# exanauts/SqpSolver.jl

Hardware: AMD Instinct MI355X
Metric: QP subproblems/sec on batched ACOPF; fp64 KKT LDL^T TFLOPS vs MFMA peak (higher is better)
Workload: dtype f64

## Files before the change

include/sqphip_test_hooks.h:

```cpp
#ifndef SQPHIP_TEST_HOOKS_H
#define SQPHIP_TEST_HOOKS_H
#include "sqphip.h"
#ifdef __cplusplus
extern "C" {
#endif

int sqphip_mf_host_solve(int64_t n, int64_t m, int64_t nnzJ, const int64_t *jrow, const int64_t *jcol,
                         int64_t nnzH, const int64_t *hrow, const int64_t *hcol, const double *gL, const double *gU,
                         int32_t condense, const double *Jval, const double *Hval, const double *Dd,
                         const double *sigp, const double *hd, const int32_t *rtype, double hsc, double dw,
                         const double *rhs, double *sol, double *dinv_by_unknown, int32_t *npos);
double sqphip_mf_host_top2_err(void);
double sqphip_mf_host_spine_err(void);
int sqphip_mf_solve_test(sqphip_ctx *ctx, int32_t inst, const double *Jval, const double *Hval, const double *Dd,
                         const double *sigp, const double *hd, const int32_t *rtype, double hsc, double dw,
                         const double *rhs, double *sol_fused, double *sol_standalone, double *dinv_by_unknown);
int sqphip_mf_batch_test(sqphip_ctx *ctx, const int32_t *active, const double *Jval, const double *Hval, const double *Dd,
                         const double *sigp, const double *hd, const int32_t *rtype, const double *hsc, const double *dw,
                         const double *dw_last, const int32_t *fac_attempt, const double *rhs, double *sol_fused,
                         double *sol_standalone, double *dinv0, double *dinv1, int32_t *decision, double *dw_out);
int sqphip_mf_census(const sqphip_ctx *ctx, int64_t *counts, char *names, int32_t cap, int32_t *n_kernels);
int sqphip_trans_inline_groups(const sqphip_ctx *ctx, int64_t *count);
int sqphip_mf_plan_info(int64_t n, int64_t m, int64_t nnzJ, const int64_t *jrow, const int64_t *jcol, int64_t nnzH,
                        const int64_t *hrow, const int64_t *hcol, const double *gL, const double *gU, int32_t condense,
                        int32_t batch, int32_t *fronts, int32_t cap_fronts, int32_t *n_fronts, int32_t *launches,
                        int32_t cap_launches, int32_t *n_launches, int64_t *top2_lds_bytes, int32_t *spine_fronts);
int sqphip_ldlt_factor_host(int32_t device, int32_t batch, int64_t N, double *A, double *dinv,
                            int32_t *npos);
int sqphip_ldlt_solve_host(int32_t device, int32_t batch, int64_t N, const double *A,
                           double *rhs);
int sqphip_ldlt_bench(int32_t device, int32_t batch, int64_t N, int32_t reps,
                      double *sec_per_factor, double *sec_trailing, int64_t *trailing_launches);
int sqphip_ldlt_tile_masks(int32_t batch, int64_t N, const double *A, int32_t Ts, uint8_t *tmask, int32_t *pair_ptr,
                           int32_t *pair_k, int32_t cap_k, int32_t *n_k);
int sqphip_ldlt_case_test(int32_t device, int32_t batch, int64_t N, const double *A, int32_t nan_upper, const double *rhs,
                          const int32_t *phase, int32_t want, int32_t Ts, int32_t no_tile_mask, double sentinel,
                          double *factor, double *dinv, int32_t *npos, double *b, double *v, double *x_fused,
                          double *x_standalone, int64_t *counts, char *names, int32_t cap, int64_t *info);

int sqphip_ldlt_stress(int32_t device, int32_t batch, int64_t N, int32_t reps, int32_t *mismatches);
int sqphip_mfma_f64_peak(int32_t device, double *tflops);

int sqphip_seat_peek(sqphip_ctx *ctx, int32_t inst, double *p, double *lambda, double *mult_x_U, double *mult_x_L,
                     double *slack, int32_t *moi_status);

#ifdef __cplusplus
}
#endif
#endif
```

sqpsolver.jl_amd/__init__.py:

```python
from . import acopf_synth
from . import dense_synth
from . import qcqp
from . import nlp_terms
from . import _lib
from . import host
from .host import (Context, QpData, QpHip, default_options, SqpHipError, kkt_order,
                   kkt_symbolic, mf_host_solve, mf_host_top2_err, mf_host_spine_err, mf_plan_info)
```

sqpsolver.jl_amd/_lib.py:

```python
from __future__ import annotations

import ctypes as C
import os
import subprocess
import sys

_CSRC = os.path.join(os.path.dirname(os.path.abspath(__file__)), "csrc")
SO_PATH = os.path.join(_CSRC, "libsqphip.so")
if os.environ.get("SQPHIP_SO"):
    SO_PATH = os.path.abspath(os.environ["SQPHIP_SO"])
SOURCES = ["ldlt.hip", "kernel_api.hip", "ipm.hip", "acopf.hip", "sqp.hip", "api.hip", "order.hip", "symbolic.hip",
           "mfplan.hip", "mfront.hip", "comm.hip"]
HEADERS = ["sqphip_internal.hpp", "ctx.hpp", "sparse.hpp", "dev_util.hpp", "mf_dev.hpp", "sqp_dev.hpp", "acopf_dev.hpp", "qcqp_dev.hpp", "nlp_dev.hpp", os.path.join("..", "..", "include", "sqphip.h"),
           os.path.join("..", "..", "include", "sqphip_test_hooks.h")]

_lib = None


EXTRA_FLAGS = {"mfront.hip": ["-mllvm", "-amdgpu-mfma-vgpr-form", "-mllvm", "-pragma-unroll-threshold=131072"]}
_OBJ = os.path.join(_CSRC, "build")


def build(force: bool = False, verbose: bool = False) -> str:
    from concurrent.futures import ThreadPoolExecutor
# ... 27 lines not shown
            if rc != 0 or verbose:
                sys.stderr.write("\n".join(other) + "\n")
            if rc != 0:
                raise subprocess.CalledProcessError(rc, cmd)
    objs = [os.path.join(_OBJ, sname + ".o") for sname in srcs]
    if jobs or not os.path.exists(SO_PATH) or any(os.path.getmtime(o) > os.path.getmtime(SO_PATH) for o in objs):
        cmd = [hipcc, "--offload-arch=gfx950", "-shared", "-fPIC", "-o", SO_PATH] + objs + ["-ldl"]
        if verbose:
            print(" ".join(cmd))
        subprocess.check_call(cmd)
        remarks = ""
        for o in objs:
            if os.path.exists(o + ".remarks"):
                remarks += open(o + ".remarks").read()
        _write_kernel_resources(remarks)
    return SO_PATH


RESOURCES_PATH = os.path.join(_CSRC, "kernel_resources.json")


def _write_kernel_resources(remarks: str) -> None:
    import json
    import re
    out, cur = {}, None
    for ln in remarks.splitlines():
        m = re.search(r"Function Name: (\S+)", ln)
        if m:
            cur = out.setdefault(m.group(1), {})
            continue
        m = re.search(r"remark:\s+(VGPRs|AGPRs|ScratchSize \[bytes/lane\]|LDS Size \[bytes/block\]|Occupancy \[waves/SIMD\]): (\d+)", ln)
        if m and cur is not None:
            cur[m.group(1).split(" [")[0]] = int(m.group(2))
    with open(RESOURCES_PATH, "w") as fh:
        json.dump(out, fh, indent=0, sort_keys=True)


class Options(C.Structure):
    _fields_ = [(k, C.c_double) for k in
                ("tol_direction", "tol_residual", "tol_infeas", "init_mu", "max_mu", "tr_size",
                 "rho", "eta", "tau", "min_alpha")] + \
               [("max_iter", C.c_int32), ("use_soc", C.c_int32), ("literal_quirks", C.c_int32),
                ("ipm_tol", C.c_double), ("ipm_max_iter", C.c_int32), ("ipm_phase1", C.c_int32),
                ("device", C.c_int32), ("ipm_corrector", C.c_int32),
                ("kkt_condense", C.c_int32), ("kkt_tile_order", C.c_int32), ("kkt_mode", C.c_int32),
                ("ipm_warm_start", C.c_int32)]


class Counters(C.Structure):
    _fields_ = [("n_qp", C.c_int64), ("n_ipm_iter", C.c_int64), ("n_factor", C.c_int64),
                ("ldlt_flops", C.c_double), ("ldlt_seconds", C.c_double),
                ("trailing_seconds", C.c_double), ("solve_seconds", C.c_double),
                ("total_seconds", C.c_double), ("trailing_launches", C.c_int64), ("kkt_order", C.c_int64),
                ("lead_tiles", C.c_int64), ("trailing_flops_per_factor", C.c_double),
                ("sparse", C.c_int64), ("nnz_k", C.c_int64), ("nnz_l", C.c_int64), ("n_supernodes", C.c_int64),
                ("n_levels", C.c_int64), ("max_front", C.c_int64), ("factor_flops", C.c_double),
                ("front_doubles", C.c_int64), ("cb_doubles", C.c_int64), ("factor_launches", C.c_int64),
                ("solve_launches", C.c_int64), ("n_sweeps", C.c_int64), ("n_solve", C.c_int64), ("n_groups", C.c_int64),
                ("nnz_l_top", C.c_int64), ("nnz_k_top", C.c_int64), ("cols_top", C.c_int64)]


class SymbolicStats(C.Structure):
    _fields_ = [(k, C.c_int64) for k in ("order", "nnz_k_lower", "n_supernodes", "n_levels", "max_front", "max_cols",
                                         "nnz_l", "nnz_l_exact")] + \
               [("flops", C.c_double), ("flops_exact", C.c_double), ("front_doubles", C.c_int64)]


def lib():
    global _lib
    if _lib is None:
        if not os.path.exists(SO_PATH):
            raise RuntimeError(
                f"{SO_PATH} is missing: build it with __graft_entry__.build() "
                "(hipcc --offload-arch=gfx950); this package has no CPU fallback")
        L = C.CDLL(SO_PATH)
        dp, ip, lp = C.POINTER(C.c_double), C.POINTER(C.c_int32), C.POINTER(C.c_int64)
        vp = C.c_void_p
        if hasattr(L, "sqphip_default_options"):
            L.sqphip_default_options.argtypes = [C.POINTER(Options)]
        L.sqphip_ldlt_factor_host.argtypes = [C.c_int32, C.c_int32, C.c_int64, dp, dp, ip]
        L.sqphip_ldlt_solve_host.argtypes = [C.c_int32, C.c_int32, C.c_int64, dp, dp]
        L.sqphip_ldlt_bench.argtypes = [C.c_int32, C.c_int32, C.c_int64, C.c_int32, dp, dp, lp]
        L.sqphip_mfma_f64_peak.argtypes = [C.c_int32, dp]
        L.sqphip_ldlt_tile_masks.argtypes = [C.c_int32, C.c_int64, dp, C.c_int32, C.POINTER(C.c_uint8), ip, ip, C.c_int32, ip]
        L.sqphip_ldlt_case_test.argtypes = [C.c_int32, C.c_int32, C.c_int64, dp, C.c_int32, dp, ip, C.c_int32, C.c_int32,
                                            C.c_int32, C.c_double, dp, dp, ip, dp, dp, dp, dp, lp, C.c_char_p, C.c_int32, lp]
        if hasattr(L, "sqphip_create"):
            L.sqphip_create.argtypes = [C.POINTER(vp), C.c_int64, C.c_int64, C.c_int64,
                                        C.c_int64, lp, lp, C.c_int64, lp, lp, dp, dp, dp, dp,
                                        C.POINTER(Options), C.c_int32]
            L.sqphip_destroy.argtypes = [vp]
            L.sqphip_last_error.restype = C.c_char_p
            L.sqphip_last_error.argtypes = [vp]
            L.sqphip_set_bounds.argtypes = [vp, C.c_int32, dp, dp, dp, dp]
            L.sqphip_qp_solve.argtypes = [vp, C.c_int32, dp, C.c_double, C.c_double, dp, dp, dp, dp,
                                          dp, dp, dp, dp, dp, ip]
            L.sqphip_qp_stats.argtypes = [vp, ip, ip]
            if hasattr(L, "sqphip_qp_solve_batch"):
                L.sqphip_qp_solve_batch.argtypes = [vp, C.c_int32, ip, ip] + [dp] * 7 + [dp] * 5 + [ip]
                L.sqphip_qp_stats_batch.argtypes = [vp, C.c_int32, ip, ip, ip, ip, dp]
                L.sqphip_seat_peek.argtypes = [vp, C.c_int32, dp, dp, dp, dp, dp, ip]
                L.sqphip_norm_violations_batch.argtypes = [vp, C.c_int32, ip, dp, dp, C.c_int32, dp]
                L.sqphip_kt_residuals_batch.argtypes = [vp, C.c_int32, ip, dp, dp, dp, dp, dp, dp]
                L.sqphip_norm_complementarity_batch.argtypes = [vp, C.c_int32, ip, dp, dp, C.c_int32, dp]
                L.sqphip_compute_phi_batch.argtypes = [vp, C.c_int32, ip, dp, dp, dp, dp, C.c_int32, dp]
                L.sqphip_compute_qmodel_batch.argtypes = [vp, C.c_int32, ip, dp, dp, dp, dp, dp, dp, dp, C.c_int32, dp]
                L.sqphip_compute_derivative_full_batch.argtypes = [vp, C.c_int32, ip, dp, dp, dp, dp, dp, C.c_int32, dp, dp]
            L.sqphip_qp_termination.argtypes = [vp, ip, dp]
            L.sqphip_sqp_qp_log_term.argtypes = [vp, C.c_int32, dp, ip, C.c_int32, ip]
            L.sqphip_get_termination_counters.argtypes = [vp, C.POINTER(C.c_int64)]
            L.sqphip_norm_violations.argtypes = [vp, dp, dp, C.c_int32, dp]
            L.sqphip_kt_residuals.argtypes = [vp, dp, dp, dp, dp, dp, dp]
            L.sqphip_norm_complementarity.argtypes = [vp, dp, dp, C.c_int32, dp]
            L.sqphip_compute_phi.argtypes = [vp, C.c_double, dp, dp, C.c_double, C.c_int32, dp]
            L.sqphip_compute_qmodel.argtypes = [vp, dp, dp, dp, dp, dp, dp, C.c_double, C.c_int32, dp]
            L.sqphip_compute_derivative.argtypes = [vp, dp, dp, dp, C.c_double, dp]
            L.sqphip_compute_derivative_full.argtypes = [vp, dp, dp, dp, C.c_double, dp, C.c_int32, dp, dp]
            L.sqphip_compute_mu_rule_dev.argtypes = [vp, C.c_int32, C.c_int64, C.c_double, dp, dp, dp, dp, dp, dp, dp]
            L.sqphip_acopf_armijo.argtypes = [vp, C.c_int32, dp, dp] + [C.c_double] * 6 + [C.c_int32, dp, ip, ip]
            L.sqphip_tr_update.argtypes = [C.c_double, C.c_double, C.c_double, C.c_double,
                                           C.c_double, C.c_double, ip, dp]
            L.sqphip_acopf_attach.argtypes = [vp, C.c_int32, C.c_int32, C.c_int32, ip, ip, ip, ip, ip,
                                              ip, dp, C.c_int32]
            L.sqphip_acopf_attach_acr.argtypes = [vp, C.c_int32, C.c_int32, C.c_int32, ip, ip, ip, ip, ip,
                                              ip, dp, C.c_int32]
            L.sqphip_acopf_attach_acwr.argtypes = [vp, C.c_int32, C.c_int32, C.c_int32, ip, ip, ip, ip, ip, ip, dp, C.c_int32,
                                                   C.c_int32, ip, ip, ip, dp, dp, dp]
            L.sqphip_acopf_set_instance.argtypes = [vp, C.c_int32, dp, dp, dp, dp]
            L.sqphip_dense_attach.argtypes = [vp, dp, dp, C.c_double]
            L.sqphip_dense_set_instance.argtypes = [vp, C.c_int32, dp, dp]
            L.sqphip_qcqp_attach.argtypes = [vp, C.c_int64, lp, lp, dp, C.c_int64, lp, lp, dp, C.c_int64, lp, lp, lp, dp,
                                             dp, dp, C.c_double]
            L.sqphip_qcqp_set_instance.argtypes = [vp, C.c_int32] + [dp] * 7
            if not os.environ.get("SQPHIP_SO") or hasattr(L, "sqphip_nlp_attach"):
                L.sqphip_nlp_attach.argtypes = [vp, C.c_int64, lp, dp, lp, lp, ip, ip, dp, dp, dp, C.c_double]
                L.sqphip_nlp_set_instance.argtypes = [vp, C.c_int32, dp, dp, dp, dp]
            if not os.environ.get("SQPHIP_SO") or hasattr(L, "sqphip_nlp_attach_affine"):
                L.sqphip_nlp_attach_affine.argtypes = [vp, C.c_int64, lp, dp, lp, lp, lp, dp, ip, ip, dp, dp, C.c_double]
            L.sqphip_acopf_set_shunts.argtypes = [vp, C.c_int32, ip, dp, dp]
            L.sqphip_acopf_set_dclines.argtypes = [vp, C.c_int32, dp]
            L.sqphip_kkt_order.argtypes = [C.c_int64, C.c_int64, C.c_int64, lp, lp, C.c_int64, lp, lp, dp, dp, C.c_int32,
                                           ip, ip, ip]
            L.sqphip_kkt_symbolic.argtypes = [C.c_int64, C.c_int64, C.c_int64, lp, lp, C.c_int64, lp, lp, dp, dp, C.c_int32,
                                              C.c_int32, C.c_int32, C.c_double, ip, C.POINTER(SymbolicStats)]
            L.sqphip_mf_host_solve.argtypes = [C.c_int64, C.c_int64, C.c_int64, lp, lp, C.c_int64, lp, lp, dp, dp, C.c_int32,
                                               dp, dp, dp, dp, dp, ip, C.c_double, C.c_double, dp, dp, dp, ip]
            L.sqphip_mf_host_top2_err.argtypes = []
            L.sqphip_mf_host_top2_err.restype = C.c_double
            L.sqphip_mf_host_spine_err.argtypes = []
            L.sqphip_mf_host_spine_err.restype = C.c_double
            L.sqphip_mf_solve_test.argtypes = [vp, C.c_int32, dp, dp, dp, dp, dp, ip, C.c_double, C.c_double, dp, dp, dp, dp]
            L.sqphip_mf_batch_test.argtypes = [vp, ip, dp, dp, dp, dp, dp, ip, dp, dp, dp, ip, dp, dp, dp, dp, dp, ip, dp]
            L.sqphip_mf_census.argtypes = [vp, lp, C.c_char_p, C.c_int32, ip]
            if hasattr(L, "sqphip_trans_inline_groups"):
                L.sqphip_trans_inline_groups.argtypes = [vp, lp]
            L.sqphip_mf_plan_info.argtypes = [C.c_int64, C.c_int64, C.c_int64, lp, lp, C.c_int64, lp, lp, dp, dp, C.c_int32,
                                              C.c_int32, ip, C.c_int32, ip, ip, C.c_int32, ip, lp, ip]
            L.sqphip_acopf_eval.argtypes = [vp, C.c_int32, dp, C.c_double, dp, dp, dp, dp, dp, dp]
            L.sqphip_sqp_reset.argtypes = [vp]
            L.sqphip_sqp_run.argtypes = [vp, C.c_int32]
            L.sqphip_sqp_get.argtypes = [vp, C.c_int32, dp, dp, dp, dp, dp, dp, ip, ip]
            L.sqphip_sqp_status.argtypes = [vp, ip, ip, ip]
            L.sqphip_sqp_trace.argtypes = [vp, C.c_int32, dp, C.c_int32, ip]
            L.sqphip_comm_unique_id.argtypes = [vp]
            L.sqphip_comm_init.argtypes = [vp, vp, C.c_int32, C.c_int32]
            L.sqphip_gather_status.argtypes = [vp, C.c_int32, ip, ip, ip]
            L.sqphip_comm_destroy.argtypes = [vp]
            L.sqphip_get_counters.argtypes = [vp, C.POINTER(Counters)]
            L.sqphip_get_mode_counters.argtypes = [vp, C.POINTER(C.c_int64)]
            L.sqphip_sqp_qp_log.argtypes = [vp, C.c_int32, ip, C.c_int32, ip]
            L.sqphip_sqp_last_request.argtypes = [vp, C.c_int32, ip, dp, dp, dp, dp, dp, dp, dp]
            L.sqphip_sqp_stream_begin.argtypes = [vp, C.c_int32]
            L.sqphip_sqp_stream_set.argtypes = [vp, C.c_int32] + [dp] * 8
            L.sqphip_sqp_stream_run.argtypes = [vp]
            L.sqphip_sqp_stream_get.argtypes = [vp, C.c_int32, dp, dp, ip, ip]
            L.sqphip_qcqp_stream_begin.argtypes = [vp, C.c_int32, C.c_int32]
            L.sqphip_qcqp_stream_set.argtypes = [vp, C.c_int32] + [dp] * 11
            L.sqphip_sqp_stream_get_full.argtypes = [vp, C.c_int32, dp, dp, dp, dp, dp, dp, ip, ip]
            if not os.environ.get("SQPHIP_SO") or hasattr(L, "sqphip_nlp_stream_begin"):
                L.sqphip_nlp_stream_begin.argtypes = [vp, C.c_int32, C.c_int32]
                L.sqphip_nlp_stream_set.argtypes = [vp, C.c_int32] + [dp] * 8
            L.sqphip_sqp_work.argtypes = [vp, C.POINTER(C.c_int64), C.POINTER(C.c_int64), C.POINTER(C.c_int64)]
            L.sqphip_reset_counters.argtypes = [vp]
            L.sqphip_set_timing.argtypes = [vp, C.c_int32]
            L.sqphip_get_kernel_times.argtypes = [vp, dp, C.POINTER(C.c_int64), C.c_int32]
        _lib = L
    return _lib


EXPORTS = [
    "sqphip_default_options", "sqphip_create", "sqphip_destroy", "sqphip_last_error",
    "sqphip_set_bounds", "sqphip_qp_solve", "sqphip_qp_stats",
    "sqphip_qp_solve_batch", "sqphip_qp_stats_batch", "sqphip_seat_peek", "sqphip_norm_violations_batch", "sqphip_kt_residuals_batch",
    "sqphip_norm_complementarity_batch", "sqphip_compute_phi_batch", "sqphip_compute_qmodel_batch",
    "sqphip_compute_derivative_full_batch", "sqphip_qp_termination", "sqphip_sqp_qp_log_term", "sqphip_get_termination_counters", "sqphip_norm_violations",
    "sqphip_kt_residuals", "sqphip_norm_complementarity", "sqphip_compute_phi",
    "sqphip_compute_qmodel", "sqphip_compute_derivative", "sqphip_compute_derivative_full", "sqphip_compute_mu_rule_dev",
    "sqphip_acopf_armijo", "sqphip_tr_update",
    "sqphip_kkt_order", "sqphip_kkt_symbolic", "sqphip_mf_host_solve", "sqphip_mf_host_top2_err", "sqphip_mf_host_spine_err", "sqphip_mf_solve_test", "sqphip_mf_batch_test", "sqphip_mf_census", "sqphip_trans_inline_groups", "sqphip_mf_plan_info", "sqphip_acopf_attach", "sqphip_acopf_attach_acr", "sqphip_acopf_attach_acwr", "sqphip_acopf_set_shunts", "sqphip_acopf_set_dclines", "sqphip_acopf_set_instance", "sqphip_dense_attach", "sqphip_dense_set_instance", "sqphip_qcqp_attach", "sqphip_qcqp_set_instance", "sqphip_nlp_attach", "sqphip_nlp_attach_affine", "sqphip_nlp_set_instance", "sqphip_acopf_eval", "sqphip_sqp_reset",
    "sqphip_sqp_run", "sqphip_sqp_get", "sqphip_sqp_status", "sqphip_sqp_trace",
    "sqphip_comm_available", "sqphip_comm_unique_id", "sqphip_comm_init", "sqphip_gather_status", "sqphip_comm_destroy",
    "sqphip_get_counters", "sqphip_get_mode_counters", "sqphip_sqp_work", "sqphip_sqp_stream_begin", "sqphip_sqp_stream_set", "sqphip_sqp_stream_run", "sqphip_sqp_stream_get", "sqphip_sqp_stream_assign", "sqphip_sqp_stream_append", "sqphip_sqp_stream_release", "sqphip_sqp_stream_run_some", "sqphip_qcqp_stream_begin", "sqphip_qcqp_stream_set", "sqphip_nlp_stream_begin", "sqphip_nlp_stream_set", "sqphip_sqp_stream_get_full", "sqphip_sqp_last_request", "sqphip_sqp_qp_log", "sqphip_reset_counters", "sqphip_set_timing", "sqphip_get_kernel_times", "sqphip_ldlt_factor_host",
    "sqphip_ldlt_solve_host", "sqphip_ldlt_bench", "sqphip_ldlt_stress", "sqphip_ldlt_tile_masks", "sqphip_ldlt_case_test", "sqphip_mfma_f64_peak", "sqphip_armijo_alpha", "sqphip_compute_mu_rule",
]
```

sqpsolver.jl_amd/csrc/api.hip:

```cpp
#include "ctx.hpp"
#include "qcqp_dev.hpp"
#include "nlp_dev.hpp"
#include <algorithm>
#include <array>
#include <chrono>
#include <cmath>
#include <cstring>
#include <tuple>
#include <unordered_map>

using namespace sqphip;

Ctx::~Ctx()
{
    lanes.clear();
    tm.flush();
    comm_release(*this);
    plan.destroy_lookahead();
    for (void *p : allocs) hipFree(p);
    if (h_counters) hipHostFree(h_counters);
    if (stg_h) hipHostFree(stg_h);
    if (side) { hipStreamDestroy(side); for (auto &e : evS) if (e) hipEventDestroy(e); for (auto &e : evC) if (e) hipEventDestroy(e); }
    if (stream && owns_stream) hipStreamDestroy(stream);
}
// ... 161 lines not shown
    const IpmState *ist;
    long ist_off;
};

template <bool TO_SLOTS>
__global__ __launch_bounds__(256) void k_seat_stage(StageMap M, double *stg, const int *inst)
{
    const int k = blockIdx.y, b = inst[k];
    double *row = stg + (long)k * M.row;
#pragma unroll
    for (int f = 0; f < SQPHIP_SEAT_FIELDS; ++f) {
        if (f >= M.nf) break;
        const int len = M.len[f];
        double *slot = M.base[f] + (long)b * M.stride[f];
        const bool al = ((unsigned long)slot & 15ul) == 0;
        for (int q = blockIdx.x * 256 + threadIdx.x; 2 * q < len; q += gridDim.x * 256) {
            const bool two = 2 * q + 1 < len;
            if (TO_SLOTS) {
                const double2 v = M.off[f] < 0 ? make_double2(0.0, 0.0) : *(const double2 *)(row + M.off[f] + 2 * q);
                if (two && al) *(double2 *)(slot + 2 * q) = v;
                else { slot[2 * q] = v.x; if (two) slot[2 * q + 1] = v.y; }
            } else {
                double2 v;
                if (two && al) v = *(const double2 *)(slot + 2 * q);
                else { v.x = slot[2 * q]; v.y = two ? slot[2 * q + 1] : 0.0; }
                *(double2 *)(row + M.off[f] + 2 * q) = v;
            }
        }
    }
    if (!TO_SLOTS && M.ist && blockIdx.x == 0) {
        constexpr int W = (int)(sizeof(IpmState) / 8);
        const unsigned long long *src = (const unsigned long long *)(M.ist + b);
        unsigned long long *dst = (unsigned long long *)(stg + M.ist_off) + (long)k * W;
        for (int w = threadIdx.x; w < W; w += 256) dst[w] = src[w];
    }
}
static_assert(sizeof(IpmState) % 8 == 0, "k_seat_stage copies IpmState in 8-byte words");

__global__ void k_mf_test_setup(DV d, int inst, double hsc, double dw, int ph)
{
    for (int i = threadIdx.x; i < d.B; i += blockDim.x) { d.phase[i] = PH_IDLE; d.ist[i].start = 0; }
    __syncthreads();
    if (threadIdx.x == 0) { d.ist[inst].hsc = hsc; d.ist[inst].dw = dw; d.ist[inst].stage = 0; d.ist[inst].sel = 0; d.ist[inst].fac_attempt = 0; d.phase[inst] = ph; }
}

__global__ void k_mf_inst_set(DV d, int inst, int start, int ph, double hsc, double dw, double dw_last, int fac_attempt)
{
    if (threadIdx.x != 0) return;
    IpmState &I = d.ist[inst];
    I.start = start;
    if (start) { I.mode = 0; I.delta = 1.0; I.mu_pen = 1.0; I.rho_big = 1e4; I.ipm_iters = 0; I.n_solve = 0; I.status = 0; }
    I.stage = 0; I.hsc = hsc; I.dw = dw; I.dw_last = dw_last; I.sel = 0; I.fac_attempt = fac_attempt; I.n_factor = 0; I.rc = 0;
    d.phase[inst] = ph;
}

}

extern "C" void sqphip_default_options(sqphip_options *o)
{
    o->tol_direction = 1e-8; o->tol_residual = 1e-8; o->tol_infeas = 1e-8;
    o->init_mu = 1.0; o->max_mu = 1e10; o->tr_size = 10.0;
    o->rho = 0.8; o->eta = 0.4; o->tau = 0.9; o->min_alpha = 1e-6;
    o->max_iter = 3000; o->use_soc = 0; o->literal_quirks = 1;
    o->ipm_tol = 1e-9; o->ipm_max_iter = 200; o->ipm_phase1 = 0; o->device = 0; o->ipm_corrector = 0; o->kkt_condense = 1; o->kkt_tile_order = 1;
    o->kkt_mode = 0; o->ipm_warm_start = 0;
}

extern "C" int sqphip_create(sqphip_ctx **out, int64_t n, int64_t m, int64_t num_linear, int64_t nnzJ,
                             const int64_t *jrow, const int64_t *jcol, int64_t nnzH, const int64_t *hrow,
                             const int64_t *hcol, const double *xL, const double *xU, const double *gL,
                             const double *gU, const sqphip_options *opt, int32_t batch)
{
    if (!out || n <= 0 || m < 0 || batch <= 0 || !opt || num_linear < 0 || num_linear > m) return SQPHIP_EINVAL;
    if (nnzJ < 0 || nnzH < 0 || (nnzJ > 0 && (!jrow || !jcol)) || (nnzH > 0 && (!hrow || !hcol))) return SQPHIP_EINVAL;
    if (!xL || !xU || (m > 0 && (!gL || !gU))) return SQPHIP_EINVAL;
    for (int64_t k = 0; k < nnzJ; ++k)
        if (jrow[k] < 1 || jrow[k] > m || jcol[k] < 1 || jcol[k] > n) return SQPHIP_EINVAL;
    for (int64_t k = 0; k < nnzH; ++k)
        if (hrow[k] < 1 || hrow[k] > n || hcol[k] < 1 || hcol[k] > n) return SQPHIP_EINVAL;
    for (int64_t i = 0; i < m; ++i)
        if (gL[i] == -INFINITY && gU[i] == INFINITY) return SQPHIP_EINVAL;
    sqphip_ctx *h = new (std::nothrow) sqphip_ctx();
    if (!h) return SQPHIP_ENOMEM;
    h->c.opt = *opt;
    int rc = guarded(h, [&](Ctx &C) {
        SQPHIP_HIP_OK(hipStreamCreate(&C.stream));
        SQPHIP_HIP_OK(hipHostMalloc((void **)&C.h_counters, 8 * sizeof(int)));
        DV &d = C.d;
        std::memset(&d, 0, sizeof(d));
        C.n = n; C.m = m;
        C.h_jrow.assign(jrow, jrow + nnzJ); C.h_jcol.assign(jcol, jcol + nnzJ);
        C.h_hrow.assign(hrow, hrow + nnzH); C.h_hcol.assign(hcol, hcol + nnzH);
        C.h_xL.assign(xL, xL + n); C.h_xU.assign(xU, xU + n);
        if (m > 0) { C.h_gL.assign(gL, gL + m); C.h_gU.assign(gU, gU + m); }
        const int B = batch;
        d.n = (int)n; d.m = (int)m; d.nlin = (int)num_linear; d.N = (int)(n + m);
        d.Npad = (d.N + 63) / 64 * 64; d.B = B;
        d.nnzj_coo = (int)nnzJ; d.nnzh_coo = (int)nnzH;
        Pattern PJ = build_pattern(n, nnzJ, jrow, jcol, false);
        Pattern PH = build_pattern(n, nnzH, hrow, hcol, true);
        d.nnzjc = (int)PJ.rowval.size(); d.nnzhc = (int)PH.rowval.size();
        d.hfull = n > 1 && (long)d.nnzhc == (long)n * n;
        std::vector<int> rptr(m + 1, 0), rcol(d.nnzjc), rslot(d.nnzjc);
        for (int s = 0; s < d.nnzjc; ++s) rptr[PJ.rowval[s] + 1]++;
        for (int64_t i = 0; i < m; ++i) rptr[i + 1] += rptr[i];
        {
            std::vector<int> fill(rptr.begin(), rptr.end() - 1);
            for (int j = 0; j < (int)n; ++j)
                for (int s = PJ.colptr[j]; s < PJ.colptr[j + 1]; ++s) {
                    const int i = PJ.rowval[s];
                    rcol[fill[i]] = j; rslot[fill[i]] = s; fill[i]++;
                }
        }
        d.jcolptr = C.upload(PJ.colptr); d.jrowval = C.upload(PJ.rowval);
        d.jrowptr = C.upload(rptr); d.jrcol = C.upload(rcol); d.jrslot = C.upload(rslot);
        {
            std::vector<int> kpos(m > 0 ? m : 1, -1), krow;
            for (int64_t i = 0; i < m; ++i)
                if (kkt_row_is_kept(gL[i], gU[i], rptr[i + 1] - rptr[i])) { kpos[i] = (int)krow.size(); krow.push_back((int)i); }
            d.condense = opt->kkt_condense != 0; d.mk = (int)krow.size();
            if (krow.empty()) krow.push_back(0);
            d.kpos = C.upload(kpos); d.krow = C.upload(krow);
            C.h_kpos = kpos;
        }
        {
            const std::vector<int> &kpos = C.h_kpos;
            const int nu = d.condense ? d.n + d.mk : d.N;
            std::vector<int> upos(nu);
            d.Ts = 0; d.Nf = nu; d.sparse = 0;
            if (opt->kkt_mode != 1) {
                std::vector<int> kp(kpos);
                if (!d.condense) for (int64_t i = 0; i < m; ++i) kp[i] = (int)i;
                const SymOptions so = mf_sym_options(B);
                C.mfp_ = std::make_shared<MfPlan>(mf_build_plan(d.n, (int)m, kp, d.condense ? d.mk : (int)m, PH.colptr, PH.rowval, rptr, rcol, rslot, so));
                const SparseSym &S = C.mfp().S;
                const double dense_flops = (double)nu * nu * nu / 3.0;
                const bool fits = S.max_front <= 1024;
                if (opt->kkt_mode == 2 && !fits) throw std::string("kkt_mode = 2: a front of " + std::to_string(S.max_front) + " rows exceeds the multifrontal kernels' limit (1024)");
                d.sparse = opt->kkt_mode == 2 || (fits && S.max_front <= 512 && S.flops <= 0.25 * dense_flops);
            }
            if (d.sparse) {
                const MfPlan &P = C.mfp();
                const SparseSym &S = P.S;
                upos = S.pos;
                MfDev &M = d.mf;
                M.ns = S.ns; M.stride = P.stride;
                M.first = C.upload(S.sn_first); M.nc = C.upload(S.sn_nc); M.nr = C.upload(S.sn_nr);
                M.rowptr = C.upload(S.sn_rowptr); M.rows = C.upload(S.sn_rows.empty() ? std::vector<int>(1, 0) : S.sn_rows);
                M.rel = C.upload(S.rel.empty() ? std::vector<int>(1, 0) : S.rel);
                M.child_ptr = C.upload(S.child_ptr); M.child = C.upload(S.child.empty() ? std::vector<int>(1, 0) : S.child);
                M.off = C.upload(P.off);
                M.asm_ptr = C.upload(P.asm_ptr); M.dest_loc = C.upload(P.dest_loc); M.item_ptr = C.upload(P.item_ptr);
                M.items = C.upload(P.items); M.sched = C.upload(P.sched);
                auto nz = [](const std::vector<int> &v) { return v.empty() ? std::vector<int>(1, 0) : v; };
                M.dest_rc = C.upload(P.dest_rc);
                M.ea_ptr = C.upload(P.ea_ptr); M.ea_rc = C.upload(nz(P.ea_rc));
                M.ea_src_ptr = C.upload(P.ea_src_ptr); M.ea_src = C.upload(nz(P.ea_src));
                M.ev_ptr = C.upload(P.ev_ptr); M.ev_idx = C.upload(nz(P.ev_idx));
                M.ev_src_ptr = C.upload(P.ev_src_ptr); M.ev_src = C.upload(nz(P.ev_src));
                M.level_ptr = C.upload(S.level_ptr); M.level_sn = C.upload(S.level_sn);
                M.nlevels = S.nlevels; M.max_front = S.max_front;
                M.sol_items = C.upload(nz(P.sol_items));
                M.desc = C.upload(P.desc);
                M.ea_ent = C.upload(P.ea_ent.empty() ? std::vector<MfGather>(1) : P.ea_ent);
                M.ev_ent = C.upload(P.ev_ent.empty() ? std::vector<MfGather>(1) : P.ev_ent);
                int lds_max = 0;
                if (hipDeviceGetAttribute(&lds_max, hipDeviceAttributeMaxSharedMemoryPerBlock, C.opt.device) != hipSuccess) lds_max = 0;
                M.top_n = P.top2_lds_bytes > 0 && P.top2_lds_bytes <= lds_max ? (int)P.top_fr.size() : 0;
                if (M.top_n > 0) {
                    M.top_fr = C.upload(P.top_fr); M.top_gptr = C.upload(P.top_gptr); M.top_gsrc = C.upload(nz(P.top_gsrc));
                    M.top_rows = C.upload(nz(P.top_rows)); M.top_ext = C.upload(nz(P.top_ext));
                    M.top_next = (int)P.top_ext.size(); M.top_utotal = P.top_utotal; M.top_xtotal = P.top_xtotal;
                    M.top_buf0 = P.top_buf0; M.top_buf1 = P.top_buf1;
                }
                M.sp_n = P.spine_lds_bytes > 0 && P.spine_lds_bytes <= lds_max ? (int)P.sp_fr.size() : 0;
                if (M.sp_n > 0) {
                    M.sp_fr = C.upload(P.sp_fr); M.sp_ent = C.upload(P.sp_ent.empty() ? std::vector<MfGather>(1) : P.sp_ent);
                    M.sp_src = C.upload(nz(P.sp_src)); M.sp_rel = C.upload(nz(P.sp_rel)); M.sp_T = P.spine_T; M.sp_stage = P.spine_stage;
                }
                M.nnzK = (int)P.nnzK;
                M.vals = C.dalloc<double>((size_t)B * P.nnzK);
                M.fronts = C.dalloc<double>((size_t)B * P.stride);
                const bool small_arena = (double)B * (double)P.stride * 8.0 <= 1e9;
                d.spec_mode = getenv("SQPHIP_MF_SPEC") ? atoi(getenv("SQPHIP_MF_SPEC")) : (B <= (opt->ipm_corrector ? 256 : 192) && small_arena ? 1 : 0);
                C.spec_tail = d.spec_mode == 0 && small_arena ? (getenv("SQPHIP_MF_SPEC_TAIL") ? atoi(getenv("SQPHIP_MF_SPEC_TAIL")) : (getenv("SQPHIP_MF_SPEC") ? 0 : 32)) : 0;
                C.spec_mode0 = d.spec_mode;
            } else if (d.condense && opt->kkt_tile_order) {
                KktOrder o = kkt_order(d.n, (int)m, kpos, d.mk, PH.colptr, PH.rowval, rptr, rcol, true);
                upos = o.pos; d.Ts = o.Ts; d.Nf = o.Nf;
                if (o.Ts > 0 && o.Tr > 0 && !getenv("SQPHIP_NO_TILE_MASK")) {
                    C.plan.tmask = C.upload(o.tmask);
                    d.tmask = C.plan.tmask;
                    C.plan.pair_ptr = C.upload(o.pair_ptr);
                    C.plan.pair_k = C.upload(o.pair_k.empty() ? std::vector<int>(1, 0) : o.pair_k);
                    double fl = 0.0;
                    for (int ti = 0, pi = 0; ti < o.Tr; ++ti)
                        for (int tj = 0; tj <= ti; ++tj, ++pi)
                            fl += (ti == tj ? 64.0 * 65.0 / 2.0 : 64.0 * 64.0) * 2.0 * 64.0 * (o.pair_ptr[pi + 1] - o.pair_ptr[pi]);
                    C.plan.lead_update_flops = fl;
                }
            } else {
                for (int u = 0; u < nu; ++u) upos[u] = u;
            }
            d.Fpad = (d.Nf + 63) / 64 * 64; d.ld = d.Fpad;
            std::vector<int> uinv(d.Fpad, -1);
            for (int u = 0; u < nu; ++u) uinv[upos[u]] = u;
            d.upos = C.upload(upos); d.uinv = C.upload(uinv);
        }
        d.hcolptr = C.upload(PH.colptr); d.hrowval = C.upload(PH.rowval);
        d.jg_ptr = C.upload(PJ.g_ptr); d.jg_src = C.upload(PJ.g_src);
        d.hg_ptr = C.upload(PH.g_ptr); d.hg_src = C.upload(PH.g_src);
        const size_t Bn = (size_t)B * n, Bm = (size_t)B * m, BN = (size_t)B * d.Npad;
        d.xL = C.dalloc<double>(Bn); d.xU = C.dalloc<double>(Bn);
        d.gL = C.dalloc<double>(Bm); d.gU = C.dalloc<double>(Bm);
        for (int b = 0; b < B; ++b) {
            h2d(C, d.xL + (size_t)b * n, xL, n); h2d(C, d.xU + (size_t)b * n, xU, n);
            h2d(C, d.gL + (size_t)b * m, gL, m); h2d(C, d.gU + (size_t)b * m, gU, m);
        }
        d.xk = C.dalloc<double>(Bn); d.cin = C.dalloc<double>(Bn); d.bE = C.dalloc<double>(Bm);
        d.jcoo = C.dalloc<double>((size_t)B * nnzJ); d.hcoo = C.dalloc<double>((size_t)B * nnzH);
        d.jv = C.dalloc<double>((size_t)B * d.nnzjc); d.hv = C.dalloc<double>((size_t)B * d.nnzhc);
        double **nvec[] = { &d.c, &d.hd, &d.lb, &d.ub, &d.p, &d.zl, &d.zu, &d.dp, &d.dzl, &d.dzu, &d.rd,
                            &d.sigp, &d.wn, &d.op, &d.omxU, &d.omxL, &d.x, &d.mxL, &d.mxU, &d.df, &d.pstep,
                            &d.psoc, &d.pmxL, &d.pmxU, &d.tmpx, &d.x0, &d.socZL, &d.socZU };
        for (auto pp : nvec) *pp = C.dalloc<double>(Bn);
        double **mvec[] = { &d.lo, &d.hi, &d.wp, &d.wm, &d.s, &d.tp, &d.tm, &d.y, &d.vl, &d.vu, &d.ds,
                            &d.dtp, &d.dtm, &d.dy, &d.dvl, &d.dvu, &d.rp, &d.Dd, &d.olam, &d.lambda, &d.E,
                            &d.plam, &d.Esoc, &d.tmpE, &d.hlam, &d.zp, &d.zm, &d.rdir,
                            &d.socZP, &d.socZM, &d.socVL, &d.socVU };
        for (auto pp : mvec) *pp = C.dalloc<double>(Bm);
        d.oslack = C.dalloc<double>(2 * Bm);
        d.rtype = C.dalloc<int>(Bm); d.rbase = C.dalloc<int>(Bm); d.hard = C.dalloc<int>(Bm);
        d.rhs = C.dalloc<double>(BN); d.sol = C.dalloc<double>(BN); d.wN = C.dalloc<double>(BN);
        const size_t BF = (size_t)B * d.Fpad;
        d.xv = C.dalloc<double>(BF); d.vv = C.dalloc<double>(BF); d.dinv = C.dalloc<double>(BF);
        d.K = C.dalloc<double>(d.sparse ? 1 : (size_t)B * d.ld * d.Fpad);
        d.ist = C.dalloc<IpmState>(B); d.sst = C.dalloc<SqpState>(B);
        d.phase = C.dalloc<int>(B); d.counters = C.dalloc<int>(64);
        d.trace = C.dalloc<double>((size_t)B * SQPHIP_TRACE_CAP * SQPHIP_TRACE_COLS);
        d.ipm_tol = opt->ipm_tol; d.ipm_max_iter = opt->ipm_max_iter; d.ipm_phase1 = opt->ipm_phase1; d.ipm_corrector = opt->ipm_corrector; d.ipm_warm = opt->ipm_warm_start;
        d.refine_tol = getenv("SQPHIP_REFINE_TOL") ? atof(getenv("SQPHIP_REFINE_TOL")) : 1e-11;
        d.vstage = (d.n + d.N <= 7000 && !getenv("SQPHIP_NO_VSTAGE")) ? d.n + d.N : 0;
        d.flat = getenv("SQPHIP_VEC_FLAT") ? (atoi(getenv("SQPHIP_VEC_FLAT")) != 0) : (d.vstage == 0 && d.n + d.N > 7000);
        d.vals_inline = d.sparse && !d.flat && getenv("SQPHIP_MF_VALS_INLINE") && atoi(getenv("SQPHIP_MF_VALS_INLINE")) == 1;
        if (d.vals_inline) C.spec_tail = 0;
        if (d.sparse && (d.spec_mode != 0 || C.spec_tail > 0)) {
            d.mf.vals1 = C.dalloc<double>((size_t)B * C.mfp().nnzK);
            d.mf.fronts1 = C.dalloc<double>((size_t)B * C.mfp().stride);
            d.vv1 = C.dalloc<double>(BF); d.dinv1 = C.dalloc<double>(BF);
        }
        if (d.flat) {
            d.vstage = 0;
            d.fH = C.dalloc<double>(Bn); d.fJt = C.dalloc<double>(Bn); d.fJ = C.dalloc<double>(Bm); d.fX = C.dalloc<double>(Bm);
        }
        d.tol_direction = opt->tol_direction; d.tol_residual = opt->tol_residual;
        d.tol_infeas = opt->tol_infeas; d.init_mu = opt->init_mu; d.tr_size = opt->tr_size;
        d.max_iter = opt->max_iter; d.use_soc = opt->use_soc; d.literal_quirks = opt->literal_quirks;
        C.plan.N = d.Nf; C.plan.Npad = d.Fpad; C.plan.T = d.Fpad / 64; C.plan.ld = d.ld; C.plan.B = B;
        C.plan.Ts = d.Ts;
        C.plan.stream = C.stream;
        if (opt->kkt_tile_order && !d.condense && !d.sparse)
            C.err = "note: options.kkt_tile_order needs options.kkt_condense = 1 and was ignored";
        if (!d.sparse) {
            C.plan.Wbuf = C.dalloc<double>((size_t)std::max(2 * LdltPlan::MAX_R, d.Ts) * B * d.Fpad * 64);
            C.plan.init_lookahead();
        }
        SQPHIP_HIP_OK(hipStreamSynchronize(C.stream));
        if (const char *e = getenv("SQPHIP_TRANS_PERIOD")) C.trans_period = atoi(e);
        if (const char *e = getenv("SQPHIP_TRANS_RIDE")) C.trans_ride = atoi(e);
        C.refine_slot = getenv("SQPHIP_REFINE_SLOT") && atoi(getenv("SQPHIP_REFINE_SLOT")) == 1;
        if (const char *e = getenv("SQPHIP_REFINE_PERIOD")) C.refine_period = atoi(e);
        if (d.sparse) mf_device_setup(C);
        C.post_split = getenv("SQPHIP_POST_SPLIT") && atoi(getenv("SQPHIP_POST_SPLIT")) == 1;
        C.side_mode = getenv("SQPHIP_SIDE_TRANS") && atoi(getenv("SQPHIP_SIDE_TRANS")) == 1;
        make_lanes(C);
        return SQPHIP_OK;
    });
    if (rc != SQPHIP_OK) {
        fprintf(stderr, "sqphip_create: %s\n", h->c.err.c_str());
        delete h;
        return rc;
    }
    *out = h;
    return SQPHIP_OK;
}

extern "C" void sqphip_destroy(sqphip_ctx *h)
{
    if (!h) return;
    hipSetDevice(h->c.opt.device);
    delete h;
}

extern "C" const char *sqphip_last_error(const sqphip_ctx *h) { return h ? h->c.err.c_str() : "null context"; }

extern "C" int sqphip_set_bounds(sqphip_ctx *h, int32_t inst, const double *xL, const double *xU,
                                 const double *gL, const double *gU)
{
    if (!h || inst < 0 || inst >= h->c.d.B || !xL || !xU || (h->c.d.m > 0 && (!gL || !gU))) return SQPHIP_EINVAL;
    for (int i = 0; i < h->c.d.m; ++i)
        if (gL[i] == -INFINITY && gU[i] == INFINITY) { h->c.err = "sqphip_set_bounds: row " + std::to_string(i) + " is unbounded on both sides"; return SQPHIP_EINVAL; }
    return guarded(h, [&](Ctx &C) {
        DV &d = C.d;
        if (d.condense)
            for (int i = 0; i < d.m; ++i)
                if (gL[i] == gU[i] && C.h_kpos[i] < 0) {
// ... 5 lines not shown
        h2d(C, d.gL + (size_t)inst * d.m, gL, d.m); h2d(C, d.gU + (size_t)inst * d.m, gU, d.m);
        SQPHIP_HIP_OK(hipStreamSynchronize(C.stream));
        return SQPHIP_OK;
    });
}

extern "C" int sqphip_qp_solve(sqphip_ctx *h, int32_t mode, const double *x_k, double delta, double mu,
                               const double *df, const double *E, const double *Jval, const double *Hval,
                               double *p, double *lambda, double *mult_x_U, double *mult_x_L, double *slack,
                               int32_t *moi_status)
{
    if (!h || !x_k || !Jval || !p || !lambda || !mult_x_U || !mult_x_L || !moi_status) return SQPHIP_EINVAL;
    if (mode < 0 || mode > SQPHIP_MODE_INFEAS) return SQPHIP_EINVAL;
    if (mode != SQPHIP_MODE_LP && (!df || !E)) return SQPHIP_EINVAL;
    return guarded(h, [&](Ctx &C) {
        DV &d = C.d;
        auto t0 = std::chrono::steady_clock::now();
        h2d(C, d.xk, x_k, d.n);
        h2d(C, d.cin, df, d.n);
        h2d(C, d.bE, E, d.m);
        h2d(C, d.jcoo, Jval, d.nnzj_coo);
        if (Hval) h2d(C, d.hcoo, Hval, d.nnzh_coo);
        else SQPHIP_HIP_OK(hipMemsetAsync(d.hcoo, 0, sizeof(double) * (size_t)d.nnzh_coo, C.stream));
        hipLaunchKernelGGL(k_qp_request, dim3(1), dim3(64), 0, C.stream, d, 0, (int)mode, delta, mu);
        launch_qp_gather(C);
        ipm_run_all(C);
        IpmState st;
        SQPHIP_HIP_OK(hipMemcpyAsync(&st, d.ist, sizeof(IpmState), hipMemcpyDeviceToHost, C.stream));
        d2h(C, p, d.op, d.n); d2h(C, lambda, d.olam, d.m);
        d2h(C, mult_x_U, d.omxU, d.n); d2h(C, mult_x_L, d.omxL, d.n);
        d2h(C, slack, d.oslack, 2 * (size_t)d.m);
        SQPHIP_HIP_OK(hipStreamSynchronize(C.stream));
        *moi_status = st.status;
        C.last_ipm_iters = st.ipm_iters; C.last_n_factor = st.n_factor;
        C.last_rule = st.rc == 0 ? st.acc_rule : -1; C.last_e0 = st.e0;
        C.n_qp += 1; C.n_ipm_iter += st.ipm_iters; C.n_factor += st.n_factor; C.n_solve += st.n_solve;
        C.total_seconds += std::chrono::duration<double>(std::chrono::steady_clock::now() - t0).count();
        return SQPHIP_OK;
    });
}

extern "C" int sqphip_mf_solve_test(sqphip_ctx *h, int32_t inst, const double *Jval, const double *Hval,
                                    const double *Dd, const double *sigp, const double *hd, const int32_t *rtype,
                                    double hsc, double dw, const double *rhs, double *sol_fused,
                                    double *sol_standalone, double *dinv_by_unknown)
{
    if (!h || inst < 0 || inst >= h->c.d.B || !Jval || !Dd || !sigp || !hd || !rtype || !rhs) return SQPHIP_EINVAL;
    if (!h->c.d.sparse) { h->c.err = "sqphip_mf_solve_test: the context does not use the sparse solver"; return SQPHIP_ESTATE; }
    return guarded(h, [&](Ctx &C) {
        DV &d = C.d;
        const SparseSym &S = C.mfp().S;
        const size_t on = (size_t)inst * d.n, om = (size_t)inst * d.m;
        h2d(C, d.jcoo + (size_t)inst * d.nnzj_coo, Jval, d.nnzj_coo);
        if (Hval) h2d(C, d.hcoo + (size_t)inst * d.nnzh_coo, Hval, d.nnzh_coo);
        else SQPHIP_HIP_OK(hipMemsetAsync(d.hcoo + (size_t)inst * d.nnzh_coo, 0, sizeof(double) * (size_t)d.nnzh_coo, C.stream));
        hipLaunchKernelGGL(k_qp_request, dim3(1), dim3(64), 0, C.stream, d, (int)inst, 0, 1.0, 1.0);
        launch_qp_gather(C);
        hipLaunchKernelGGL(k_mf_test_setup, dim3(1), dim3(64), 0, C.stream, d, (int)inst, hsc, dw, (int)PH_FACTOR);
        h2d(C, d.Dd + om, Dd, d.m); h2d(C, d.sigp + on, sigp, d.n); h2d(C, d.hd + on, hd, d.n);
        SQPHIP_HIP_OK(hipMemcpyAsync(d.rtype + om, rtype, sizeof(int) * (size_t)d.m, hipMemcpyHostToDevice, C.stream));
        std::vector<double> xp(d.Fpad, 0.0), out(d.Fpad), dv(d.Fpad);
        for (int u = 0; u < S.nu; ++u) xp[S.pos[u]] = rhs[u];
        double *xv = d.xv + (size_t)inst * d.Fpad;
        h2d(C, xv, xp.data(), d.Fpad);
        mf_factor(C, PH_FACTOR, true);
        mf_solve(C, PH_FACTOR, true);
        d2h(C, out.data(), xv, d.Fpad); d2h(C, dv.data(), d.dinv + (size_t)inst * d.Fpad, d.Fpad);
        SQPHIP_HIP_OK(hipStreamSynchronize(C.stream));
        for (int u = 0; u < S.nu; ++u) {
            if (sol_fused) sol_fused[u] = out[S.pos[u]];
            if (dinv_by_unknown) dinv_by_unknown[u] = dv[S.pos[u]];
        }
        h2d(C, xv, xp.data(), d.Fpad);
        mf_solve(C, PH_FACTOR, false);
        d2h(C, out.data(), xv, d.Fpad);
        hipLaunchKernelGGL(k_mf_test_setup, dim3(1), dim3(64), 0, C.stream, d, (int)inst, 0.0, 0.0, (int)PH_IDLE);
        SQPHIP_HIP_OK(hipStreamSynchronize(C.stream));
        SQPHIP_HIP_OK(hipGetLastError());
        if (sol_standalone) for (int u = 0; u < S.nu; ++u) sol_standalone[u] = out[S.pos[u]];
        return SQPHIP_OK;
    });
}

extern "C" int sqphip_mf_batch_test(sqphip_ctx *h, const int32_t *active, const double *Jval, const double *Hval,
                                    const double *Dd, const double *sigp, const double *hd, const int32_t *rtype,
                                    const double *hsc, const double *dw, const double *dw_last, const int32_t *fac_attempt,
                                    const double *rhs, double *sol_fused, double *sol_standalone, double *dinv0,
                                    double *dinv1, int32_t *decision, double *dw_out)
{
    if (!h || !active || !Jval || !Dd || !sigp || !hd || !rtype || !hsc || !dw || !dw_last || !fac_attempt || !rhs)
        return SQPHIP_EINVAL;
    if (!h->c.d.sparse) { h->c.err = "sqphip_mf_batch_test: the context does not use the sparse solver"; return SQPHIP_ESTATE; }
    return guarded(h, [&](Ctx &C) {
        DV &d = C.d;
        const SparseSym &S = C.mfp().S;
        const int B = d.B, nu = S.nu;
        std::vector<double> xp((size_t)B * d.Fpad, 0.0), out((size_t)B * d.Fpad), dv((size_t)B * d.Fpad), dv1((size_t)B * d.Fpad, 0.0);
        for (int b = 0; b < B; ++b) {
            const size_t on = (size_t)b * d.n, om = (size_t)b * d.m;
            h2d(C, d.jcoo + (size_t)b * d.nnzj_coo, Jval + (size_t)b * d.nnzj_coo, d.nnzj_coo);
            if (Hval) h2d(C, d.hcoo + (size_t)b * d.nnzh_coo, Hval + (size_t)b * d.nnzh_coo, d.nnzh_coo);
            else SQPHIP_HIP_OK(hipMemsetAsync(d.hcoo + (size_t)b * d.nnzh_coo, 0, sizeof(double) * (size_t)d.nnzh_coo, C.stream));
            h2d(C, d.Dd + om, Dd + om, d.m); h2d(C, d.sigp + on, sigp + on, d.n); h2d(C, d.hd + on, hd + on, d.n);
            SQPHIP_HIP_OK(hipMemcpyAsync(d.rtype + om, rtype + om, sizeof(int) * (size_t)d.m, hipMemcpyHostToDevice, C.stream));
            for (int u = 0; u < nu; ++u) xp[(size_t)b * d.Fpad + S.pos[u]] = rhs[(size_t)b * nu + u];
            hipLaunchKernelGGL(k_mf_inst_set, dim3(1), dim3(64), 0, C.stream, d, b, active[b] ? 1 : 0, (int)PH_IDLE, 0.0, 0.0, 0.0, 0);
        }
        h2d(C, d.xv, xp.data(), xp.size());
        launch_qp_gather(C);
        for (int b = 0; b < B; ++b)
            hipLaunchKernelGGL(k_mf_inst_set, dim3(1), dim3(64), 0, C.stream, d, b, 0, active[b] ? (int)PH_FACTOR : (int)PH_IDLE,
                               hsc[b], dw[b], dw_last[b], (int)fac_attempt[b]);
        const bool top_inertia = mf_solve_tests_inertia(C);
        mf_factor(C, PH_FACTOR, true);
        if (!top_inertia) launch_inertia(C);
        mf_solve(C, PH_SOLVE, true, top_inertia);
        d2h(C, out.data(), d.xv, out.size()); d2h(C, dv.data(), d.dinv, dv.size());
        if (d.dinv1) d2h(C, dv1.data(), d.dinv1, dv1.size());
        std::vector<IpmState> st(B);
        std::vector<int> ph(B);
        SQPHIP_HIP_OK(hipMemcpyAsync(st.data(), d.ist, sizeof(IpmState) * (size_t)B, hipMemcpyDeviceToHost, C.stream));
        SQPHIP_HIP_OK(hipMemcpyAsync(ph.data(), d.phase, sizeof(int) * (size_t)B, hipMemcpyDeviceToHost, C.stream));
        SQPHIP_HIP_OK(hipStreamSynchronize(C.stream));
        for (int b = 0; b < B; ++b) {
            const size_t f = (size_t)b * d.Fpad, o = (size_t)b * nu;
            for (int u = 0; u < nu; ++u) {
                if (sol_fused) sol_fused[o + u] = out[f + S.pos[u]];
                if (dinv0) dinv0[o + u] = dv[f + S.pos[u]];
                if (dinv1) dinv1[o + u] = dv1[f + S.pos[u]];
            }
            const IpmState &I = st[b];
            const bool spec = d.mf.fronts1 != nullptr && d.spec_mode != 0 && (fac_attempt[b] > 0 || (d.spec_mode == 1 && dw[b] > 0.0));
            if (decision) {
                int32_t *r = decision + 5 * (size_t)b;
                r[0] = !active[b] ? 0 : ph[b] == PH_FACTOR ? 1 : ph[b] == PH_SOLVE ? 2 : 3;
                r[1] = I.sel; r[2] = I.n_factor; r[3] = I.fac_attempt; r[4] = active[b] && spec ? 1 : 0;
            }
            if (dw_out) dw_out[b] = I.dw;
        }
        h2d(C, d.xv, xp.data(), xp.size());
        mf_solve(C, PH_SOLVE, false);
        d2h(C, out.data(), d.xv, out.size());
        for (int b = 0; b < B; ++b)
            hipLaunchKernelGGL(k_mf_inst_set, dim3(1), dim3(64), 0, C.stream, d, b, 0, (int)PH_IDLE, 0.0, 0.0, 0.0, 0);
        SQPHIP_HIP_OK(hipStreamSynchronize(C.stream));
        SQPHIP_HIP_OK(hipGetLastError());
        if (sol_standalone)
            for (int b = 0; b < B; ++b)
                for (int u = 0; u < nu; ++u) sol_standalone[(size_t)b * nu + u] = out[(size_t)b * d.Fpad + S.pos[u]];
        return SQPHIP_OK;
    });
}

extern "C" int sqphip_mf_census(const sqphip_ctx *h, int64_t *counts, char *names, int32_t cap, int32_t *n_kernels)
{
    if (!h || cap < 0 || (cap > 0 && !counts)) return SQPHIP_EINVAL;
    if (n_kernels) *n_kernels = MFK_COUNT;
    for (int k = 0; k < MFK_COUNT && k < cap; ++k) {
        long c = h->c.mf_census[k];
        for (const auto &L : h->c.lanes) c += L->mf_census[k];
        counts[k] = c;
        if (names) { std::strncpy(names + 64 * (size_t)k, mf_kernel_names[k], 63); names[64 * (size_t)k + 63] = 0; }
    }
    return SQPHIP_OK;
}

extern "C" int sqphip_trans_inline_groups(const sqphip_ctx *h, int64_t *count)
{
    if (!h || !count) return SQPHIP_EINVAL;
    long c = h->c.n_trans_inline;
    for (const auto &L : h->c.lanes) c += L->n_trans_inline;
    *count = c;
    return SQPHIP_OK;
}

extern "C" int sqphip_qp_stats(const sqphip_ctx *h, int32_t *ipm_iters, int32_t *n_factor)
{
    if (!h) return SQPHIP_EINVAL;
    if (ipm_iters) *ipm_iters = h->c.last_ipm_iters;
    if (n_factor) *n_factor = h->c.last_n_factor;
    return SQPHIP_OK;
}

extern "C" int sqphip_qp_termination(const sqphip_ctx *h, int32_t *rule, double *scaled_error)
{
    if (!h) return SQPHIP_EINVAL;
    if (rule) *rule = h->c.last_rule;
    if (scaled_error) *scaled_error = h->c.last_e0;
    return SQPHIP_OK;
}

namespace {

inline long ev(long k) { return (k + 1) & ~1L; }

int seat_check(sqphip_ctx *h, const char *fn, int32_t count, const int32_t *inst)
{
    Ctx &C = h->c;
    if (count < 1 || count > C.d.B) { C.err = std::string(fn) + ": count " + std::to_string(count) + " is outside 1 .. batch = " + std::to_string(C.d.B); return SQPHIP_EINVAL; }
    if (!inst) { C.err = std::string(fn) + ": inst is NULL"; return SQPHIP_EINVAL; }
    std::vector<int> seen((size_t)C.d.B, -1);
    for (int k = 0; k < count; ++k) {
        if (inst[k] < 0 || inst[k] >= C.d.B) { C.err = std::string(fn) + ": inst[" + std::to_string(k) + "] = " + std::to_string(inst[k]) + " is outside 0 .. batch - 1 = " + std::to_string(C.d.B - 1); return SQPHIP_EINVAL; }
        if (seen[inst[k]] >= 0) { C.err = std::string(fn) + ": inst[" + std::to_string(k) + "] = " + std::to_string(inst[k]) + " repeats inst[" + std::to_string(seen[inst[k]]) + "]"; return SQPHIP_EINVAL; }
        seen[inst[k]] = k;
    }
    return SQPHIP_OK;
}

struct SeatCall {
    Ctx &C;
    int count; long cp, rows0;
    StageMap in{}, out{};
    const double *src[SQPHIP_SEAT_FIELDS] = {};
    SeatCall(Ctx &C_, int count_) : C(C_), count(count_), cp(ev(count_)), rows0(3 * ev(count_))
    {
        if (!C.stg_h) {
            const DV &d = C.d;
            const long row = 3 * ev(d.n) + 4 * ev(d.m) + ev(d.nnzj_coo) + ev(d.nnzh_coo) + (long)(sizeof(IpmState) / 8) + 2;
            C.stg_doubles = 3 * ev(d.B) + (long)d.B * row;
            SQPHIP_HIP_OK(hipHostMalloc((void **)&C.stg_h, sizeof(double) * (size_t)C.stg_doubles));
            C.stg_d = C.dalloc<double>((size_t)C.stg_doubles);
        }
    }
    double *a0() { return C.stg_h; }
    double *a1() { return C.stg_h + cp; }
    int *inst() { return (int *)(C.stg_h + 2 * cp); }
    int *mode() { return (int *)(C.stg_h + 2 * cp) + cp; }
    const double *a0_dev() const { return C.stg_d; }
    const double *a1_dev() const { return C.stg_d + cp; }
    const int *inst_dev() const { return (const int *)(C.stg_d + 2 * cp); }
    const int *mode_dev() const { return (const int *)(C.stg_d + 2 * cp) + cp; }
    void operand(const double *host, double *base, int len, bool zero = false)
    {
        if ((!host && !zero) || len == 0) return;
        const int f = in.nf++;
        in.len[f] = len; in.stride[f] = len; in.base[f] = base; src[f] = host;
        in.off[f] = host ? in.row : -1;
        if (host) in.row += (int)ev(len);
    }
    void result(double *base, int len)
    {
        if (len == 0) return;
        const int f = out.nf++;
        out.len[f] = len; out.stride[f] = len; out.base[f] = base; out.off[f] = out.row;
        out.row += (int)ev(len);
    }
    static dim3 grid(const StageMap &M, int count) { return dim3((unsigned)std::min(32L, std::max(1L, (M.row / 2 + 255L) / 256)), (unsigned)count); }
    void send(const int32_t *inst_host, const int32_t *mode_host, const double *a0_host, const double *a1_host)
    {
        for (int k = 0; k < count; ++k) {
            a0()[k] = a0_host ? a0_host[k] : 0.0; a1()[k] = a1_host ? a1_host[k] : 0.0;
            inst()[k] = inst_host[k]; mode()[k] = mode_host ? mode_host[k] : 0;
        }
        for (int k = 0; k < count; ++k)
            for (int f = 0; f < in.nf; ++f)
                if (src[f]) std::memcpy(C.stg_h + rows0 + (long)k * in.row + in.off[f], src[f] + (size_t)k * in.len[f], sizeof(double) * (size_t)in.len[f]);
        SQPHIP_HIP_OK(hipMemcpyAsync(C.stg_d, C.stg_h, sizeof(double) * (size_t)(rows0 + (long)count * in.row), hipMemcpyHostToDevice, C.stream));
        if (in.nf) hipLaunchKernelGGL(k_seat_stage<true>, grid(in, count), dim3(256), 0, C.stream, in, C.stg_d + rows0, inst_dev());
    }
    long fetch(bool with_states, long extra = 0)
    {
        const long body = (long)count * out.row;
        out.ist = with_states ? C.d.ist : nullptr; out.ist_off = body;
        if (out.nf || with_states) hipLaunchKernelGGL(k_seat_stage<false>, grid(out, count), dim3(256), 0, C.stream, out, C.stg_d + rows0, inst_dev());
        const long total = body + (with_states ? (long)count * (long)(sizeof(IpmState) / 8) : 0) + extra;
        SQPHIP_HIP_OK(hipMemcpyAsync(C.stg_h + rows0, C.stg_d + rows0, sizeof(double) * (size_t)total, hipMemcpyDeviceToHost, C.stream));
        SQPHIP_HIP_OK(hipStreamSynchronize(C.stream));
        SQPHIP_HIP_OK(hipGetLastError());
        return body;
    }
    void unpack(int f, double *host) const
    {
        if (!host) return;
        for (int k = 0; k < count; ++k)
            std::memcpy(host + (size_t)k * out.len[f], C.stg_h + rows0 + (long)k * out.row + out.off[f], sizeof(double) * (size_t)out.len[f]);
    }
    IpmState state(int k, long body) const
    {
        IpmState st;
        std::memcpy(&st, (const char *)(C.stg_h + rows0 + body) + sizeof(IpmState) * (size_t)k, sizeof(IpmState));
        return st;
    }
};

}

extern "C" int sqphip_qp_solve_batch(sqphip_ctx *h, int32_t count, const int32_t *inst, const int32_t *mode, const double *x_k,
                                     const double *delta, const double *mu, const double *df, const double *E,
                                     const double *Jval, const double *Hval, double *p, double *lambda, double *mult_x_U,
                                     double *mult_x_L, double *slack, int32_t *moi_status)
{
    if (!h || !mode || !x_k || !delta || !mu || !Jval || !p || !lambda || !mult_x_U || !mult_x_L || !moi_status) return SQPHIP_EINVAL;
    if (int rc = seat_check(h, "sqphip_qp_solve_batch", count, inst)) return rc;
    for (int k = 0; k < count; ++k) {
        if (mode[k] < 0 || mode[k] > SQPHIP_MODE_INFEAS) { h->c.err = "sqphip_qp_solve_batch: mode[" + std::to_string(k) + "] = " + std::to_string(mode[k]) + " is no sub-problem mode"; return SQPHIP_EINVAL; }
        if (mode[k] != SQPHIP_MODE_LP && (!df || !E)) { h->c.err = "sqphip_qp_solve_batch: mode[" + std::to_string(k) + "] needs df and E"; return SQPHIP_EINVAL; }
    }
    return guarded(h, [&](Ctx &C) {
        DV &d = C.d;
        auto t0 = std::chrono::steady_clock::now();
        SeatCall S(C, count);
        S.operand(x_k, d.xk, d.n); S.operand(df, d.cin, d.n); S.operand(E, d.bE, d.m);
        S.operand(Jval, d.jcoo, d.nnzj_coo); S.operand(Hval, d.hcoo, d.nnzh_coo, true);
        S.send(inst, mode, delta, mu);
        hipLaunchKernelGGL(k_qp_request_batch, dim3(1), dim3(256), 0, C.stream, d, (int)count, S.inst_dev(), S.mode_dev(), S.a0_dev(), S.a1_dev());
// ... 1546 lines not shown
```

sqpsolver.jl_amd/csrc/ctx.hpp:

```cpp
#pragma once
#include <memory>
#include <vector>
#include "../../include/sqphip.h"
#include "../../include/sqphip_test_hooks.h"
#include "sqphip_internal.hpp"
#include "sparse.hpp"

namespace sqphip {

enum { PH_IDLE = 0, PH_PREP = 1, PH_FACTOR = 2, PH_SOLVE = 3, PH_STEP = 4, PH_MPC = 5, PH_RESOLVE = 6, PH_DONE = 9,
       PH_PEND = 10, PH_DONE2 = 11, PH_PREP_S = 12 };
enum { ROW_FREE = 0, ROW_EQ = 1, ROW_INEQ = 2 };

enum MfKernel { MFK_VALUES, MFK_FACTOR_R1, MFK_F2_1_3, MFK_F2_2_5, MFK_F2_4_4, MFK_F2_4_9, MFK_F2_8_12,
                MFK_FRONT_1, MFK_FRONT_2, MFK_FRONT_3, MFK_FRONT_4_2, MFK_FRONT_4_4, MFK_FRONT_5_2, MFK_FRONT_5_4,
                MFK_FRONT_6_4, MFK_FRONT_6_4_IMG, MFK_FRONT_6_8_IMG, MFK_FRONT_7_4, MFK_FRONT_7_4_IMG, MFK_FRONT_7_8_IMG,
                MFK_FRONT_8_4, MFK_FRONT_8_4_IMG, MFK_FRONT_8_8_IMG, MFK_FRONT_9, MFK_FRONT_10, MFK_FRONT_11, MFK_FRONT_12,
                MFK_SPINE, MFK_SOLVE_INST, MFK_FWD, MFK_FWD2, MFK_FWD2_BIG, MFK_SOLVE_TOP, MFK_SOLVE_TOP2, MFK_BWD, MFK_BWD2,
                MFK_BWD2_BIG, MFK_INERTIA, MFK_COUNT };
extern const char *const mf_kernel_names[];

struct IpmState {
    int mode, start, stage;
    double delta, mu_pen;
    double sf, rho_big, soft_w, hsc;
    double mu, tau, dw, dw_last, dw_floor, cn, relres, rn, e0;
    int iter, rc, fac_attempt, dir_attempt, refine_it, n_acc, n_acc2, n_acc3;
    int mpc, use_soc;
    double cavg;
    double e_best;
    int n_stall;
    int prev_mode;
    int status, ipm_iters, n_factor, n_solve;
    int reload;
    int sel;
    int acc_rule;
    double elastic;
};

#define SQPHIP_QLOG_CAP 64
struct SqpState {
    double f, phi, mu, Delta, prim_infeas, dual_infeas, pnorm, obj_val;
    double f_trial, phi_k, q0, ared, pred;
    int iter, ret, step_acceptance, fr, sub_status, done, stage, need_qp, qp_mode, want_eval;
    int n_qp, trace_len, it_ipm, soc_pending, lp_pending, started;
    long tot_ipm, tot_fac, tot_sol;
    long md_qp[4], md_ipm[4], md_fac[4];
    int qlog_n, qlog[4 * SQPHIP_QLOG_CAP];
    float qerr[SQPHIP_QLOG_CAP];
    signed char qrule[SQPHIP_QLOG_CAP];
    long term_rule[4];
    int budget;
};

enum { ST_TOP = 0, ST_QP = 1, ST_SOC = 2, ST_LP = 3, ST_DONE = 4 };

#define SQPHIP_TRACE_COLS 12
#define SQPHIP_TRACE_CAP 4096

struct MfDev {
    int ns;
    const int *first, *nc, *nr, *rowptr, *rows, *rel, *child_ptr, *child;
    const long *off;
    long stride;
    double *fronts;
    double *fronts1, *vals1;
    const int *asm_ptr, *dest_loc, *dest_rc, *item_ptr;
    const MfItem *items;
    const int *ea_ptr, *ea_rc, *ea_src_ptr, *ea_src;
    const int *ev_ptr, *ev_idx, *ev_src_ptr, *ev_src;
    const MfFrontDesc *desc;
    const MfGather *ea_ent, *ev_ent;
    const int *level_ptr, *level_sn;
    int nlevels, max_front;
    const int *sched, *sol_items;
    const MfTopFront *top_fr;
    const int *top_gptr, *top_gsrc, *top_rows, *top_ext;
    int top_n, top_next, top_utotal, top_xtotal, top_buf0, top_buf1;
    const MfSpineFront *sp_fr;
    const MfGather *sp_ent;
    const int *sp_src, *sp_rel;
    int sp_n, sp_T, sp_stage;
    int nnzK;
    double *vals;
};

struct StreamDev {
    int M;
    int *next;
    int *qend;
    int *qids;
    int *slot_scen;
    const double *xL, *xU, *gL, *gU, *ohm, *c2, *c1, *x0;
    double *rx, *robj;
    int *rstat, *riter;
    const double *val;
    double *rE, *rlam, *rmxL, *rmxU;
};

struct QcqpDev;
struct NlpDev;

struct DV {
    int n, m, nlin, N, Npad, ld, B;
    int Nf, Fpad;
    int condense, mk;
    const int *kpos, *krow;
    const int *upos, *uinv;
    int Ts;
    const unsigned char *tmask;
    int sparse;
    MfDev mf;
    int nnzj_coo, nnzh_coo, nnzjc, nnzhc;
    const int *jcolptr, *jrowval, *jrowptr, *jrcol, *jrslot;
    const int *hcolptr, *hrowval;
    const int *jg_ptr, *jg_src, *hg_ptr, *hg_src;
    double *xL, *xU, *gL, *gU;
    double *xk, *cin, *bE, *jcoo, *hcoo, *jv, *hv;
    double *c, *hd, *lb, *ub, *lo, *hi, *wp, *wm;
    int *rtype, *rbase, *hard;
    double *p, *zl, *zu, *s, *tp, *tm, *y, *vl, *vu, *zp, *zm, *rdir;
    double *dp, *dzl, *dzu, *ds, *dtp, *dtm, *dy, *dvl, *dvu;
    double *rd, *rp, *sigp, *Dd, *rhs, *sol, *wn, *wN;
    double *socZL, *socZU, *socZP, *socZM, *socVL, *socVU;
    double *K, *dinv, *xv, *vv;
    double *dinv1, *vv1;
    int spec_mode;
    double *op, *olam, *omxU, *omxL, *oslack;
    IpmState *ist;
    int *phase;
    int *counters;
    double ipm_tol;
    int ipm_max_iter, ipm_phase1, ipm_corrector, ipm_warm;
    int side;
    double refine_tol;
    int vstage;
    int hfull;
    int vals_inline;
    int flat;
    double *fH, *fJt, *fJ, *fX;
    double *x, *lambda, *mxL, *mxU, *df, *E, *pstep, *psoc, *plam, *pmxL, *pmxU, *Esoc, *tmpx, *tmpE,
        *hlam;
    SqpState *sst;
    double *trace;
    int nb, ng, nl, ref_bus;
    StreamDev stream;
    int dense_nlp;
    const double *dnQ, *dnA;
    double *dnc; double dn_kappa;
    int acr;
    int acwr, nbp;
    const int *bp_i, *bp_j, *br_bp;
    const double *br_sig, *bp_tmin, *bp_tmax;
    int ndc; const double *dc_loss1;
    int nsh; const int *sh_bus, *sh_of_bus; const double *sh_gs, *sh_bs;
    const int *f_bus, *t_bus, *gen_bus, *bal_ptr, *bal_colP, *bal_colQ;
    const double *bal_coef;
    double *br_ohm, *c2, *c1, *x0;
    double tol_direction, tol_residual, tol_infeas, init_mu, tr_size;
    int max_iter, use_soc, literal_quirks;
    const QcqpDev *qc;
    double *qcv;
    const NlpDev *nlp;
    double *nlv, *nlw;
};

static __device__ __forceinline__ int ph_done(const DV &d) { return d.side == 2 ? PH_DONE2 : PH_DONE; }
static __device__ __forceinline__ int ph_prep(const DV &d) { return d.side == 1 ? PH_PREP_S : PH_PREP; }
static __device__ __forceinline__ int ph_fact(const DV &d) { return d.side == 1 ? PH_PEND : PH_FACTOR; }

struct Ctx {
    sqphip_options opt;
    DV d;
    LdltPlan plan;
    std::shared_ptr<MfPlan> mfp_;
    const MfPlan &mfp() const { return *mfp_; }
    std::vector<std::unique_ptr<Ctx>> lanes;
    bool is_lane = false, owns_stream = true;
    long mf_factor_launches = 0, n_sweeps = 0;
    long mf_census[MFK_COUNT] = {};
    long run_sweep = 0;
    bool post_split = false;
    bool want_resolve = true;
    bool side_mode = false, side_on = false;
    hipStream_t side = nullptr;
    hipEvent_t evS[4] = {}, evC[4] = {};
    int spec_tail = 0, spec_mode0 = 0;
    bool refine_slot = false;
    int refine_period = 0;
    long resolve_served = -1;
    int trans_period = 0;
    int trans_ride = -1;
    long n_trans_inline = 0;
    Timers tm;
    std::vector<void *> allocs;
    std::string err;
    hipStream_t stream = nullptr;
    int *h_counters = nullptr;
    double *stg_h = nullptr, *stg_d = nullptr;
    long stg_doubles = 0;
    std::vector<int> h_kpos;
    std::vector<int64_t> h_jrow, h_jcol, h_hrow, h_hcol;
    long qc_nv = 0;
    long qc_off[7] = {};
    std::vector<double> h_qc_base;
    long nl_nv = 0, nl_nfac = 0, nl_nterms = 0;
    std::vector<double> h_nl_base;
    std::vector<double> h_xL, h_xU, h_gL, h_gU;
    bool acopf_attached = false;
    bool mf_big_lds = false;
    bool stream_started = false;
    void *comm = nullptr, *comm_buf = nullptr;
    int comm_world = 1, comm_rank = 0, comm_cap = 0;
    int64_t n = 0, m = 0;
    int64_t n_qp = 0, n_ipm_iter = 0, n_factor = 0, n_solve = 0;
    double total_seconds = 0;
    int last_ipm_iters = 0, last_n_factor = 0, last_rule = -1;
    double last_e0 = 0.0;

    template <class T> T *dalloc(size_t count)
    {
        void *p = nullptr;
        SQPHIP_HIP_OK(hipMalloc(&p, sizeof(T) * (count ? count : 1)));
        SQPHIP_HIP_OK(hipMemsetAsync(p, 0, sizeof(T) * (count ? count : 1), stream));
        allocs.push_back(p);
        return (T *)p;
    }
    template <class T> T *upload(const std::vector<T> &v)
    {
        T *p = dalloc<T>(v.size());
        if (!v.empty())
            SQPHIP_HIP_OK(hipMemcpyAsync(p, v.data(), sizeof(T) * v.size(), hipMemcpyHostToDevice, stream));
        return p;
    }
    ~Ctx();
};

void ipm_run_all(Ctx &C);
bool ipm_sweep(Ctx &C, bool sqp_level, int *host_slot = nullptr);
void sqp_stage_kernels(Ctx &C, hipStream_t s, const DV &d);
void sqp_stream_arm(Ctx &C);
void sqp_stream_rearm(Ctx &C);
void launch_qp_gather(Ctx &C);
void comm_release(Ctx &C);
void mf_device_setup(Ctx &C);
void mf_factor(Ctx &C, int want, bool with_rhs, bool values_done = false);
void mf_solve(Ctx &C, int want, bool skip_fwd, bool inertia = false, int also = -1);
bool mf_solve_tests_inertia(const Ctx &C);
void launch_inertia(Ctx &C);
void launch_acopf_eval_point(Ctx &C, int inst, const double *x_dev, double sigma, const double *lam_dev,
                             double *f_dev, double *grad_dev, double *g_dev, double *jcoo_dev,
                             double *hcoo_dev);
void sqp_reset(Ctx &C);
void sqp_run(Ctx &C, int max_outer);
void merit_eval(Ctx &C, int op, double a0, double a1, int flag, double *out_host);
void merit_eval_batch(Ctx &C, int count, const int *inst_dev, int op, const double *a0_dev, const double *a1_dev, int flag,
                      double *out_dev);
void armijo_eval(Ctx &C, int inst, double mu, double phi0, double D, double eta, double tau, double min_alpha, int fr,
                 double *out3_host);

}

struct sqphip_ctx { sqphip::Ctx c; };
```

sqpsolver.jl_amd/csrc/mfplan.hip:

```cpp
#include "sparse.hpp"
#include "../../include/sqphip.h"
#include "../../include/sqphip_test_hooks.h"
#include <algorithm>
#include <cmath>
#include <cstdio>
#include <cstdlib>
#include <tuple>

namespace sqphip {

MfPlan mf_build_plan(int n, int m, const std::vector<int> &kpos, int mk, const std::vector<int> &hcolptr,
                     const std::vector<int> &hrowval, const std::vector<int> &jrowptr, const std::vector<int> &jrcol,
                     const std::vector<int> &jrslot, const SymOptions &opt)
{
    MfPlan P;
    std::vector<std::vector<int>> adj, before;
    kkt_graph(n, m, kpos, mk, hcolptr, hrowval, jrowptr, jrcol, adj, before);
    P.S = sparse_symbolic(n + mk, adj, before, opt);
    const SparseSym &S = P.S;
    P.off.resize(S.ns);
    for (int s = 0; s < S.ns; ++s) {
        const long fs = S.sn_nc[s] + S.sn_nr[s];
        P.off[s] = P.stride;
        P.stride += ((fs + 1) * fs + 1) / 2 * 2;
    }
    struct Rec { int sn, loc, seq; MfItem it; };
    std::vector<Rec> recs;
    auto add = [&](int ua, int ub, MfItem it) {
        int pa = S.pos[ua], pb = S.pos[ub];
        if (pa < pb) std::swap(pa, pb);
        const int s = S.col2sn[pb], f = S.sn_first[s], nc = S.sn_nc[s], fs = nc + S.sn_nr[s];
        int li;
        if (pa < f + nc) li = pa - f;
        else {
            const int *R = S.sn_rows.data() + S.sn_rowptr[s];
            const int *q = std::lower_bound(R, R + S.sn_nr[s], pa);
            if (q == R + S.sn_nr[s] || *q != pa) { fprintf(stderr, "sqphip: mf_build_plan: entry outside its front\n"); abort(); }
            li = nc + (int)(q - R);
        }
        recs.push_back({s, (pb - f) * (fs + 1) + li, (int)recs.size(), it});
    };
    for (int j = 0; j < n; ++j) {
        add(j, j, {MF_ITEM_VDIAG, -1, j, 0});
        for (int k = hcolptr[j]; k < hcolptr[j + 1]; ++k) {
            const int i = hrowval[k];
            if (i >= j) add(i, j, {MF_ITEM_H, -1, k, 0});
        }
    }
    for (int i = 0; i < m; ++i) {
        const int s = jrowptr[i], e = jrowptr[i + 1];
        if (kpos[i] >= 0) {
            add(n + kpos[i], n + kpos[i], {MF_ITEM_RDIAG, i, 0, 0});
            for (int t = s; t < e; ++t) add(n + kpos[i], jrcol[t], {MF_ITEM_JKEPT, i, jrslot[t], 0});
        } else {
            for (int a = s; a < e; ++a)
                for (int b = s; b <= a; ++b) add(jrcol[a], jrcol[b], {MF_ITEM_PAIR, i, jrslot[a], jrslot[b]});
        }
    }
    std::sort(recs.begin(), recs.end(), [](const Rec &x, const Rec &y) {
        return std::tie(x.sn, x.loc, x.seq) < std::tie(y.sn, y.loc, y.seq); });
    P.asm_ptr.assign(S.ns + 1, 0);
    for (size_t r = 0; r < recs.size(); ++r) {
        const bool fresh = r == 0 || recs[r].sn != recs[r - 1].sn || recs[r].loc != recs[r - 1].loc;
        if (fresh) {
            P.dest_loc.push_back(recs[r].loc);
            P.item_ptr.push_back((int)P.items.size());
            P.asm_ptr[recs[r].sn + 1]++;
        }
        P.items.push_back(recs[r].it);
    }
    P.item_ptr.push_back((int)P.items.size());
    for (int s = 0; s < S.ns; ++s) P.asm_ptr[s + 1] += P.asm_ptr[s];
    P.nnzK = (long)P.dest_loc.size();
    P.dest_rc.resize(P.dest_loc.size());
    for (int s = 0; s < S.ns; ++s) {
        const int ld = S.sn_nc[s] + S.sn_nr[s] + 1;
        for (int e = P.asm_ptr[s]; e < P.asm_ptr[s + 1]; ++e) P.dest_rc[e] = (P.dest_loc[e] % ld) | ((P.dest_loc[e] / ld) << 16);
    }
    if (P.stride >= (1L << 31)) { fprintf(stderr, "sqphip: mf_build_plan: front arena too large for 32-bit offsets\n"); abort(); }
    const bool big_solve = !(getenv("SQPHIP_MF_BIG_SOLVE") && atoi(getenv("SQPHIP_MF_BIG_SOLVE")) == 0);
    P.top_level = S.nlevels;
    if (big_solve && !(getenv("SQPHIP_MF_TOP") && atoi(getenv("SQPHIP_MF_TOP")) == 0)) {
        auto joins = [&](int lev) {
            const int cnt = S.level_ptr[lev + 1] - S.level_ptr[lev];
            if (cnt <= 2) return true;
            if (cnt > 4 || getenv("SQPHIP_MF_TOP_NARROW")) return false;
            for (int q = S.level_ptr[lev]; q < S.level_ptr[lev + 1]; ++q)
                if (S.sn_nc[S.level_sn[q]] + S.sn_nr[S.level_sn[q]] > 64) return false;
            return true;
        };
        int l = S.nlevels;
        while (l > 0 && joins(l - 1)) --l;
        if (S.nlevels - l >= 2) P.top_level = l;
    }
    P.spine_level = P.top_level; P.narrow_level = P.top_level;
    auto children_of = [&](int s) {
        std::vector<int> ch(S.child.begin() + S.child_ptr[s], S.child.begin() + S.child_ptr[s + 1]);
        std::stable_sort(ch.begin(), ch.end(), [&](int a, int b) { return (S.sn_level[a] >= P.spine_level) < (S.sn_level[b] >= P.spine_level); });
        return ch;
    };
    P.ea_ptr.assign(S.ns + 1, 0);
    P.ea_src_ptr.push_back(0);
    {
        std::vector<std::tuple<int, int, int>> con;
        for (int s = 0; s < S.ns; ++s) {
            const int fs = S.sn_nc[s] + S.sn_nr[s];
            con.clear();
            for (int c : children_of(s)) {
                const int cnc = S.sn_nc[c], cnr = S.sn_nr[c], cld = cnc + cnr + 1;
                const int *rel = S.rel.data() + S.sn_rowptr[c];
                for (int jj = 0; jj < cnr; ++jj)
                    for (int ii = jj; ii <= cnr; ++ii)
                        con.emplace_back(rel[jj], ii < cnr ? rel[ii] : fs, (int)(P.off[c] + (long)(cnc + jj) * cld + cnc + ii));
            }
            std::stable_sort(con.begin(), con.end(), [](const std::tuple<int, int, int> &a, const std::tuple<int, int, int> &b) {
                return std::tie(std::get<0>(a), std::get<1>(a)) < std::tie(std::get<0>(b), std::get<1>(b)); });
            for (size_t r = 0; r < con.size(); ++r) {
                const bool fresh = r == 0 || std::get<0>(con[r]) != std::get<0>(con[r - 1]) || std::get<1>(con[r]) != std::get<1>(con[r - 1]);
                if (fresh) {
                    if (r) P.ea_src_ptr.push_back((int)P.ea_src.size());
                    P.ea_rc.push_back(std::get<1>(con[r]) | (std::get<0>(con[r]) << 16));
                    P.ea_ptr[s + 1]++;
                }
                P.ea_src.push_back(std::get<2>(con[r]));
            }
            if (!con.empty()) P.ea_src_ptr.push_back((int)P.ea_src.size());
        }
        for (int s = 0; s < S.ns; ++s) P.ea_ptr[s + 1] += P.ea_ptr[s];
    }
    P.ev_ptr.assign(S.ns + 1, 0);
    P.ev_src_ptr.push_back(0);
    {
        std::vector<std::pair<int, int>> con;
        for (int s = 0; s < S.ns; ++s) {
            con.clear();
            for (int q = S.child_ptr[s]; q < S.child_ptr[s + 1]; ++q) {
                const int c = S.child[q], cnc = S.sn_nc[c], cnr = S.sn_nr[c], cfs = cnc + cnr, cld = cfs + 1;
                const int *rel = S.rel.data() + S.sn_rowptr[c];
                for (int jj = 0; jj < cnr; ++jj) con.emplace_back(rel[jj], (int)(P.off[c] + (long)(cnc + jj) * cld + cfs));
            }
            std::stable_sort(con.begin(), con.end(), [](const std::pair<int, int> &a, const std::pair<int, int> &b) { return a.first < b.first; });
            for (size_t r = 0; r < con.size(); ++r) {
                if (r == 0 || con[r].first != con[r - 1].first) {
                    if (r) P.ev_src_ptr.push_back((int)P.ev_src.size());
                    P.ev_idx.push_back(con[r].first);
                    P.ev_ptr[s + 1]++;
                }
                P.ev_src.push_back(con[r].second);
            }
            if (!con.empty()) P.ev_src_ptr.push_back((int)P.ev_src.size());
        }
        for (int s = 0; s < S.ns; ++s) P.ev_ptr[s + 1] += P.ev_ptr[s];
    }
    auto tiles = [&](int s) { return (S.sn_nc[s] + S.sn_nr[s] + 1 + 15) / 16; };
    auto cls = [&](int s) { const int T = tiles(s); return T <= 2 ? 1 : (T <= 6 ? T - 1 : (T <= 8 ? 7 : (T <= 13 ? 8 : 9))); };
    for (int l = 0; l < S.nlevels; ++l) {
        int cnt = 0, tmax = 0;
        for (int q = S.level_ptr[l]; q < S.level_ptr[l + 1]; ++q) { ++cnt; tmax = std::max(tmax, tiles(S.level_sn[q])); }
        const int merge_t = getenv("SQPHIP_MF_MERGE_T") ? atoi(getenv("SQPHIP_MF_MERGE_T")) : opt.merge_tiles;
        const bool merge = ((cnt <= 8 && tmax <= 8) || tmax <= merge_t) && !getenv("SQPHIP_MF_NO_LEVEL_MERGE");
        for (int c = 0; c < 10; ++c) {
            MfLaunch L{(int)P.sched.size(), 0, 0, 0, c, 0};
            L.level = l;
            for (int q = S.level_ptr[l]; q < S.level_ptr[l + 1]; ++q) {
                const int s = S.level_sn[q];
                if (merge ? c != tmax - 1 : cls(s) != c) continue;
                P.sched.push_back(s);
                L.count++;
                L.tiles = std::max(L.tiles, tiles(s));
            }
            if (!L.count) continue;
            if (!merge && c == 1) L.tiles = 2;
            if (!merge && c == 7) L.tiles = 8;
            P.fac.push_back(L);
        }
    }
    auto build_solve_launches = [&]() {
    P.sol_items.clear(); P.fwd.clear(); P.bwd.clear(); P.top = MfLaunch{0, 0, 256, 0, 0, 0};
    int top_maxfs = 64, top_lcap = 0;
    for (int l = 0; l < S.nlevels; ++l) {
        const bool top = l >= P.top_level;
        MfLaunch L{(int)P.sol_items.size() / 4, 0, 256, 0, 0, 0};
        int maxfs = 64, lcap = 0;
        std::vector<int> small;
        for (int q = S.level_ptr[l]; q < S.level_ptr[l + 1]; ++q) {
            const int s = S.level_sn[q], fs = S.sn_nc[s] + S.sn_nr[s];
            if (!big_solve) maxfs = std::max(maxfs, fs);
            if (fs > 64 && big_solve) {
                for (int t : {s, -2, -2, -2}) P.sol_items.push_back(t);
                maxfs = std::max(maxfs, fs);
                const int nc = S.sn_nc[s];
                if (nc <= 80) lcap = std::max(lcap, nc * nc);
            } else small.push_back(s);
        }
        for (size_t q = 0; q < small.size(); q += 4)
            for (size_t t = q; t < q + 4; ++t) P.sol_items.push_back(t < small.size() ? small[t] : -1);
        L.count = (int)P.sol_items.size() / 4 - L.begin;
        L.tiles = big_solve ? 64 : maxfs;
        L.cls = std::max(4 * L.tiles, maxfs + 16);
        L.lds_bytes = 8 * (L.cls + lcap);
        {
            int wimg = 0; long bigimg = 0; bool ok2 = big_solve;
            for (int q = S.level_ptr[l]; q < S.level_ptr[l + 1]; ++q) {
                const int s = S.level_sn[q], nc = S.sn_nc[s], fs = nc + S.sn_nr[s];
                if (fs > 128 || nc > 112) { ok2 = false; break; }
                if (fs > 64) bigimg = std::max(bigimg, (long)nc * (fs | 1)); else wimg = std::max(wimg, nc * (fs | 1));
            }
            const long lds2 = 8 * std::max(4L * (64 + wimg), 128 + bigimg);
            if (ok2 && lds2 <= 150 * 1024) { L.wimg = wimg; L.lds2 = (int)lds2; L.hasbig = bigimg > 0 ? 1 : 0; }
        }
        if (!top) { P.fwd.push_back(L); continue; }
        if (l == P.top_level) P.top.begin = L.begin;
        P.top.count += L.count;
        top_maxfs = std::max(top_maxfs, maxfs); top_lcap = std::max(top_lcap, lcap);
    }
    if (P.top.count) {
        P.top.tiles = 64;
        P.top.cls = std::max(4 * 64, top_maxfs + 16);
        P.top.lds_bytes = 8 * (P.top.cls + top_lcap);
    }
    P.bwd.assign(P.fwd.rbegin(), P.fwd.rend());
    };
    build_solve_launches();
    if (P.top.count > 0 && !(getenv("SQPHIP_MF_TOP2") && atoi(getenv("SQPHIP_MF_TOP2")) == 0)) {
        std::vector<int> kof(S.ns, -1);
        bool ok = true;
// ... 200 lines not shown
                        err = std::max(err, std::fabs(img[c * Rn + r] - A[c * ld + r]));
                        scale = std::max(scale, std::fabs(A[c * ld + r]));
                    }
                g_spine_err = std::max(g_spine_err, err / std::max(scale, 1e-300));
            }
        }
        for (int k = 0; k < nc; ++k) {
            const double d = A[k * ld + k], di = 1.0 / d;
            dinv[f0 + k] = di;
            for (int j = k + 1; j < fs; ++j) {
                const double lj = A[k * ld + j] * di;
                for (int i = j; i <= fs; ++i) A[j * ld + i] -= A[k * ld + i] * lj;
            }
            for (int i = k + 1; i <= fs; ++i) A[k * ld + i] *= di;
            v[f0 + k] = A[k * ld + fs];
        }
    }
    g_top2_err = -1.0;
    std::vector<double> xtop, ytop;
    if (P.top2_lds_bytes > 0) {
        const int n_ext = (int)P.top_ext.size();
        std::vector<double> uvec(n_ext + P.top_utotal, 0.0), y;
        xtop.assign(P.top_xtotal, 0.0); ytop.assign(P.top_xtotal, 0.0);
        for (int t = 0; t < n_ext; ++t) uvec[t] = F[P.top_ext[t]];
        double err = 0.0, scale = 0.0;
        for (const MfTopFront &T : P.top_fr) {
            const int nc = T.nc, fs = T.nc + T.nr, ld = fs + 1;
            const double *A = F.data() + T.off;
            y.assign(fs, 0.0);
            for (int i = 0; i < fs; ++i) {
                if (i < nc) y[i] = x[T.first + i];
                for (int q = P.top_gptr[T.gptr + i]; q < P.top_gptr[T.gptr + i + 1]; ++q) y[i] += uvec[P.top_gsrc[T.gsrc0 + q]];
            }
            for (int k = 0; k < nc; ++k)
                for (int i = k + 1; i < fs; ++i) y[i] -= A[k * ld + i] * y[k];
            for (int i = 0; i < nc; ++i) {
                ytop[T.xloc + i] = y[i] * dinv[T.first + i];
                err = std::max(err, std::fabs(ytop[T.xloc + i] - v[T.first + i])); scale = std::max(scale, std::fabs(v[T.first + i]));
            }
            for (int i = nc; i < fs; ++i) uvec[n_ext + T.uoff + i - nc] = y[i];
        }
        g_top2_err = err / std::max(scale, 1e-300);
    }
    for (int s = S.ns - 1; s >= 0; --s) {
        const int nc = S.sn_nc[s], nr = S.sn_nr[s], fs = nc + nr, ld = fs + 1, f0 = S.sn_first[s];
        const double *A = F.data() + P.off[s];
        const int *R = S.sn_rows.data() + S.sn_rowptr[s];
        for (int k = nc - 1; k >= 0; --k) {
            double a = v[f0 + k];
            for (int i = k + 1; i < nc; ++i) a -= A[k * ld + i] * x[f0 + i];
            for (int r = 0; r < nr; ++r) a -= A[k * ld + nc + r] * x[R[r]];
            x[f0 + k] = a;
        }
    }
    if (P.top2_lds_bytes > 0) {
        double err = 0.0, scale = 0.0;
        std::vector<double> t;
        for (int k = (int)P.top_fr.size() - 1; k >= 0; --k) {
            const MfTopFront &T = P.top_fr[k];
            const int nc = T.nc, nr = T.nr, fs = nc + nr, ld = fs + 1;
            const double *A = F.data() + T.off;
            t.assign(nc, 0.0);
            for (int c = 0; c < nc; ++c) {
                t[c] = ytop[T.xloc + c];
                for (int r = 0; r < nr; ++r) t[c] -= A[c * ld + nc + r] * xtop[P.top_rows[T.rloc + r]];
            }
            for (int i = nc - 1; i >= 1; --i)
                for (int c = 0; c < i; ++c) t[c] -= A[c * ld + i] * t[i];
            for (int c = 0; c < nc; ++c) {
                xtop[T.xloc + c] = t[c];
                err = std::max(err, std::fabs(t[c] - x[T.first + c])); scale = std::max(scale, std::fabs(x[T.first + c]));
            }
        }
        g_top2_err = std::max(g_top2_err, err / std::max(scale, 1e-300));
    }
    for (int u = 0; u < S.nu; ++u) sol[u] = x[S.pos[u]];
}

}

extern "C" double sqphip_mf_host_top2_err(void) { return sqphip::g_top2_err; }
extern "C" double sqphip_mf_host_spine_err(void) { return sqphip::g_spine_err; }

namespace {

sqphip::MfPlan host_plan(int64_t n, int64_t m, int64_t nnzJ, const int64_t *jrow, const int64_t *jcol, int64_t nnzH,
                         const int64_t *hrow, const int64_t *hcol, const double *gL, const double *gU, int32_t condense,
                         const sqphip::SymOptions &so, const double *Jval, const double *Hval, std::vector<double> &jv,
                         std::vector<double> &hv)
{
    using namespace sqphip;
    struct Ent { int c, r; double v; };
    auto build = [](int64_t ncols, int64_t nnz, const int64_t *row, const int64_t *col, const double *val, bool sym,
                    std::vector<int> &colptr, std::vector<int> &rowval, std::vector<double> &vals) {
        std::vector<Ent> e;
        for (int64_t k = 0; k < nnz; ++k) {
            e.push_back({(int)col[k] - 1, (int)row[k] - 1, val ? val[k] : 0.0});
            if (sym && row[k] != col[k]) e.push_back({(int)row[k] - 1, (int)col[k] - 1, val ? val[k] : 0.0});
        }
        std::stable_sort(e.begin(), e.end(), [](const Ent &a, const Ent &b) { return std::tie(a.c, a.r) < std::tie(b.c, b.r); });
        colptr.assign(ncols + 1, 0);
        for (size_t i = 0; i < e.size(); ++i) {
            if (i && e[i].c == e[i - 1].c && e[i].r == e[i - 1].r) { vals.back() += e[i].v; continue; }
            rowval.push_back(e[i].r); vals.push_back(e[i].v); colptr[e[i].c + 1]++;
        }
        for (int64_t j = 0; j < ncols; ++j) colptr[j + 1] += colptr[j];
    };
    std::vector<int> jcp, jrv, hcp, hrv;
    build(n, nnzJ, jrow, jcol, Jval, false, jcp, jrv, jv);
    build(n, nnzH, hrow, hcol, Hval, true, hcp, hrv, hv);
    std::vector<int> rptr(m + 1, 0), rcol(jrv.size()), rslot(jrv.size());
    for (int r : jrv) rptr[r + 1]++;
    for (int64_t i = 0; i < m; ++i) rptr[i + 1] += rptr[i];
    {
        std::vector<int> fill(rptr.begin(), rptr.end() - 1);
        for (int j = 0; j < (int)n; ++j)
            for (int s = jcp[j]; s < jcp[j + 1]; ++s) { const int i = jrv[s]; rcol[fill[i]] = j; rslot[fill[i]] = s; fill[i]++; }
    }
    std::vector<int> kpos(m > 0 ? m : 1, -1);
    int mk = 0;
    for (int64_t i = 0; i < m; ++i)
        if (!condense || kkt_row_is_kept(gL[i], gU[i], rptr[i + 1] - rptr[i])) kpos[i] = mk++;
    return mf_build_plan((int)n, (int)m, kpos, mk, hcp, hrv, rptr, rcol, rslot, so);
}

}

extern "C" int sqphip_mf_host_solve(int64_t n, int64_t m, int64_t nnzJ, const int64_t *jrow, const int64_t *jcol,
                                    int64_t nnzH, const int64_t *hrow, const int64_t *hcol, const double *gL,
                                    const double *gU, int32_t condense, const double *Jval, const double *Hval,
                                    const double *Dd, const double *sigp, const double *hd, const int32_t *rtype,
                                    double hsc, double dw, const double *rhs, double *sol, double *dinv_by_unknown,
                                    int32_t *npos)
{
    if (n <= 0 || m < 0 || !rhs || !sol) return SQPHIP_EINVAL;
    using namespace sqphip;
    std::vector<double> jv, hv;
    MfPlan P = host_plan(n, m, nnzJ, jrow, jcol, nnzH, hrow, hcol, gL, gU, condense, SymOptions(), Jval, Hval, jv, hv);
    std::vector<int> rt(m > 0 ? m : 1, 1);
    for (int64_t i = 0; i < m; ++i) rt[i] = rtype ? rtype[i] : 1;
    MfValues V{hv.data(), jv.data(), Dd, sigp, hd, rt.data(), hsc, dw};
    std::vector<double> dinv(P.S.nu);
    mf_host_factor_solve(P, V, rhs, sol, dinv.data());
    int np = 0;
    for (int u = 0; u < P.S.nu; ++u) {
        const double d = dinv[P.S.pos[u]];
        if (dinv_by_unknown) dinv_by_unknown[u] = d;
        if (d > 0.0 && std::isfinite(d)) ++np;
    }
    if (npos) *npos = np;
    return SQPHIP_OK;
}

extern "C" int sqphip_mf_plan_info(int64_t n, int64_t m, int64_t nnzJ, const int64_t *jrow, const int64_t *jcol, int64_t nnzH,
                                   const int64_t *hrow, const int64_t *hcol, const double *gL, const double *gU,
                                   int32_t condense, int32_t batch, int32_t *fronts, int32_t cap_fronts, int32_t *n_fronts,
                                   int32_t *launches, int32_t cap_launches, int32_t *n_launches, int64_t *top2_lds_bytes,
                                   int32_t *spine_fronts)
{
    if (n <= 0 || m < 0 || batch <= 0 || cap_fronts < 0 || cap_launches < 0 || (cap_fronts > 0 && !fronts) ||
        (cap_launches > 0 && !launches))
        return SQPHIP_EINVAL;
    using namespace sqphip;
    const SymOptions so = mf_sym_options(batch);
    std::vector<double> jv, hv;
    const MfPlan P = host_plan(n, m, nnzJ, jrow, jcol, nnzH, hrow, hcol, gL, gU, condense, so, nullptr, nullptr, jv, hv);
    const SparseSym &S = P.S;
    std::vector<int> level(S.ns, 0);
    for (int l = 0; l < S.nlevels; ++l)
        for (int q = S.level_ptr[l]; q < S.level_ptr[l + 1]; ++q) level[S.level_sn[q]] = l;
    for (int f = 0; f < S.ns && f < cap_fronts; ++f) { fronts[3 * f] = S.sn_nc[f]; fronts[3 * f + 1] = S.sn_nr[f]; fronts[3 * f + 2] = level[f]; }
    for (int k = 0; k < (int)P.fac.size() && k < cap_launches; ++k) {
        const MfLaunch &L = P.fac[k];
        int tmin = 1 << 30;
        for (int q = L.begin; q < L.begin + L.count; ++q) tmin = std::min(tmin, (S.sn_nc[P.sched[q]] + S.sn_nr[P.sched[q]] + 1 + 15) / 16);
        launches[4 * k] = L.level; launches[4 * k + 1] = L.tiles; launches[4 * k + 2] = L.count; launches[4 * k + 3] = tmin;
    }
    if (n_fronts) *n_fronts = S.ns;
    if (n_launches) *n_launches = (int32_t)P.fac.size();
    if (top2_lds_bytes) *top2_lds_bytes = P.top2_lds_bytes;
    if (spine_fronts) *spine_fronts = (int32_t)P.sp_fr.size();
    return SQPHIP_OK;
}
```

sqpsolver.jl_amd/csrc/mfront.hip:

```cpp
#include "ctx.hpp"
#include "dev_util.hpp"
#include "mf_dev.hpp"
#include <cstdlib>
#include <mutex>

namespace sqphip {

#ifdef SQPHIP_MF_TRACE
__device__ long long g_mf_trace[1 << 16][8];
#define MF_TR(i) if (inst == 0 && threadIdx.x == 0 && s < (1 << 16)) g_mf_trace[s][i] = (long long)wall_clock64();
__device__ long long g_mf_trace2[1 << 12][16];
#define MF_TRW(i) if (W == 0 && trs >= 0 && trs < (1 << 12) && lane == 0) g_mf_trace2[trs][i] = (long long)clock64();
__device__ long long g_mf_trace3[1 << 12][16];
#define MF_TRS(i) if (inst == 0 && tid == 0 && s < (1 << 12)) g_mf_trace3[s][i] = (long long)clock64();
#define MF_TR2S(a, b) if (inst == 0 && lane == 0 && j < 64 && wave < 2) g_mf_trace3[(do_fwd ? 64 : 0) + j][wave == 0 ? (a) : (b)] = (long long)clock64();
#define MF_TR2W(c) if (trj >= 0 && lane == 0) g_mf_trace3[trj][c] = (long long)clock64();
#define MF_TRSP(c) if (inst == 0 && cand == 0 && tid == 0 && k < 64) g_mf_trace3[128 + k][c] = (long long)wall_clock64();
#else
#define MF_TR(i)
#define MF_TRW(i)
#define MF_TRS(i)
#define MF_TR2S(a, b)
#define MF_TR2W(c)
#define MF_TRSP(c)
#endif

template <int NT, bool INPLACE>
__global__ __launch_bounds__(NT) void k_mf_factor(DV d, int sbegin, int want, int with_rhs)
{
    int inst, cand;
    if (!mf_candidate(d, want, inst, cand)) return;
    const MfDev &M = d.mf;
    const int s = M.sched[sbegin + blockIdx.x];
    const MfFrontDesc Fd = M.desc[s];
    const int nc = Fd.nc, nr = Fd.nr, fs = nc + nr, ld = fs + 1, f0 = Fd.first;
    double *G = mf_arena(d, inst, cand) + Fd.off;
    extern __shared__ double mf_lds[];
    double *F = INPLACE ? G : mf_lds;
    const int tid = threadIdx.x;
    const int rl_log = ld <= 16 ? 4 : (ld <= 32 ? 5 : 6);
    const int RL = 1 << rl_log, rlane = tid & (RL - 1), cg = tid >> rl_log, ncg = NT >> rl_log;
    MF_TR(0)
    for (int e = tid; e < ld * fs; e += NT) F[e] = 0.0;
    __syncthreads();
    MF_TR(1)
    {
        const IpmState &st = d.ist[inst];
        const double hsc = st.hsc, dw = cand ? next_shift(st.dw, st.dw_last) : st.dw;
        const double *hv = d.hv + (long)inst * d.nnzhc, *jv = d.jv + (long)inst * d.nnzjc;
        const double *Dd = d.Dd + (long)inst * d.m, *sigp = d.sigp + (long)inst * d.n, *hd = d.hd + (long)inst * d.n;
        const int *rt = d.rtype + (long)inst * d.m;
        for (int e = Fd.asm_begin + tid; e < Fd.asm_end; e += NT) {
            double a = 0.0;
            for (int k = M.item_ptr[e]; k < M.item_ptr[e + 1]; ++k) a += mf_item_value(M.items[k], hv, jv, Dd, sigp, hd, rt, hsc, dw);
            F[M.dest_loc[e]] = a;
        }
        if (with_rhs) {
            const double *b = d.xv + (long)inst * d.Fpad + f0;
            for (int j = tid; j < nc; j += NT) F[j * ld + fs] = b[j];
        }
    }
    __syncthreads();
    MF_TR(2)
    for (int q = M.child_ptr[s]; q < M.child_ptr[s + 1]; ++q) {
        const int c = M.child[q];
        const int cnc = M.nc[c], cnr = M.nr[c], cld = cnc + cnr + 1;
        const double *Cg = mf_arena(d, inst, cand) + M.off[c] + (long)cnc * cld + cnc;
        const int *rel = M.rel + M.rowptr[c];
        for (int jj = cg; jj < cnr; jj += ncg) {
            const int gj = rel[jj] * ld;
            const double *Cc = Cg + (long)jj * cld;
            for (int ii = jj + rlane; ii <= cnr; ii += RL) F[gj + (ii < cnr ? rel[ii] : fs)] += Cc[ii];
        }
        __syncthreads();
    }
    MF_TR(3)
    for (int k = 0; k < nc; ++k) {
        const double *Fk = F + k * ld;
        const double di = 1.0 / Fk[k];
        for (int j = k + 1 + cg; j < fs; j += ncg) {
            const double lj = Fk[j] * di;
            double *Fj = F + j * ld;
            for (int i = j + rlane; i <= fs; i += RL) Fj[i] -= Fk[i] * lj;
        }
        __syncthreads();
    }
    MF_TR(4)
    double *dinv = mf_dinv(d, inst, cand) + f0, *vv = mf_vv(d, inst, cand) + f0;
    for (int j = cg; j < fs; j += ncg) {
        const double *Fj = F + j * ld;
        double *Gj = G + (long)j * ld;
        if (j < nc) {
            const double di = 1.0 / Fj[j];
            for (int i = j + 1 + rlane; i < fs; i += RL) Gj[i] = Fj[i] * di;
            if (rlane == 0) { dinv[j] = di; if (with_rhs) vv[j] = Fj[fs] * di; }
        } else if (!INPLACE) {
            for (int i = j + rlane; i <= fs; i += RL) Gj[i] = Fj[i];
        }
    }
    MF_TR(5)
}

#ifdef SQPHIP_MF_TRACE
extern "C" int sqphip_mf_trace_read(long long *out, int nfronts)
{
    return (int)hipMemcpyFromSymbol(out, HIP_SYMBOL(g_mf_trace), sizeof(long long) * 8 * (size_t)nfronts);
}
extern "C" int sqphip_mf_trace3_read(long long *out, int nfronts)
{
    return (int)hipMemcpyFromSymbol(out, HIP_SYMBOL(g_mf_trace3), sizeof(long long) * 16 * (size_t)nfronts);
}
extern "C" int sqphip_mf_trace2_read(long long *out, int nfronts)
{
    return (int)hipMemcpyFromSymbol(out, HIP_SYMBOL(g_mf_trace2), sizeof(long long) * 16 * (size_t)nfronts);
}
#endif

__global__ __launch_bounds__(256) void k_mf_values(DV d, int want)
{
    int inst, cand;
    if (!mf_candidate(d, want, inst, cand)) return;
    const MfDev &M = d.mf;
    const int e = blockIdx.x * 256 + threadIdx.x;
    if (e >= M.nnzK) return;
    const IpmState &st = d.ist[inst];
    const double dw = cand ? next_shift(st.dw, st.dw_last) : st.dw;
    const double *hv = d.hv + (long)inst * d.nnzhc, *jv = d.jv + (long)inst * d.nnzjc;
    const double *Dd = d.Dd + (long)inst * d.m, *sigp = d.sigp + (long)inst * d.n, *hd = d.hd + (long)inst * d.n;
    const int *rt = d.rtype + (long)inst * d.m;
    double a = 0.0;
    for (int k = M.item_ptr[e]; k < M.item_ptr[e + 1]; ++k) a += mf_item_value(M.items[k], hv, jv, Dd, sigp, hd, rt, st.hsc, dw);
    mf_vals(d, inst, cand)[e] = a;
}

typedef double d4 __attribute__((ext_vector_type(4)));

#ifndef SQPHIP_MF_RCP_NR
#define SQPHIP_MF_RCP_NR 2
#endif
#ifndef SQPHIP_MF_LDL4_FAST
#define SQPHIP_MF_LDL4_FAST 0
#endif
__device__ __forceinline__ double mf_rcp(double x)
{
    double r = __builtin_amdgcn_rcp(x);
    r = fma(fma(-x, r, 1.0), r, r);
#if SQPHIP_MF_RCP_NR >= 2
    r = fma(fma(-x, r, 1.0), r, r);
#endif
    return r;
}

__device__ __forceinline__ double mf_readlane(double x, int lane)
{
    const int lo = __builtin_amdgcn_readlane(__double2loint(x), lane), hi = __builtin_amdgcn_readlane(__double2hiint(x), lane);
    return __hiloint2double(hi, lo);
}

#ifndef SQPHIP_MF_SHFL
#define SQPHIP_MF_SHFL 0
#endif
#ifndef SQPHIP_MF_EARLY_STORE
#define SQPHIP_MF_EARLY_STORE 1
#endif
struct MfRows { double r0, r1, r2; };
__device__ __forceinline__ double mf_hilo(unsigned hi, unsigned lo) { return __hiloint2double((int)hi, (int)lo); }
__device__ __forceinline__ MfRows mf_rows3(double x, int l15)
{
#if SQPHIP_MF_SHFL
    return {__shfl(x, l15), __shfl(x, l15 + 16), __shfl(x, l15 + 32)};
#else
    (void)l15;
    const unsigned lo = (unsigned)__double2loint(x), hi = (unsigned)__double2hiint(x);
    const auto pl = __builtin_amdgcn_permlane16_swap(lo, lo, false, false), ph = __builtin_amdgcn_permlane16_swap(hi, hi, false, false);
    const auto al = __builtin_amdgcn_permlane32_swap(pl[0], pl[0], false, false), ah = __builtin_amdgcn_permlane32_swap(ph[0], ph[0], false, false);
    const auto bl = __builtin_amdgcn_permlane32_swap(pl[1], pl[1], false, false), bh = __builtin_amdgcn_permlane32_swap(ph[1], ph[1], false, false);
    return {mf_hilo(ah[0], al[0]), mf_hilo(bh[0], bl[0]), mf_hilo(ah[1], al[1])};
#endif
}

template <int NW, int MAXT, bool LDSIMG>
__global__ __launch_bounds__(64 * NW) void k_mf_factor2(DV d, int sbegin, int want, int with_rhs, int Tl)
{
    constexpr int NT = 64 * NW;
    int inst, cand;
    if (!mf_candidate(d, want, inst, cand)) return;
    const MfDev &M = d.mf;
    const int s = M.sched[sbegin + blockIdx.x];
    const MfFrontDesc Fd = M.desc[s];
    const int nc = Fd.nc, nr = Fd.nr, fs = nc + nr, ld = fs + 1, f0 = Fd.first;
    const double *arena = mf_arena(d, inst, cand);
    double *G = mf_arena(d, inst, cand) + Fd.off;
    extern __shared__ double mf_lds[];
    const int R = 16 * Tl;
    double *Xp = mf_lds + (LDSIMG ? R * R : 0), *Lp = Xp + 4 * R, *blk = Lp + 4 * R, *dl = blk + 16;
    double *F = LDSIMG ? mf_lds : G;
    const int LD = LDSIMG ? R : ld;
    const int tid = threadIdx.x, lane = tid & 63, l15 = lane & 15, l4 = lane >> 4;
    const int wave = __builtin_amdgcn_readfirstlane(tid >> 6);
    const int T = (ld + 15) >> 4;
    MF_TR(0)
    if (LDSIMG) {
        if (T == Tl) for (int e = tid; e < R * R; e += NT) F[e] = 0.0;
        else for (int e = tid; e < 256 * T * T; e += NT) F[(e / (16 * T)) * LD + e % (16 * T)] = 0.0;
    } else for (int e = tid; e < ld * fs; e += NT) F[e] = 0.0;
    __syncthreads();
    MF_TR(1)
    {
        const double *vals = mf_vals(d, inst, cand);
        for (int e = Fd.asm_begin + tid; e < Fd.asm_end; e += NT) {
            const int rc = M.dest_rc[e];
            F[(rc >> 16) * LD + (rc & 0xffff)] = vals[e];
        }
        if (with_rhs) {
            const double *b = d.xv + (long)inst * d.Fpad + f0;
            for (int j = tid; j < nc; j += NT) F[j * LD + fs] = b[j];
        }
    }
    __syncthreads();
    MF_TR(2)
    for (int t = Fd.ea_begin + tid; t < Fd.ea_end; t += NT) {
        const MfGather g = M.ea_ent[t];
        double a = arena[g.src0];
        for (int q = g.src_begin + 1; q < g.src_end; ++q) a += arena[M.ea_src[q]];
        const int rc = g.where;
        F[(rc >> 16) * LD + (rc & 0xffff)] += a;
    }
    __syncthreads();
    MF_TR(3)
    int ti_[MAXT], tj_[MAXT];
    d4 acc[MAXT];
#pragma unroll
    for (int q = 0; q < MAXT; ++q) {
        int rem = q * NW + wave, tj = 0;
        while (tj < T && rem >= T - tj) { rem -= T - tj; ++tj; }
        const bool valid = tj < T;
        const int ti = tj + rem;
        ti_[q] = valid ? ti : -1; tj_[q] = tj;
#pragma unroll
        for (int rr = 0; rr < 4; ++rr) {
            const int col = 16 * tj + l4 + 4 * rr, row = 16 * ti + l15;
            const bool in = valid && (LDSIMG || (row <= fs && col < fs));
            acc[q][rr] = in ? F[col * LD + row] : 0.0;
        }
    }
    __syncthreads();
    for (int tk = 0; 16 * tk < nc; ++tk) {
#pragma unroll
        for (int rr0 = 0; rr0 < 4; ++rr0) {
            const int k0 = 16 * tk + 4 * rr0;
            if (k0 >= nc) break;
            const int bw = nc - k0 < 4 ? nc - k0 : 4;
            double a00, a10, a11, a20, a21, a22, a30, a31, a32, a33;
            if (NW == 1) {
                double dv = 0.0;
#pragma unroll
                for (int q = 0; q < MAXT; ++q) if (ti_[q] == tk && tj_[q] == tk) dv = acc[q][rr0];
                const int b0 = 4 * rr0;
                a00 = mf_readlane(dv, b0);
                a10 = mf_readlane(dv, b0 + 1); a11 = mf_readlane(dv, b0 + 1 + 16);
                a20 = mf_readlane(dv, b0 + 2); a21 = mf_readlane(dv, b0 + 2 + 16); a22 = mf_readlane(dv, b0 + 2 + 32);
                a30 = mf_readlane(dv, b0 + 3); a31 = mf_readlane(dv, b0 + 3 + 16); a32 = mf_readlane(dv, b0 + 3 + 32);
                a33 = mf_readlane(dv, b0 + 3 + 48);
            } else {
#pragma unroll
                for (int q = 0; q < MAXT; ++q)
                    if (ti_[q] == tk && tj_[q] == tk) {
                        const int a = l15 - 4 * rr0;
                        if (a >= 0 && a < 4) blk[a * 4 + l4] = acc[q][rr0];
                    }
                __syncthreads();
                a00 = blk[0]; a10 = blk[4]; a11 = blk[5]; a20 = blk[8]; a21 = blk[9]; a22 = blk[10]; a30 = blk[12]; a31 = blk[13];
                a32 = blk[14]; a33 = blk[15];
            }
            double i1 = 0.0, i2 = 0.0, i3 = 0.0, l21 = 0.0, l31 = 0.0, l32 = 0.0;
            const double i0 = mf_rcp(a00);
            const double l10 = a10 * i0, l20 = a20 * i0, l30 = a30 * i0;
            a11 -= l10 * a10; a21 -= l10 * a20; a22 -= l20 * a20; a31 -= l10 * a30; a32 -= l20 * a30; a33 -= l30 * a30;
            if (bw > 1) { i1 = mf_rcp(a11); l21 = a21 * i1; l31 = a31 * i1; a22 -= l21 * a21; a32 -= l21 * a31; a33 -= l31 * a31; }
            if (bw > 2) { i2 = mf_rcp(a22); l32 = a32 * i2; a33 -= l32 * a32; }
            if (bw > 3) i3 = mf_rcp(a33);
            const double lc0 = l4 == 1 ? l10 : (l4 == 2 ? l20 : (l4 == 3 ? l30 : 0.0));
            const double lc1 = l4 == 2 ? l21 : (l4 == 3 ? l31 : 0.0);
            const double lc2 = l4 == 3 ? l32 : 0.0;
            const double ic = l4 == 0 ? i0 : (l4 == 1 ? i1 : (l4 == 2 ? i2 : i3));
#pragma unroll
            for (int q = 0; q < MAXT; ++q)
                if (tj_[q] == tk && ti_[q] >= 0) {
                    double x = acc[q][rr0];
                    x -= __shfl(x, l15) * lc0;
                    x -= __shfl(x, l15 + 16) * lc1;
                    x -= __shfl(x, l15 + 32) * lc2;
                    acc[q][rr0] = x;
                    const int row = 16 * ti_[q] + l15;
                    Xp[l4 * R + row] = x;
                    Lp[l4 * R + row] = row >= k0 + 4 ? x * ic : 0.0;
                }
            if (tid < bw) dl[k0 + tid] = tid == 0 ? i0 : (tid == 1 ? i1 : (tid == 2 ? i2 : i3));
            __syncthreads();
#pragma unroll
            for (int q = 0; q < MAXT; ++q)
                if (ti_[q] >= 0 && tj_[q] >= tk) {
                    const double b = Xp[l4 * R + 16 * ti_[q] + l15];
                    const double a = -Lp[l4 * R + 16 * tj_[q] + l15];
                    acc[q] = __builtin_amdgcn_mfma_f64_16x16x4f64(a, b, acc[q], 0, 0, 0);
                }
        }
    }
    __syncthreads();
    MF_TR(4)
    double *dinv = mf_dinv(d, inst, cand) + f0, *vv = mf_vv(d, inst, cand) + f0;
#pragma unroll
    for (int q = 0; q < MAXT; ++q) {
        if (ti_[q] < 0) continue;
#pragma unroll
        for (int rr = 0; rr < 4; ++rr) {
            const int col = 16 * tj_[q] + l4 + 4 * rr, row = 16 * ti_[q] + l15;
            const double v = acc[q][rr];
            if (col < nc) {
                if (row > col && row < fs) G[(long)col * ld + row] = v * dl[col];
                else if (row == fs && with_rhs) vv[col] = v * dl[col];
            } else if (col < fs && row >= col && row <= fs) G[(long)col * ld + row] = v;
        }
    }
    for (int k = tid; k < nc; k += NT) dinv[k] = dl[k];
    MF_TR(5)
}

struct MfBlk4 { double i0, i1, i2, i3, m10, m20, m21, m30, m31, m32; };

__device__ __forceinline__ MfBlk4 mf_ldl4(double a00, double a10, double a11, double a20, double a21, double a22, double a30,
                                           double a31, double a32, double a33, int bw)
{
    double i1 = 0.0, i2 = 0.0, i3 = 0.0, l21 = 0.0, l31 = 0.0, l32 = 0.0;
    const double i0 = mf_rcp(a00);
    const double l10 = a10 * i0, l20 = a20 * i0, l30 = a30 * i0;
#if SQPHIP_MF_LDL4_FAST
    {
        const double p11 = a10 * a10, p21 = a10 * a20, p22 = a20 * a20, p31 = a10 * a30, p32 = a20 * a30, p33 = a30 * a30;
        a11 = fma(-p11, i0, a11); a21 = fma(-p21, i0, a21); a22 = fma(-p22, i0, a22); a31 = fma(-p31, i0, a31); a32 = fma(-p32, i0, a32); a33 = fma(-p33, i0, a33);
    }
    if (bw > 1) {
        i1 = mf_rcp(a11); l21 = a21 * i1; l31 = a31 * i1;
        const double q22 = a21 * a21, q32 = a21 * a31, q33 = a31 * a31;
        a22 = fma(-q22, i1, a22); a32 = fma(-q32, i1, a32); a33 = fma(-q33, i1, a33);
    }
    if (bw > 2) { i2 = mf_rcp(a22); l32 = a32 * i2; a33 = fma(-(a32 * a32), i2, a33); }
#else
    a11 -= l10 * a10; a21 -= l10 * a20; a22 -= l20 * a20; a31 -= l10 * a30; a32 -= l20 * a30; a33 -= l30 * a30;
    if (bw > 1) { i1 = mf_rcp(a11); l21 = a21 * i1; l31 = a31 * i1; a22 -= l21 * a21; a32 -= l21 * a31; a33 -= l31 * a31; }
    if (bw > 2) { i2 = mf_rcp(a22); l32 = a32 * i2; a33 -= l32 * a32; }
#endif
    if (bw > 3) i3 = mf_rcp(a33);
    MfBlk4 B;
    B.i0 = i0; B.i1 = i1; B.i2 = i2; B.i3 = i3;
    B.m10 = -l10; B.m21 = -l21; B.m32 = -l32;
    B.m20 = -(l20 + l21 * B.m10);
    B.m31 = -(l31 + l32 * B.m21);
    B.m30 = -(l30 + l31 * B.m10 + l32 * B.m20);
    return B;
}

struct MfLaneSel { double s0, s1, s2, s3; };
__device__ __forceinline__ MfLaneSel mf_lane_sel(int l4)
{
    return {l4 == 0 ? 1.0 : 0.0, l4 == 1 ? 1.0 : 0.0, l4 == 2 ? 1.0 : 0.0, l4 == 3 ? 1.0 : 0.0};
}
__device__ __forceinline__ double mf_sel_ic(const MfLaneSel &S, const MfBlk4 &B)
{
    return fma(S.s3, B.i3, fma(S.s2, B.i2, fma(S.s1, B.i1, S.s0 * B.i0)));
}
__device__ __forceinline__ double mf_apply4(double x, int l15, const MfLaneSel &S, const MfBlk4 &B)
{
    const MfRows V = mf_rows3(x, l15);
    const double v0 = V.r0, v1 = V.r1, v2 = V.r2;
    const double c0 = fma(S.s3, B.m30, fma(S.s2, B.m20, S.s1 * B.m10));
    const double c1 = fma(S.s3, B.m31, S.s2 * B.m21);
    const double c2 = S.s3 * B.m32;
    return fma(c2, v2, fma(c1, v1, fma(c0, v0, x)));
}

__device__ __forceinline__ void wave_sync_lds()
{
    __builtin_amdgcn_fence(__ATOMIC_ACQ_REL, "wavefront");
    __builtin_amdgcn_wave_barrier();
}

__host__ __device__ constexpr int mf_front_lds_doubles(int T, int NW, bool ldsimg)
{
    const int R = 16 * T, u = (ldsimg ? R * R : 0) > 16 * R ? R * R : 16 * R;
    return u + 256 + 40 + R + 64 * NW;
}

template <int T, int NW, int W> struct MfTileSet {
    static constexpr int NROWS = W < T ? (T - W + NW - 1) / NW : 0;
    static constexpr int NTILES = NROWS > 0 ? NROWS * (2 * W + (NROWS - 1) * NW + 2) / 2 : 1;
// ... 1186 lines not shown
    for (int cb = lw; cb < nc; cb += CH * NLW) {
        double v0[CH], v1[CH];
#pragma unroll
        for (int q = 0; q < CH; ++q) {
            const int c = cb + q * NLW;
            v0[q] = 0.0; v1[q] = 0.0;
            if (c < nc) { v0[q] = G[(unsigned)(c * ld) + (unsigned)r0]; if constexpr (TWO) v1[q] = G[(unsigned)(c * ld) + (unsigned)r1]; }
        }
#pragma unroll
        for (int q = 0; q < CH; ++q) {
            const int c = cb + q * NLW;
            if (c < nc) { Bf[c * ll + r0] = r0 > c ? v0[q] : 0.0; if constexpr (TWO) Bf[c * ll + r1] = r1 > c ? v1[q] : 0.0; }
        }
    }
}

template <bool HASBIG>
__global__ __launch_bounds__(256, HASBIG ? 4 : 6) void k_mf_fwd2(DV d, int ibegin, int want, int wimg)
{
    const int inst = blockIdx.y;
    if (d.phase[inst] != want) return;
    extern __shared__ double mf_lds[];
    const MfDev &M = d.mf;
    const int4 it = reinterpret_cast<const int4 *>(M.sol_items)[ibegin + blockIdx.x];
    const int tid = threadIdx.x, lane = tid & 63, wave = __builtin_amdgcn_readfirstlane(tid >> 6);
    const bool big = HASBIG && it.y == -2;
    const int s = big ? it.x : (wave == 0 ? it.x : (wave == 1 ? it.y : (wave == 2 ? it.z : it.w)));
    if (s < 0) return;
    const MfFrontDesc Fd = M.desc[s];
    const int nc = Fd.nc, nr = Fd.nr, fs = nc + nr, ld = fs + 1, f0 = Fd.first, ll = fs | 1;
    const int cand = d.ist[inst].sel;
    const double *arena = mf_arena(d, inst, cand);
    double *G = mf_arena(d, inst, cand) + Fd.off;
    const double *b = d.xv + (long)inst * d.Fpad + f0, *dinv = mf_dinv(d, inst, cand) + f0;
    double *vv = mf_vv(d, inst, cand) + f0;
    double *y = big ? mf_lds : mf_lds + wave * (64 + wimg), *Bf = y + (big ? 128 : 64);
    const int i0 = lane, i1 = lane + 64;
    if (!big || wave == 0) {
        const int t0 = Fd.ev_begin + i0, t1 = Fd.ev_begin + i1;
        MfGather g0{0, 0, 0, 0}, g1{0, 0, 0, 0};
        const bool h0 = t0 < Fd.ev_end, h1 = big && t1 < Fd.ev_end;
        if (h0) g0 = M.ev_ent[t0];
        if (h1) g1 = M.ev_ent[t1];
        const double b0 = i0 < nc ? b[i0] : 0.0, b1 = (big && i1 < nc) ? b[i1] : 0.0;
        const double d0 = i0 < nc ? dinv[i0] : 0.0, d1 = (big && i1 < nc) ? dinv[i1] : 0.0;
        if (!big) mf_img_load<1, 24, false>(G, ld, nc, fs, Bf, ll, 0, lane);
        else mf_img_load<4, 14, true>(G, ld, nc, fs, Bf, ll, 0, lane);
        if (i0 < fs) y[i0] = b0;
        if (big && i1 < fs) y[i1] = b1;
        wave_sync();
        if (h0) { double a = arena[g0.src0]; for (int q = g0.src_begin + 1; q < g0.src_end; ++q) a += arena[M.ev_src[q]]; y[g0.where] += a; }
        wave_sync();
        if (h1) { double a = arena[g1.src0]; for (int q = g1.src_begin + 1; q < g1.src_end; ++q) a += arena[M.ev_src[q]]; y[g1.where] += a; }
        wave_sync();
        double y0 = i0 < fs ? y[i0] : 0.0, y1 = (big && i1 < fs) ? y[i1] : 0.0;
        if (big) __syncthreads();
        if (!big) { wave_sync(); mf_chain_fwd<false>(Bf, ll, nc, fs, lane, y0, y1); }
        else mf_chain_fwd<true>(Bf, ll, nc, fs, lane, y0, y1);
        if (i0 < nc) vv[i0] = y0 * d0; else if (i0 < fs) G[(long)i0 * ld + fs] = y0;
        if (big) { if (i1 < nc) vv[i1] = y1 * d1; else if (i1 < fs) G[(long)i1 * ld + fs] = y1; }
    } else {
        mf_img_load<4, 14, true>(G, ld, nc, fs, Bf, ll, wave, lane);
        __syncthreads();
    }
}

template <bool HASBIG>
__global__ __launch_bounds__(256, HASBIG ? 4 : 5) void k_mf_bwd2(DV d, int ibegin, int want, int wimg, int also)
{
    const int inst = blockIdx.y;
    const int ph = d.phase[inst];
    if (ph != want && ph != also) return;
    extern __shared__ double mf_lds[];
    const MfDev &M = d.mf;
    const int4 it = reinterpret_cast<const int4 *>(M.sol_items)[ibegin + blockIdx.x];
    const int tid = threadIdx.x, lane = tid & 63, wave = __builtin_amdgcn_readfirstlane(tid >> 6);
    const bool big = HASBIG && it.y == -2;
    const int s = big ? it.x : (wave == 0 ? it.x : (wave == 1 ? it.y : (wave == 2 ? it.z : it.w)));
    if (s < 0) return;
    const MfFrontDesc Fd = M.desc[s];
    const int nc = Fd.nc, nr = Fd.nr, fs = nc + nr, ld = fs + 1, f0 = Fd.first, ll = fs | 1;
    const int cand = d.ist[inst].sel;
    const double *G = mf_arena(d, inst, cand) + Fd.off;
    double *xg = d.xv + (long)inst * d.Fpad;
    const double *vv = mf_vv(d, inst, cand) + f0;
    const int *rows = M.rows + Fd.rowptr;
    double *Bf = (big ? mf_lds : mf_lds + wave * (64 + wimg)) + (big ? 128 : 64);
    const int i0 = lane, i1 = lane + 64;
    if (!big || wave == 0) {
        const int q0 = i0 < nr ? rows[i0] : -1, q1 = (big && i1 < nr) ? rows[i1] : -1;
        double t0 = i0 < nc ? vv[i0] : 0.0, t1 = (big && i1 < nc) ? vv[i1] : 0.0;
        if (!big) mf_img_load<1, 24, false>(G, ld, nc, fs, Bf, ll, 0, lane);
        else mf_img_load<4, 14, true>(G, ld, nc, fs, Bf, ll, 0, lane);
        const double xr0 = q0 >= 0 ? xg[q0] : 0.0, xr1 = q1 >= 0 ? xg[q1] : 0.0;
        if (big) __syncthreads(); else wave_sync();
        if (nc <= 64) mf_chain_bwd<false>(Bf, ll, nc, nr, lane, xr0, xr1, t0, t1);
        else mf_chain_bwd<true>(Bf, ll, nc, nr, lane, xr0, xr1, t0, t1);
        if (i0 < nc) xg[f0 + i0] = t0;
        if (big && i1 < nc) xg[f0 + i1] = t1;
    } else {
        mf_img_load<4, 14, true>(G, ld, nc, fs, Bf, ll, wave, lane);
        __syncthreads();
    }
}

const char *const mf_kernel_names[] = {
    "k_mf_values", "k_mf_factor<256, true>", "k_mf_factor2<1, 3, true>", "k_mf_factor2<2, 5, true>", "k_mf_factor2<4, 4, true>",
    "k_mf_factor2<4, 9, false>", "k_mf_factor2<8, 12, false>",
    "k_mf_front<1, 1, true>", "k_mf_front<2, 1, true>", "k_mf_front<3, 1, true>", "k_mf_front<4, 2, true>", "k_mf_front<4, 4, true>",
    "k_mf_front<5, 2, true>", "k_mf_front<5, 4, true>",
    "k_mf_front<6, 4, false>", "k_mf_front<6, 4, true>", "k_mf_front<6, 8, true>",
    "k_mf_front<7, 4, false>", "k_mf_front<7, 4, true>", "k_mf_front<7, 8, true>",
    "k_mf_front<8, 4, false>", "k_mf_front<8, 4, true>", "k_mf_front<8, 8, true>",
    "k_mf_front<9, 8, false>", "k_mf_front<10, 8, false>", "k_mf_front<11, 8, false>", "k_mf_front<12, 8, false>",
    "k_mf_spine", "k_mf_solve_inst<16>", "k_mf_fwd", "k_mf_fwd2<false>", "k_mf_fwd2<true>", "k_mf_solve_top", "k_mf_solve_top2",
    "k_mf_bwd", "k_mf_bwd2<false>", "k_mf_bwd2<true>", "k_inertia" };
static_assert(sizeof(mf_kernel_names) / sizeof(mf_kernel_names[0]) == MFK_COUNT, "a name per MfKernel entry");
static constexpr int mf_front_kid(int T, int NW, bool IMG)
{
    return T >= 1 && T <= 3 ? (NW == 1 && IMG ? MFK_FRONT_1 + T - 1 : -1)
         : T <= 5 ? ((NW == 2 || NW == 4) && IMG ? MFK_FRONT_4_2 + 2 * (T - 4) + (NW == 4) : -1)
         : T <= 8 ? (NW == 4 ? MFK_FRONT_6_4 + 3 * (T - 6) + (IMG ? 1 : 0) : NW == 8 && IMG ? MFK_FRONT_6_4 + 3 * (T - 6) + 2 : -1)
         : T <= 12 ? (NW == 8 && !IMG ? MFK_FRONT_9 + T - 9 : -1) : -1;
}
static constexpr int mf_factor2_kid(int NW, int MAXT, bool IMG)
{
    return NW == 1 && MAXT == 3 && IMG ? MFK_F2_1_3 : NW == 2 && MAXT == 5 && IMG ? MFK_F2_2_5 : NW == 4 && MAXT == 4 && IMG ? MFK_F2_4_4
         : NW == 4 && MAXT == 9 && !IMG ? MFK_F2_4_9 : NW == 8 && MAXT == 12 && !IMG ? MFK_F2_8_12 : -1;
}

static int mf_generic_solves()
{
    static const int g = getenv("SQPHIP_MF_GENERIC") ? atoi(getenv("SQPHIP_MF_GENERIC")) : 0;
    return g;
}

void mf_device_setup(Ctx &C)
{
    static std::mutex mu;
    std::lock_guard<std::mutex> lk(mu);
    bool ok = true;
    auto big = [&](const void *f) { ok &= hipFuncSetAttribute(f, hipFuncAttributeMaxDynamicSharedMemorySize, 160 * 1024) == hipSuccess; };
    big(reinterpret_cast<const void *>(k_mf_front<6, 4, true>)); big(reinterpret_cast<const void *>(k_mf_front<7, 4, true>));
    big(reinterpret_cast<const void *>(k_mf_front<8, 4, true>)); big(reinterpret_cast<const void *>(k_mf_front<6, 8, true>));
    big(reinterpret_cast<const void *>(k_mf_front<7, 8, true>)); big(reinterpret_cast<const void *>(k_mf_front<8, 8, true>));
    big(reinterpret_cast<const void *>(k_mf_fwd2<true>)); big(reinterpret_cast<const void *>(k_mf_bwd2<true>));
    big(reinterpret_cast<const void *>(k_mf_fwd2<false>)); big(reinterpret_cast<const void *>(k_mf_bwd2<false>));
    big(reinterpret_cast<const void *>(k_mf_solve_top2));
    big(reinterpret_cast<const void *>(k_mf_spine));
    (void)hipGetLastError();
    C.mf_big_lds = ok;
}

void mf_factor(Ctx &C, int want, bool with_rhs, bool values_done)
{
    const DV &d = C.d;
    hipStream_t s = C.stream;
    static const bool v1 = getenv("SQPHIP_MF_V1") != nullptr;
    const int wr = (int)with_rhs;
    const int nb = d.mf.fronts1 && d.spec_mode != 0 ? 2 * d.B : d.B;
    if (!v1 && !values_done) { C.tm.open(s); C.mf_census[MFK_VALUES]++; hipLaunchKernelGGL(k_mf_values, dim3((d.mf.nnzK + 255) / 256, nb), dim3(256), 0, s, d, want); C.tm.close(KC_VALUES, s); }
    const bool stat = !(getenv("SQPHIP_MF_STATIC") && atoi(getenv("SQPHIP_MF_STATIC")) == 0);
    const bool spine = !v1 && d.mf.sp_n > 0 && C.mf_big_lds;
    int li = 0, cls_open = -1;
    for (const MfLaunch &L : C.mfp().fac) {
        if (spine && li++ >= C.mfp().fac_below) break;
        const int cls = L.level >= C.mfp().narrow_level ? KC_FRONTS_TOP : KC_FRONTS_LOW;
        if (cls != cls_open) { if (cls_open >= 0) C.tm.close(cls_open, s); C.tm.open(s); cls_open = cls; }
        const dim3 grid(L.count, nb);
        const int T = L.tiles, R = 16 * T;
        if (v1 || T > 13) { C.mf_census[MFK_FACTOR_R1]++; hipLaunchKernelGGL((k_mf_factor<256, true>), grid, dim3(256), 0, s, d, L.begin, want, wr); continue; }
#define MF_GENERIC(NW, MAXT, IMG) do { constexpr int kid_ = mf_factor2_kid(NW, MAXT, IMG); static_assert(kid_ >= 0, "census: no counter"); C.mf_census[kid_]++; hipLaunchKernelGGL((k_mf_factor2<NW, MAXT, IMG>), grid, dim3(64 * NW), 8 * (size_t)((IMG ? R * R : 0) + 9 * R + 16), s, d, L.begin, want, wr, T); } while (0)
#define MF_STATIC(TT, NW, IMG) do { constexpr int kid_ = mf_front_kid(TT, NW, IMG); static_assert(kid_ >= 0, "census: no counter"); C.mf_census[kid_]++; hipLaunchKernelGGL((k_mf_front<TT, NW, IMG>), grid, dim3(64 * NW), 8 * (size_t)mf_front_lds_doubles(TT, NW, IMG), s, d, L.begin, want, wr); } while (0)
        const int stat_min = getenv("SQPHIP_MF_STATIC_MIN") ? atoi(getenv("SQPHIP_MF_STATIC_MIN")) : (L.count <= 8 && L.level >= C.mfp().narrow_level ? 1 : 4);
        const bool nw8 = !(getenv("SQPHIP_MF_NW8") && atoi(getenv("SQPHIP_MF_NW8")) == 0);
        const int nw4 = L.count <= 8 ? (getenv("SQPHIP_MF_NW4") ? atoi(getenv("SQPHIP_MF_NW4")) : 3) : 0;
        const bool big_img = C.mf_big_lds && !(getenv("SQPHIP_MF_BIG_LDSIMG") && atoi(getenv("SQPHIP_MF_BIG_LDSIMG")) == 0);
        static const int stat_max = getenv("SQPHIP_MF_STATIC_MAX") ? atoi(getenv("SQPHIP_MF_STATIC_MAX")) : 12;
        if (!stat || T > stat_max || T > 12 || T < stat_min) {
            if (T <= 2) MF_GENERIC(1, 3, true);
            else if (T <= 4) MF_GENERIC(2, 5, true);
            else if (T <= 5) MF_GENERIC(4, 4, true);
            else if (T <= 8) MF_GENERIC(4, 9, false);
            else MF_GENERIC(8, 12, false);
            continue;
        }
        switch (T) {
        case 1: MF_STATIC(1, 1, true); break;
        case 2: MF_STATIC(2, 1, true); break;
        case 3: MF_STATIC(3, 1, true); break;
        case 4: if (nw4 & 1) MF_STATIC(4, 4, true); else MF_STATIC(4, 2, true); break;
        case 5: if (nw4 & 2) MF_STATIC(5, 4, true); else MF_STATIC(5, 2, true); break;
        case 6: if (big_img && L.count <= 8) { if (nw8) MF_STATIC(6, 8, true); else MF_STATIC(6, 4, true); } else MF_STATIC(6, 4, false); break;
        case 7: if (big_img && L.count <= 8) { if (nw8) MF_STATIC(7, 8, true); else MF_STATIC(7, 4, true); } else MF_STATIC(7, 4, false); break;
        case 8: if (big_img && L.count <= 8) { if (nw8) MF_STATIC(8, 8, true); else MF_STATIC(8, 4, true); } else MF_STATIC(8, 4, false); break;
        case 9: MF_STATIC(9, 8, false); break;
        case 10: MF_STATIC(10, 8, false); break;
        case 11: MF_STATIC(11, 8, false); break;
        default: MF_STATIC(12, 8, false); break;
        }
#undef MF_GENERIC
#undef MF_STATIC
    }
    if (cls_open >= 0) C.tm.close(cls_open, s);
    if (spine) { C.tm.open(s); C.mf_census[MFK_SPINE]++; hipLaunchKernelGGL(k_mf_spine, dim3(1, nb), dim3(MF_SP_NT), (size_t)C.mfp().spine_lds_bytes, s, d, want, wr); C.tm.close(KC_FRONTS_TOP, s); }
    C.mf_factor_launches += spine ? (long)C.mfp().fac_below + 1 : (long)C.mfp().fac.size();
}

bool mf_solve_tests_inertia(const Ctx &C)
{
    static const bool off = getenv("SQPHIP_MF_INERTIA_KERNEL") != nullptr;
    return !off && C.d.sparse && C.d.mf.top_n > 0 && !mf_generic_solves() && !(C.d.B >= (getenv("SQPHIP_MF_INST_SOLVE_MIN") ? atoi(getenv("SQPHIP_MF_INST_SOLVE_MIN")) : (1 << 30)));
}

void mf_solve(Ctx &C, int want, bool skip_fwd, bool inertia, int also)
{
    const DV &d = C.d;
    hipStream_t s = C.stream;
    const int generic = mf_generic_solves();
    static const int inst_min = getenv("SQPHIP_MF_INST_SOLVE_MIN") ? atoi(getenv("SQPHIP_MF_INST_SOLVE_MIN")) : (1 << 30);
    if (d.B >= inst_min && d.mf.max_front * 8 * 16 <= 64 * 1024) {
        C.mf_census[MFK_SOLVE_INST]++;
        hipLaunchKernelGGL(k_mf_solve_inst<16>, dim3(d.B), dim3(1024), (size_t)d.mf.max_front * 8 * 16, s, d, want, skip_fwd ? 0 : 1, generic);
        return;
    }
    const bool lvl2 = !(getenv("SQPHIP_MF_LEVEL2") && atoi(getenv("SQPHIP_MF_LEVEL2")) == 0);
    if (!C.mf_big_lds) throw std::string("sqphip: the solve kernels could not be granted 160 KB of dynamic LDS on this device (mf_device_setup)");
    if (also >= 0 && !(skip_fwd && d.mf.top_n > 0 && !generic && d.B < inst_min)) throw std::string("sqphip: mf_solve: a second phase needs the streamed top behind a fused forward pass");
    const int fwant = also >= 0 ? also : want;
    const bool run_fwd = !skip_fwd || also >= 0;
    if (run_fwd && !C.mfp().fwd.empty()) C.tm.open(s);
    if (run_fwd)
        for (const MfLaunch &L : C.mfp().fwd) {
            C.mf_census[lvl2 && !generic && L.wimg >= 0 ? (L.hasbig ? MFK_FWD2_BIG : MFK_FWD2) : MFK_FWD]++;
            if (lvl2 && !generic && L.wimg >= 0) {
                if (L.hasbig) hipLaunchKernelGGL(k_mf_fwd2<true>, dim3(L.count, d.B), dim3(256), L.lds2, s, d, L.begin, fwant, L.wimg);
                else hipLaunchKernelGGL(k_mf_fwd2<false>, dim3(L.count, d.B), dim3(256), L.lds2, s, d, L.begin, fwant, L.wimg);
            }
            else hipLaunchKernelGGL(k_mf_fwd, dim3(L.count, d.B), dim3(256), L.lds_bytes, s, d, L.begin, fwant, generic, L.tiles, L.cls, L.lds_bytes / 8 - L.cls);
        }
    if (run_fwd && !C.mfp().fwd.empty()) C.tm.close(KC_SOLVE_LEVELS, s);
    const bool has_top = (d.mf.top_n > 0 && !generic) || C.mfp().top.count > 0;
    if (has_top) C.tm.open(s);
    if (d.mf.top_n > 0 && !generic) {
        const size_t lds = (size_t)C.mfp().top2_lds_bytes;
        C.mf_census[MFK_SOLVE_TOP2]++;
        hipLaunchKernelGGL(k_mf_solve_top2, dim3(d.B), dim3(256), lds, s, d, want, skip_fwd ? 0 : 1, inertia ? 1 : 0, also);
    } else if (const MfLaunch &T = C.mfp().top; T.count > 0) {
        C.mf_census[MFK_SOLVE_TOP]++;
        hipLaunchKernelGGL(k_mf_solve_top, dim3(d.B), dim3(256), T.lds_bytes, s, d, T.begin, T.count, want, skip_fwd ? 0 : 1, generic,
                           T.tiles, T.cls, T.lds_bytes / 8 - T.cls);
    }
    if (has_top) C.tm.close(KC_SOLVE_TOP, s);
    if (!C.mfp().bwd.empty()) C.tm.open(s);
    for (const MfLaunch &L : C.mfp().bwd) {
        C.mf_census[lvl2 && !generic && L.wimg >= 0 ? (L.hasbig ? MFK_BWD2_BIG : MFK_BWD2) : MFK_BWD]++;
        if (lvl2 && !generic && L.wimg >= 0) {
            if (L.hasbig) hipLaunchKernelGGL(k_mf_bwd2<true>, dim3(L.count, d.B), dim3(256), L.lds2, s, d, L.begin, want, L.wimg, also);
            else hipLaunchKernelGGL(k_mf_bwd2<false>, dim3(L.count, d.B), dim3(256), L.lds2, s, d, L.begin, want, L.wimg, also);
        }
        else hipLaunchKernelGGL(k_mf_bwd, dim3(L.count, d.B), dim3(256), L.lds_bytes, s, d, L.begin, want, generic, L.tiles, L.cls, L.lds_bytes / 8 - L.cls, also);
    }
    if (!C.mfp().bwd.empty()) C.tm.close(KC_SOLVE_LEVELS, s);
}

}
```

sqpsolver.jl_amd/csrc/sparse.hpp:

```cpp
#pragma once
#include <cstdint>
#include <cstdlib>
#include <vector>

namespace sqphip {

struct SparseSym {
    int nu = 0;
    std::vector<int> pos, inv;
    int ns = 0;
    std::vector<int> sn_first, sn_nc, sn_nr, sn_rowptr, sn_rows, sn_parent, sn_level;
    std::vector<int> col2sn;
    std::vector<int> rel;
    std::vector<int> child_ptr, child;
    std::vector<long> front_off;
    long front_total = 0;
    int nlevels = 0;
    std::vector<int> level_ptr, level_sn;
    long nnzL = 0;
    long nnzL_exact = 0;
    double flops = 0;
    double flops_exact = 0;
    int max_front = 0, max_nc = 0;
};

constexpr int KKT_LONG_ROW = 32;
inline bool kkt_row_is_kept(double gl, double gu, int row_nnz) { return gl == gu || row_nnz > KKT_LONG_ROW; }

struct SymOptions {
    int rows_after_vars = 1;
    int small_front = 32;
    double zero_frac = 0.25;
    int order_method = 0;
    int merge_tiles = 0;
    int chain_front = 0;
};
inline SymOptions mf_sym_options(int B)
{
    SymOptions so;
    if (const char *e = getenv("SQPHIP_MF_SMALL_FRONT")) so.small_front = atoi(e);
    if (const char *e = getenv("SQPHIP_MF_ZERO_FRAC")) so.zero_frac = atof(e);
    if (const char *e = getenv("SQPHIP_MF_ROWS_AFTER")) so.rows_after_vars = atoi(e);
    so.merge_tiles = B <= 64 ? 4 : 0;
    return so;
}

SparseSym sparse_symbolic(int nu, const std::vector<std::vector<int>> &adj, const std::vector<std::vector<int>> &before,
                          const SymOptions &opt);

void kkt_graph(int n, int m, const std::vector<int> &kpos, int mk, const std::vector<int> &hcolptr,
               const std::vector<int> &hrowval, const std::vector<int> &jrowptr, const std::vector<int> &jrcol,
               std::vector<std::vector<int>> &adj, std::vector<std::vector<int>> &before);

enum { MF_ITEM_H = 0,
       MF_ITEM_JKEPT = 1,
       MF_ITEM_PAIR = 2,
       MF_ITEM_VDIAG = 3,
       MF_ITEM_RDIAG = 4 };
struct MfItem { int type, row, a, b; };

struct MfFrontDesc { int nc, nr, first, rowptr, off, asm_begin, asm_end, ea_begin, ea_end, ev_begin, ev_end, pad; };
struct MfGather { int where, src_begin, src_end, src0; };

struct MfLaunch { int begin, count, threads, lds_bytes, cls, tiles; int wimg = -1, lds2 = 0, hasbig = 1; int level = 0; };

struct MfTopFront { int s, nc, nr, first, off, ll, xloc, uoff, gptr, gsrc0, nsrc, rloc, lbuf, pad0, pad1, pad2; };

struct MfSpineFront { int s, nc, nr, first, off, T, asm_begin, asm_end, ea_begin, ea_end, handoff, rel, pad0, pad1, pad2, pad3; };

struct MfPlan {
    SparseSym S;
    std::vector<long> off;
    long stride = 0;
    std::vector<int> asm_ptr, dest_loc, item_ptr;
    std::vector<MfItem> items;
    std::vector<int> dest_rc;
    std::vector<int> ea_ptr, ea_rc, ea_src_ptr, ea_src;
    std::vector<int> ev_ptr, ev_idx, ev_src_ptr, ev_src;
    std::vector<int> sol_items;
    std::vector<MfFrontDesc> desc;
    std::vector<MfGather> ea_ent, ev_ent;
    std::vector<int> sched;
    std::vector<MfLaunch> fac, fwd, bwd;
    MfLaunch top{0, 0, 256, 0, 0, 0};
    int top_level = 0;
    std::vector<MfTopFront> top_fr;
    std::vector<int> top_gptr, top_gsrc, top_rows, top_ext;
    int top_xtotal = 0, top_utotal = 0, top_buf0 = 0, top_buf1 = 0;
    long top2_lds_bytes = 0;
    long nnzK = 0;
    int spine_level = 0, spine_T = 0;
    int narrow_level = 0;
    std::vector<MfSpineFront> sp_fr;
    std::vector<MfGather> sp_ent;
    std::vector<int> sp_src, sp_rel;
    long spine_lds_bytes = 0;
    int spine_stage = 0;
    int fac_below = 0;
};

MfPlan mf_build_plan(int n, int m, const std::vector<int> &kpos, int mk, const std::vector<int> &hcolptr,
                     const std::vector<int> &hrowval, const std::vector<int> &jrowptr, const std::vector<int> &jrcol,
                     const std::vector<int> &jrslot, const SymOptions &opt);

struct MfValues { const double *hv, *jv, *Dd, *sigp, *hd; const int *rtype; double hsc, dw; };
void mf_host_factor_solve(const MfPlan &P, const MfValues &V, const double *rhs, double *sol, double *dinv);

}
```

sqpsolver.jl_amd/host.py:

```python
from __future__ import annotations

import ctypes as C
import dataclasses
import math
import numpy as np

from . import _lib

MODE_QP, MODE_FR, MODE_SOC, MODE_LP, MODE_L1QP, MODE_INFEAS = range(6)
LOCALLY_SOLVED, LOCALLY_INFEASIBLE, ITERATION_LIMIT, NUMERICAL_ERROR = 4, 5, 11, 20
_OK = (1, 7, 10, 4)
_INFEAS = (2, 5)

_dp = C.POINTER(C.c_double)


def _d(a):
    return None if a is None else a.ctypes.data_as(_dp)


def _f(a):
    return None if a is None else np.ascontiguousarray(a, dtype=np.float64)


def _l(a):
    return a.ctypes.data_as(C.POINTER(C.c_int64))


def _i(a):
    return a.ctypes.data_as(C.POINTER(C.c_int32))


class SqpHipError(RuntimeError):
    pass


def default_options(**kw) -> _lib.Options:
    o = _lib.Options()
    _lib.lib().sqphip_default_options(C.byref(o))
    for k, v in kw.items():
        if not hasattr(o, k):
            raise KeyError(k)
        setattr(o, k, v)
    return o


def kkt_order(n, m, jrow, jcol, hrow, hcol, gL, gU, rows_last=True):
    L = _lib.lib()
    jr, jc, hr, hc = (np.ascontiguousarray(a, dtype=np.int64) for a in (jrow, jcol, hrow, hcol))
    mk = int(np.sum((np.asarray(gL) == np.asarray(gU)) | (np.bincount(jr - 1, minlength=m) > 32)))
    pos = np.zeros(n + mk, dtype=np.int32); ts = C.c_int32(); nf = C.c_int32()
    rc = L.sqphip_kkt_order(n, m, len(jr), jr.ctypes.data_as(C.POINTER(C.c_int64)), jc.ctypes.data_as(C.POINTER(C.c_int64)),
                            len(hr), hr.ctypes.data_as(C.POINTER(C.c_int64)), hc.ctypes.data_as(C.POINTER(C.c_int64)),
                            _d(_f(gL)), _d(_f(gU)), int(rows_last), pos.ctypes.data_as(C.POINTER(C.c_int32)), C.byref(ts), C.byref(nf))
    if rc != 0:
        raise SqpHipError(f"sqphip_kkt_order failed ({rc})")
    return pos, ts.value, nf.value


def kkt_symbolic(n, m, jrow, jcol, hrow, hcol, gL, gU, condense=True, rows_after_vars=True, small_front=0,
                 zero_frac=-1.0):
    L = _lib.lib()
    jr, jc, hr, hc = (np.ascontiguousarray(a, dtype=np.int64) for a in (jrow, jcol, hrow, hcol))
    pos = np.zeros(n + m, dtype=np.int32); st = _lib.SymbolicStats()
    rc = L.sqphip_kkt_symbolic(n, m, len(jr), _l(jr), _l(jc), len(hr), _l(hr), _l(hc), _d(_f(gL)), _d(_f(gU)),
                               int(condense), int(rows_after_vars), int(small_front), float(zero_frac), _i(pos), C.byref(st))
    if rc != 0:
        raise SqpHipError(f"sqphip_kkt_symbolic failed ({rc})")
    out = {k: getattr(st, k) for k, _ in _lib.SymbolicStats._fields_}
    return pos[:out["order"]], out


def mf_host_solve(n, m, jrow, jcol, hrow, hcol, gL, gU, condense, jval, hval, Dd, sigp, hd, rtype, hsc, dw, rhs):
    L = _lib.lib()
    jr, jc, hr, hc = (np.ascontiguousarray(a, dtype=np.int64) for a in (jrow, jcol, hrow, hcol))
    rhs = _f(rhs); sol = np.zeros_like(rhs); dinv = np.zeros_like(rhs); npos = C.c_int32()
    rt = np.ascontiguousarray(rtype, dtype=np.int32)
    rc = L.sqphip_mf_host_solve(n, m, len(jr), _l(jr), _l(jc), len(hr), _l(hr), _l(hc), _d(_f(gL)), _d(_f(gU)),
                                int(condense), _d(_f(jval)), _d(_f(hval)), _d(_f(Dd)), _d(_f(sigp)), _d(_f(hd)), _i(rt),
                                float(hsc), float(dw), _d(rhs), _d(sol), _d(dinv), C.byref(npos))
    if rc != 0:
        raise SqpHipError(f"sqphip_mf_host_solve failed ({rc})")
    return sol, dinv, npos.value


def mf_host_top2_err() -> float:
    return float(_lib.lib().sqphip_mf_host_top2_err())


def mf_host_spine_err() -> float:
    return float(_lib.lib().sqphip_mf_host_spine_err())


def mf_plan_info(n, m, jrow, jcol, hrow, hcol, gL, gU, condense=1, batch=1):
    L = _lib.lib()
    jr, jc, hr, hc = (np.ascontiguousarray(a, dtype=np.int64) for a in (jrow, jcol, hrow, hcol))
    nf, nl, top, sp = C.c_int32(), C.c_int32(), C.c_int64(), C.c_int32()
    args = (n, m, len(jr), _l(jr), _l(jc), len(hr), _l(hr), _l(hc), _d(_f(gL)), _d(_f(gU)), int(condense), int(batch))
    if L.sqphip_mf_plan_info(*args, None, 0, C.byref(nf), None, 0, C.byref(nl), C.byref(top), C.byref(sp)) != 0:
        raise SqpHipError("sqphip_mf_plan_info failed")
    fr = np.zeros((nf.value, 3), dtype=np.int32); la = np.zeros((nl.value, 4), dtype=np.int32)
    if L.sqphip_mf_plan_info(*args, _i(fr), nf.value, C.byref(nf), _i(la), nl.value, C.byref(nl), C.byref(top), C.byref(sp)) != 0:
        raise SqpHipError("sqphip_mf_plan_info failed")
    return fr, la, top.value, sp.value


class Context:

    def __init__(self, n, m, num_linear, jrow, jcol, hrow, hcol, xL, xU, gL, gU,
                 options: _lib.Options | None = None, batch: int = 1):
        self.L = _lib.lib()
        self.n, self.m, self.batch = int(n), int(m), int(batch)
        self.nnzj, self.nnzh = len(jrow), len(hrow)
        self.opts = options or default_options()
        jr, jc, hr, hc = (np.ascontiguousarray(a, dtype=np.int64) for a in (jrow, jcol, hrow, hcol))
        h = C.c_void_p()
        rc = self.L.sqphip_create(C.byref(h), n, m, num_linear, len(jr), _l(jr), _l(jc), len(hr), _l(hr),
                                  _l(hc), _d(_f(xL)), _d(_f(xU)), _d(_f(gL)), _d(_f(gU)),
                                  C.byref(self.opts), batch)
        if rc != 0:
            raise SqpHipError(f"sqphip_create failed with code {rc}")
        self.h = h

    def close(self):
        if getattr(self, "h", None):
            self.L.sqphip_destroy(self.h)
            self.h = None

    def __del__(self):
        try:
            self.close()
        except Exception:
            pass

    def _ck(self, rc):
        if rc != 0:
            msg = self.L.sqphip_last_error(self.h)
            raise SqpHipError(f"libsqphip error {rc}: {msg.decode() if msg else ''}")

    def qp_solve(self, mode, x_k, delta, mu, df, E, jval, hval):
        p = np.zeros(self.n); lam = np.zeros(self.m)
        mu_u = np.zeros(self.n); mu_l = np.zeros(self.n); slack = np.zeros(2 * self.m)
        st = C.c_int32()
        self._ck(self.L.sqphip_qp_solve(self.h, mode, _d(_f(x_k)), float(delta), float(mu), _d(_f(df)),
                                        _d(_f(E)), _d(_f(jval)),
                                        _d(_f(hval)) if hval is not None and len(hval) else None,
                                        _d(p), _d(lam), _d(mu_u), _d(mu_l), _d(slack), C.byref(st)))
        it, nf = C.c_int32(), C.c_int32()
        self.L.sqphip_qp_stats(self.h, C.byref(it), C.byref(nf))
        rule, err = C.c_int32(), C.c_double()
        self.L.sqphip_qp_termination(self.h, C.byref(rule), C.byref(err))
        return dict(p=p, lam=lam, mult_x_U=mu_u, mult_x_L=mu_l, slack=slack, status=st.value,
                    ipm_iters=it.value, n_factor=nf.value, term_rule=rule.value, scaled_error=err.value)

    def _insts(self, inst):
        a = np.ascontiguousarray(inst, dtype=np.int32)
        if a.ndim != 1 or len(a) == 0:
            raise ValueError("inst must be a non-empty list of instance numbers")
        return a

    @staticmethod
    def _rows(name, rows, count, width):
        if rows is None:
            return None
        rows = list(rows) if not isinstance(rows, np.ndarray) else rows
        if len(rows) != count:
            raise ValueError(f"{name}: {len(rows)} rows for {count} requests")
        for k, r in enumerate(rows):
            if r is None or np.ndim(r) != 1 or len(r) != width:
                raise ValueError(f"{name}[{k}]: expected a vector of length {width}")
        return np.ascontiguousarray(np.asarray(rows, dtype=np.float64).reshape(count, width))

    @staticmethod
    def _scalars(name, v, count):
        a = np.ascontiguousarray(np.broadcast_to(np.asarray(v, dtype=np.float64), (count,)) if np.ndim(v) == 0 else v,
                                 dtype=np.float64)
        if a.shape != (count,):
            raise ValueError(f"{name}: expected {count} values")
        return a

    def qp_solve_batch(self, inst, mode, x_k, delta, mu, df, E, jval, hval):
        ins = self._insts(inst); cnt = len(ins)
        md = np.ascontiguousarray(mode, dtype=np.int32)
        if md.shape != (cnt,):
            raise ValueError(f"mode: expected {cnt} values")
        dl, pen = self._scalars("delta", delta, cnt), self._scalars("mu", mu, cnt)
        xk = self._rows("x_k", x_k, cnt, self.n); c = self._rows("df", df, cnt, self.n); b = self._rows("E", E, cnt, self.m)
        jv = self._rows("jval", jval, cnt, self.nnzj)
        hv = self._rows("hval", hval, cnt, self.nnzh) if hval is not None and self.nnzh and all(h is not None for h in hval) else None
        if hval is not None and self.nnzh and hv is None and any(h is not None for h in hval):
            raise ValueError("hval: given for some requests only")
        p = np.zeros((cnt, self.n)); lam = np.zeros((cnt, self.m)); mu_u = np.zeros((cnt, self.n)); mu_l = np.zeros((cnt, self.n))
        slack = np.zeros((cnt, 2 * self.m)); st = np.zeros(cnt, dtype=np.int32)
        self._ck(self.L.sqphip_qp_solve_batch(self.h, cnt, _i(ins), _i(md), _d(xk), _d(dl), _d(pen), _d(c), _d(b), _d(jv), _d(hv),
                                              _d(p), _d(lam), _d(mu_u), _d(mu_l), _d(slack), _i(st)))
        stats = self.qp_stats_batch(ins)
        return [dict(p=p[k].copy(), lam=lam[k].copy(), mult_x_U=mu_u[k].copy(), mult_x_L=mu_l[k].copy(), slack=slack[k].copy(),
                     status=int(st[k]), **stats[k]) for k in range(cnt)]

    def qp_stats_batch(self, inst):
        ins = self._insts(inst); cnt = len(ins)
        it = np.zeros(cnt, dtype=np.int32); nf = np.zeros(cnt, dtype=np.int32); rule = np.zeros(cnt, dtype=np.int32); err = np.zeros(cnt)
        self._ck(self.L.sqphip_qp_stats_batch(self.h, cnt, _i(ins), _i(it), _i(nf), _i(rule), _d(err)))
        return [dict(ipm_iters=int(it[k]), n_factor=int(nf[k]), term_rule=int(rule[k]), scaled_error=float(err[k])) for k in range(cnt)]

    def seat_peek(self, inst):
        p = np.zeros(self.n); lam = np.zeros(self.m); mu_u = np.zeros(self.n); mu_l = np.zeros(self.n); slack = np.zeros(2 * self.m)
        st = C.c_int32()
        self._ck(self.L.sqphip_seat_peek(self.h, int(inst), _d(p), _d(lam), _d(mu_u), _d(mu_l), _d(slack), C.byref(st)))
        return dict(p=p, lam=lam, mult_x_U=mu_u, mult_x_L=mu_l, slack=slack, status=st.value)

    _PN = {1: 1, 2: 2, math.inf: 0, "inf": 0}

    def norm_violations_batch(self, inst, E, x, p=1):
        ins = self._insts(inst); cnt = len(ins); out = np.zeros(cnt)
        self._ck(self.L.sqphip_norm_violations_batch(self.h, cnt, _i(ins), _d(self._rows("E", E, cnt, self.m)),
                                                     _d(self._rows("x", x, cnt, self.n)), self._PN[p], _d(out)))
        return out

    def kt_residuals_batch(self, inst, df, lam, mult_x_U, mult_x_L, jval):
        ins = self._insts(inst); cnt = len(ins); out = np.zeros(cnt)
        self._ck(self.L.sqphip_kt_residuals_batch(self.h, cnt, _i(ins), _d(self._rows("df", df, cnt, self.n)),
                                                  _d(self._rows("lam", lam, cnt, self.m)),
                                                  _d(self._rows("mult_x_U", mult_x_U, cnt, self.n)),
                                                  _d(self._rows("mult_x_L", mult_x_L, cnt, self.n)),
                                                  _d(self._rows("jval", jval, cnt, self.nnzj)), _d(out)))
        return out

    def norm_complementarity_batch(self, inst, E, lam, p=math.inf):
        ins = self._insts(inst); cnt = len(ins); out = np.zeros(cnt)
        self._ck(self.L.sqphip_norm_complementarity_batch(self.h, cnt, _i(ins), _d(self._rows("E", E, cnt, self.m)),
                                                          _d(self._rows("lam", lam, cnt, self.m)), self._PN[p], _d(out)))
        return out

    def compute_phi_batch(self, inst, f_trial, E_trial, x_trial, mu, fr):
        ins = self._insts(inst); cnt = len(ins); out = np.zeros(cnt)
        self._ck(self.L.sqphip_compute_phi_batch(self.h, cnt, _i(ins), _d(self._scalars("f_trial", f_trial, cnt)),
                                                 _d(self._rows("E_trial", E_trial, cnt, self.m)),
                                                 _d(self._rows("x_trial", x_trial, cnt, self.n)),
                                                 _d(self._scalars("mu", mu, cnt)), int(fr), _d(out)))
        return out

    def compute_qmodel_batch(self, inst, x, p, df, E, jval, hval, mu, with_step):
        ins = self._insts(inst); cnt = len(ins); out = np.zeros(cnt)
        hv = self._rows("hval", hval, cnt, self.nnzh) if hval is not None and self.nnzh and all(h is not None for h in hval) else None
        self._ck(self.L.sqphip_compute_qmodel_batch(self.h, cnt, _i(ins), _d(self._rows("x", x, cnt, self.n)),
                                                    _d(self._rows("p", p, cnt, self.n)), _d(self._rows("df", df, cnt, self.n)),
                                                    _d(self._rows("E", E, cnt, self.m)), _d(self._rows("jval", jval, cnt, self.nnzj)),
                                                    _d(hv), _d(self._scalars("mu", mu, cnt)), int(with_step), _d(out)))
        return out

    def compute_derivative_full_batch(self, inst, df, p, E, mu, mu_vec=None, feasibility_restoration=False, slack=None):
        ins = self._insts(inst); cnt = len(ins); out = np.zeros(cnt)
        self._ck(self.L.sqphip_compute_derivative_full_batch(
            self.h, cnt, _i(ins), _d(self._rows("df", df, cnt, self.n)), _d(self._rows("p", p, cnt, self.n)),
            _d(self._rows("E", E, cnt, self.m)), _d(self._scalars("mu", mu, cnt)), _d(self._rows("mu_vec", mu_vec, cnt, self.m)),
            int(feasibility_restoration), _d(self._rows("slack", slack, cnt, 2 * self.m)), _d(out)))
        return out

    def compute_derivative_full(self, df, p, E, mu, mu_vec=None, feasibility_restoration=False, slack=None):
        out = C.c_double()
        self._ck(self.L.sqphip_compute_derivative_full(self.h, _d(_f(df)), _d(_f(p)), _d(_f(E)), float(mu), _d(_f(mu_vec)),
                                                       int(feasibility_restoration), _d(_f(slack)), C.byref(out)))
        return out.value

    def compute_mu_rule(self, rule, it, rho, x, E, df, p, hval, lam, mu):
        mu = _f(mu).copy()
        self._ck(self.L.sqphip_compute_mu_rule_dev(self.h, int(rule), int(it), float(rho), _d(_f(x)), _d(_f(E)), _d(_f(df)),
                                                   _d(_f(p)), _d(_f(hval)) if hval is not None and len(hval) else None,
                                                   _d(_f(lam)), _d(mu)))
        return mu

    def acopf_armijo(self, inst, x, p, mu, phi0, D, eta=0.4, tau=0.9, min_alpha=1e-6, feasibility_restoration=False):
        al = C.c_double(); ok = C.c_int32(); ne = C.c_int32()
        self._ck(self.L.sqphip_acopf_armijo(self.h, inst, _d(_f(x)), _d(_f(p)), float(mu), float(phi0), float(D), float(eta),
                                            float(tau), float(min_alpha), int(feasibility_restoration), C.byref(al),
                                            C.byref(ok), C.byref(ne)))
        return al.value, bool(ok.value), ne.value

    def mf_solve_test(self, inst, jval, hval, Dd, sigp, hd, rtype, hsc, dw, rhs):
        rhs = _f(rhs); a = np.zeros_like(rhs); b = np.zeros_like(rhs); dv = np.zeros_like(rhs)
        rt = np.ascontiguousarray(rtype, dtype=np.int32)
        self._ck(self.L.sqphip_mf_solve_test(self.h, inst, _d(_f(jval)), _d(_f(hval)), _d(_f(Dd)), _d(_f(sigp)),
                                             _d(_f(hd)), _i(rt), float(hsc), float(dw), _d(rhs), _d(a), _d(b), _d(dv)))
        return a, b, dv

    def mf_batch_test(self, active, jval, hval, Dd, sigp, hd, rtype, hsc, dw, dw_last, fac_attempt, rhs):
        rhs = _f(rhs); B = rhs.shape[0]
        out = {k: np.zeros_like(rhs) for k in ("fused", "standalone", "dinv0", "dinv1")}
        dec = np.zeros((B, 5), dtype=np.int32); dwo = np.zeros(B)
        i32 = lambda a: np.ascontiguousarray(a, dtype=np.int32)
        act, rt, fa = i32(active), i32(rtype), i32(fac_attempt)
        self._ck(self.L.sqphip_mf_batch_test(self.h, _i(act), _d(_f(jval)), _d(_f(hval)), _d(_f(Dd)), _d(_f(sigp)), _d(_f(hd)),
                                             _i(rt), _d(_f(hsc)), _d(_f(dw)), _d(_f(dw_last)), _i(fa), _d(rhs),
                                             _d(out["fused"]), _d(out["standalone"]), _d(out["dinv0"]), _d(out["dinv1"]),
                                             _i(dec), _d(dwo)))
        out["decision"] = dec; out["dw"] = dwo
        return out

    def mf_census(self):
        nk = C.c_int32()
        self._ck(self.L.sqphip_mf_census(self.h, None, None, 0, C.byref(nk)))
        cnt = np.zeros(nk.value, dtype=np.int64); names = C.create_string_buffer(64 * nk.value)
        self._ck(self.L.sqphip_mf_census(self.h, _l(cnt), names, nk.value, C.byref(nk)))
        return {names.raw[64 * k:64 * (k + 1)].split(b"\0")[0].decode(): int(cnt[k]) for k in range(nk.value)}

    def trans_inline_groups(self):
        out = C.c_int64()
        self._ck(self.L.sqphip_trans_inline_groups(self.h, C.byref(out)))
        return int(out.value)

    def norm_violations(self, E, x, p=1):
        out = C.c_double()
        pn = {1: 1, 2: 2, math.inf: 0, "inf": 0}[p]
        self._ck(self.L.sqphip_norm_violations(self.h, _d(_f(E)), _d(_f(x)), pn, C.byref(out)))
        return out.value

    def kt_residuals(self, df, lam, mult_x_U, mult_x_L, jval):
        out = C.c_double()
        self._ck(self.L.sqphip_kt_residuals(self.h, _d(_f(df)), _d(_f(lam)), _d(_f(mult_x_U)),
                                            _d(_f(mult_x_L)), _d(_f(jval)), C.byref(out)))
        return out.value

    def norm_complementarity(self, E, lam, p=math.inf):
        out = C.c_double()
        pn = {1: 1, 2: 2, math.inf: 0, "inf": 0}[p]
        self._ck(self.L.sqphip_norm_complementarity(self.h, _d(_f(E)), _d(_f(lam)), pn, C.byref(out)))
        return out.value

    def compute_phi(self, f_trial, E_trial, x_trial, mu, fr):
        out = C.c_double()
        self._ck(self.L.sqphip_compute_phi(self.h, float(f_trial), _d(_f(E_trial)), _d(_f(x_trial)),
                                           float(mu), int(fr), C.byref(out)))
        return out.value

    def compute_qmodel(self, x, p, df, E, jval, hval, mu, with_step):
        out = C.c_double()
        self._ck(self.L.sqphip_compute_qmodel(self.h, _d(_f(x)), _d(_f(p)), _d(_f(df)), _d(_f(E)),
                                              _d(_f(jval)),
                                              _d(_f(hval)) if hval is not None and len(hval) else None,
                                              float(mu), int(with_step), C.byref(out)))
        return out.value

    def compute_derivative(self, df, p, E, mu):
        out = C.c_double()
        self._ck(self.L.sqphip_compute_derivative(self.h, _d(_f(df)), _d(_f(p)), _d(_f(E)), float(mu),
                                                  C.byref(out)))
        return out.value

    def tr_update(self, ared, pred, delta, pnorm, delta_max=1e8):
        acc = C.c_int32(); dn = C.c_double()
        self._ck(self.L.sqphip_tr_update(float(ared), float(pred), float(delta), float(pnorm),
                                         float(delta_max), float(self.opts.tol_direction),
                                         C.byref(acc), C.byref(dn)))
        return bool(acc.value), dn.value

    def acopf_attach(self, net, lay):
        keep = [np.ascontiguousarray(a, dtype=np.int32) for a in
                (net.f_bus, net.t_bus, net.gen_bus, lay.bal_ptr, lay.bal_colP, lay.bal_colQ)]
        coef = _f(lay.bal_coef)
        form = getattr(lay, "form", "polar")
        if form == "acwr":
            bp = [np.ascontiguousarray(a, dtype=np.int32) for a in (lay.bp_i, lay.bp_j, lay.br_bp)]
            self._ck(self.L.sqphip_acopf_attach_acwr(self.h, net.nb, net.ng, net.nl, *[_i(a) for a in keep], _d(coef),
                                                     int(net.ref_bus), len(bp[0]), *[_i(a) for a in bp], _d(_f(lay.br_sig)),
                                                     _d(_f(lay.bp_tmin)), _d(_f(lay.bp_tmax))))
        else:
            attach = self.L.sqphip_acopf_attach_acr if form == "acr" else self.L.sqphip_acopf_attach
            self._ck(attach(self.h, net.nb, net.ng, net.nl, *[_i(a) for a in keep], _d(coef), int(net.ref_bus)))
        if len(lay.dc_loss1):
            self._ck(self.L.sqphip_acopf_set_dclines(self.h, len(lay.dc_loss1), _d(_f(lay.dc_loss1))))
        if len(lay.sh_bus):
            sb = np.ascontiguousarray(lay.sh_bus, dtype=np.int32)
            self._ck(self.L.sqphip_acopf_set_shunts(self.h, len(sb), _i(sb), _d(_f(lay.sh_gs)), _d(_f(lay.sh_bs))))

    def set_bounds(self, inst, lay):
        self._ck(self.L.sqphip_set_bounds(self.h, inst, _d(_f(lay.xL)), _d(_f(lay.xU)), _d(_f(lay.gL)),
                                          _d(_f(lay.gU))))

    def acopf_set_instance(self, inst, net, lay, x0=None):
        ohm = _f(net.branch_coeffs().ravel())
        self._ck(self.L.sqphip_set_bounds(self.h, inst, _d(_f(lay.xL)), _d(_f(lay.xU)), _d(_f(lay.gL)),
                                          _d(_f(lay.gU))))
        self._ck(self.L.sqphip_acopf_set_instance(self.h, inst, _d(ohm), _d(_f(net.c2)),
                                                  _d(_f(net.c1)), _d(_f(lay.x0 if x0 is None else x0))))

    def dense_attach(self, nlp):
        self._ck(self.L.sqphip_dense_attach(self.h, _d(_f(nlp.Q.ravel())), _d(_f(nlp.A.ravel())), float(nlp.kappa)))

    def dense_set_instance(self, inst, nlp, lay, x0=None):
        self._ck(self.L.sqphip_set_bounds(self.h, inst, _d(_f(lay.xL)), _d(_f(lay.xU)), _d(_f(lay.gL)), _d(_f(lay.gU))))
        self._ck(self.L.sqphip_dense_set_instance(self.h, inst, _d(_f(nlp.c)), _d(_f(lay.x0 if x0 is None else x0))))

    def qcqp_attach(self, q):
        t = [np.ascontiguousarray(a, dtype=np.int64) for a in (q.q0r, q.q0c, q.ar, q.ac, q.qi, q.qr, q.qc)]
        v = [_f(a) for a in (q.q0v, q.av, q.qv, q.c, q.g0)]
        self._ck(self.L.sqphip_qcqp_attach(self.h, len(v[0]), _l(t[0]), _l(t[1]), _d(v[0]), len(v[1]), _l(t[2]), _l(t[3]),
                                           _d(v[1]), len(v[2]), _l(t[4]), _l(t[5]), _l(t[6]), _d(v[2]), _d(v[3]), _d(v[4]),
                                           float(q.f0)))

    def qcqp_set_instance(self, inst, q=None, x0=None, **values):
        if q is not None:
            self.set_bounds(inst, q)
            values = {**{k: getattr(q, k) for k in ("f0", "c", "q0v", "g0", "av", "qv")}, **values}
            x0 = q.x0 if x0 is None else x0
        bad = set(values) - {"f0", "c", "q0v", "g0", "av", "qv"}
        if bad:
            raise TypeError(f"qcqp_set_instance: unknown values {sorted(bad)}")
        arr = [None if values.get(k) is None else _f(np.atleast_1d(values[k])) for k in ("f0", "c", "q0v", "g0", "av", "qv")]
        self._ck(self.L.sqphip_qcqp_set_instance(self.h, inst, *[_d(a) for a in arr], _d(_f(x0))))

    def nlp_attach(self, p):
        if getattr(p, "aptr", None) is not None:
            t = [np.ascontiguousarray(a, dtype=np.int64) for a in (p.trow, p.tptr, p.aptr, p.avar)]
            k = [np.ascontiguousarray(a, dtype=np.int32) for a in (p.fkind, p.fexp)]
            v = [_f(a) for a in (p.tcoef, p.acoef, p.fshift, p.g0)]
            self._ck(self.L.sqphip_nlp_attach_affine(self.h, len(t[0]), _l(t[0]), _d(v[0]), _l(t[1]), _l(t[2]), _l(t[3]), _d(v[1]),
                                                     _i(k[0]), _i(k[1]), _d(v[2]), _d(v[3]), float(p.f0)))
            return
        t = [np.ascontiguousarray(a, dtype=np.int64) for a in (p.trow, p.tptr, p.fvar)]
        k = [np.ascontiguousarray(a, dtype=np.int32) for a in (p.fkind, p.fexp)]
        v = [_f(a) for a in (p.tcoef, p.fscale, p.fshift, p.g0)]
        self._ck(self.L.sqphip_nlp_attach(self.h, len(t[0]), _l(t[0]), _d(v[0]), _l(t[1]), _l(t[2]), _i(k[0]), _i(k[1]),
                                          _d(v[1]), _d(v[2]), _d(v[3]), float(p.f0)))

    def nlp_set_instance(self, inst, p=None, x0=None, **values):
        if p is not None:
            self.set_bounds(inst, p)
            values = {**{k: getattr(p, k) for k in ("f0", "g0", "tcoef")}, **values}
            x0 = p.x0 if x0 is None else x0
        bad = set(values) - {"f0", "g0", "tcoef"}
        if bad:
            raise TypeError(f"nlp_set_instance: unknown values {sorted(bad)}")
        arr = [None if values.get(k) is None else _f(np.atleast_1d(values[k])) for k in ("f0", "g0", "tcoef")]
        self._ck(self.L.sqphip_nlp_set_instance(self.h, inst, *[_d(a) for a in arr], _d(_f(x0))))

    def acopf_eval(self, inst, x, sigma=1.0, lam=None):
        f = C.c_double(); grad = np.zeros(self.n); g = np.zeros(self.m)
        jv = np.zeros(self.nnzj); hv = np.zeros(self.nnzh) if lam is not None else None
        self._ck(self.L.sqphip_acopf_eval(self.h, inst, _d(_f(x)), float(sigma), _d(_f(lam)), C.byref(f),
                                          _d(grad), _d(g), _d(jv), _d(hv)))
        return dict(f=f.value, grad=grad, g=g, jval=jv, hval=hv)

    def sqp_reset(self):
        self._ck(self.L.sqphip_sqp_reset(self.h))

    def sqp_run(self, max_outer=0):
        self._ck(self.L.sqphip_sqp_run(self.h, int(max_outer)))

    def sqp_get(self, inst):
        x = np.zeros(self.n); g = np.zeros(self.m); mg = np.zeros(self.m)
        ml = np.zeros(self.n); mu = np.zeros(self.n)
# ... 232 lines not shown
```

Before: 9407.

## Stage KKT value items in LDS per block and pack factor2 front images

Replaces the one-thread-per-destination KKT value assembly kernel with a blocked kernel. Each 256-thread block loads up to 256 items cooperatively into shared memory, then sums them per destination, using a host-built block partition. It also adds a packed triangular-tile LDS layout for the image variant of the factor2 front kernel, enabled by default, to shrink LDS use and improve access patterns. The serial path and the unpacked layout stay available through environment variables, and test hooks compare the two value paths.

```diff
diff --git a/include/sqphip_test_hooks.h b/include/sqphip_test_hooks.h
--- a/include/sqphip_test_hooks.h
+++ b/include/sqphip_test_hooks.h
@@ -19,6 +19,16 @@
                          const double *sigp, const double *hd, const int32_t *rtype, const double *hsc, const double *dw,
                          const double *dw_last, const int32_t *fac_attempt, const double *rhs, double *sol_fused,
                          double *sol_standalone, double *dinv0, double *dinv1, int32_t *decision, double *dw_out);
+int sqphip_mf_values_test(sqphip_ctx *ctx, const int32_t *active, const double *Jval, const double *Hval, const double *Dd,
+                          const double *sigp, const double *hd, const int32_t *rtype, const double *hsc, const double *dw,
+                          const double *dw_last, const int32_t *fac_attempt, double sentinel, double *vals0, double *vals1,
+                          int64_t *nnzK);
+int sqphip_mf_values_blocks(int64_t n, int64_t m, int64_t nnzJ, const int64_t *jrow, const int64_t *jcol, int64_t nnzH,
+                            const int64_t *hrow, const int64_t *hcol, const double *gL, const double *gU, int32_t condense,
+                            const double *Jval, const double *Hval, const double *Dd, const double *sigp, const double *hd,
+                            const int32_t *rtype, double hsc, double dw, int32_t *blocks, int32_t cap_blocks,
+                            int32_t *n_blocks, int32_t *item_ptr, int64_t cap_dest, int64_t *n_dest, int64_t *n_items,
+                            double *vals_list, double *vals_block);
 int sqphip_mf_census(const sqphip_ctx *ctx, int64_t *counts, char *names, int32_t cap, int32_t *n_kernels);
 int sqphip_trans_inline_groups(const sqphip_ctx *ctx, int64_t *count);
 int sqphip_mf_plan_info(int64_t n, int64_t m, int64_t nnzJ, const int64_t *jrow, const int64_t *jcol, int64_t nnzH,
diff --git a/sqpsolver.jl_amd/__init__.py b/sqpsolver.jl_amd/__init__.py
--- a/sqpsolver.jl_amd/__init__.py
+++ b/sqpsolver.jl_amd/__init__.py
@@ -5,4 +5,4 @@
 from . import _lib
 from . import host
 from .host import (Context, QpData, QpHip, default_options, SqpHipError, kkt_order,
-                   kkt_symbolic, mf_host_solve, mf_host_top2_err, mf_host_spine_err, mf_plan_info)
+                   kkt_symbolic, mf_host_solve, mf_host_top2_err, mf_host_spine_err, mf_plan_info, mf_values_blocks)
diff --git a/sqpsolver.jl_amd/_lib.py b/sqpsolver.jl_amd/_lib.py
--- a/sqpsolver.jl_amd/_lib.py
+++ b/sqpsolver.jl_amd/_lib.py
@@ -203,6 +203,11 @@
             L.sqphip_mf_solve_test.argtypes = [vp, C.c_int32, dp, dp, dp, dp, dp, ip, C.c_double, C.c_double, dp, dp, dp, dp]
             L.sqphip_mf_batch_test.argtypes = [vp, ip, dp, dp, dp, dp, dp, ip, dp, dp, dp, ip, dp, dp, dp, dp, dp, ip, dp]
             L.sqphip_mf_census.argtypes = [vp, lp, C.c_char_p, C.c_int32, ip]
+            if not os.environ.get("SQPHIP_SO") or hasattr(L, "sqphip_mf_values_test"):
+                L.sqphip_mf_values_test.argtypes = [vp, ip, dp, dp, dp, dp, dp, ip, dp, dp, dp, ip, C.c_double, dp, dp, lp]
+                L.sqphip_mf_values_blocks.argtypes = [C.c_int64, C.c_int64, C.c_int64, lp, lp, C.c_int64, lp, lp, dp, dp, C.c_int32,
+                                                      dp, dp, dp, dp, dp, ip, C.c_double, C.c_double, ip, C.c_int32, ip, ip,
+                                                      C.c_int64, lp, lp, dp, dp]
             if hasattr(L, "sqphip_trans_inline_groups"):
                 L.sqphip_trans_inline_groups.argtypes = [vp, lp]
             L.sqphip_mf_plan_info.argtypes = [C.c_int64, C.c_int64, C.c_int64, lp, lp, C.c_int64, lp, lp, dp, dp, C.c_int32,
@@ -248,7 +253,7 @@
     "sqphip_kt_residuals", "sqphip_norm_complementarity", "sqphip_compute_phi",
     "sqphip_compute_qmodel", "sqphip_compute_derivative", "sqphip_compute_derivative_full", "sqphip_compute_mu_rule_dev",
     "sqphip_acopf_armijo", "sqphip_tr_update",
-    "sqphip_kkt_order", "sqphip_kkt_symbolic", "sqphip_mf_host_solve", "sqphip_mf_host_top2_err", "sqphip_mf_host_spine_err", "sqphip_mf_solve_test", "sqphip_mf_batch_test", "sqphip_mf_census", "sqphip_trans_inline_groups", "sqphip_mf_plan_info", "sqphip_acopf_attach", "sqphip_acopf_attach_acr", "sqphip_acopf_attach_acwr", "sqphip_acopf_set_shunts", "sqphip_acopf_set_dclines", "sqphip_acopf_set_instance", "sqphip_dense_attach", "sqphip_dense_set_instance", "sqphip_qcqp_attach", "sqphip_qcqp_set_instance", "sqphip_nlp_attach", "sqphip_nlp_attach_affine", "sqphip_nlp_set_instance", "sqphip_acopf_eval", "sqphip_sqp_reset",
+    "sqphip_kkt_order", "sqphip_kkt_symbolic", "sqphip_mf_host_solve", "sqphip_mf_host_top2_err", "sqphip_mf_host_spine_err", "sqphip_mf_solve_test", "sqphip_mf_batch_test", "sqphip_mf_values_test", "sqphip_mf_values_blocks", "sqphip_mf_census", "sqphip_trans_inline_groups", "sqphip_mf_plan_info", "sqphip_acopf_attach", "sqphip_acopf_attach_acr", "sqphip_acopf_attach_acwr", "sqphip_acopf_set_shunts", "sqphip_acopf_set_dclines", "sqphip_acopf_set_instance", "sqphip_dense_attach", "sqphip_dense_set_instance", "sqphip_qcqp_attach", "sqphip_qcqp_set_instance", "sqphip_nlp_attach", "sqphip_nlp_attach_affine", "sqphip_nlp_set_instance", "sqphip_acopf_eval", "sqphip_sqp_reset",
     "sqphip_sqp_run", "sqphip_sqp_get", "sqphip_sqp_status", "sqphip_sqp_trace",
     "sqphip_comm_available", "sqphip_comm_unique_id", "sqphip_comm_init", "sqphip_gather_status", "sqphip_comm_destroy",
     "sqphip_get_counters", "sqphip_get_mode_counters", "sqphip_sqp_work", "sqphip_sqp_stream_begin", "sqphip_sqp_stream_set", "sqphip_sqp_stream_run", "sqphip_sqp_stream_get", "sqphip_sqp_stream_assign", "sqphip_sqp_stream_append", "sqphip_sqp_stream_release", "sqphip_sqp_stream_run_some", "sqphip_qcqp_stream_begin", "sqphip_qcqp_stream_set", "sqphip_nlp_stream_begin", "sqphip_nlp_stream_set", "sqphip_sqp_stream_get_full", "sqphip_sqp_last_request", "sqphip_sqp_qp_log", "sqphip_reset_counters", "sqphip_set_timing", "sqphip_get_kernel_times", "sqphip_ldlt_factor_host",
diff --git a/sqpsolver.jl_amd/csrc/api.hip b/sqpsolver.jl_amd/csrc/api.hip
--- a/sqpsolver.jl_amd/csrc/api.hip
+++ b/sqpsolver.jl_amd/csrc/api.hip
@@ -337,6 +337,8 @@
                 M.off = C.upload(P.off);
                 M.asm_ptr = C.upload(P.asm_ptr); M.dest_loc = C.upload(P.dest_loc); M.item_ptr = C.upload(P.item_ptr);
                 M.items = C.upload(P.items); M.sched = C.upload(P.sched);
+                M.nvblk = (int)P.vblk.size();
+                if (M.nvblk > 0) { M.vitems = C.upload(P.vitems); M.vblk = C.upload(P.vblk); }
                 auto nz = [](const std::vector<int> &v) { return v.empty() ? std::vector<int>(1, 0) : v; };
                 M.dest_rc = C.upload(P.dest_rc);
                 M.ea_ptr = C.upload(P.ea_ptr); M.ea_rc = C.upload(nz(P.ea_rc));
@@ -648,6 +650,48 @@
     });
 }
 
+extern "C" int sqphip_mf_values_test(sqphip_ctx *h, const int32_t *active, const double *Jval, const double *Hval,
+                                     const double *Dd, const double *sigp, const double *hd, const int32_t *rtype,
+                                     const double *hsc, const double *dw, const double *dw_last, const int32_t *fac_attempt,
+                                     double sentinel, double *vals0, double *vals1, int64_t *nnzK)
+{
+    if (!h) return SQPHIP_EINVAL;
+    if (!h->c.d.sparse) { h->c.err = "sqphip_mf_values_test: the context does not use the sparse solver"; return SQPHIP_ESTATE; }
+    if (nnzK) *nnzK = h->c.d.mf.nnzK;
+    if (!vals0 && !vals1) return SQPHIP_OK;
+    if (!active || !Jval || !Dd || !sigp || !hd || !rtype || !hsc || !dw || !dw_last || !fac_attempt) return SQPHIP_EINVAL;
+    return guarded(h, [&](Ctx &C) {
+        DV &d = C.d;
+        const int B = d.B;
+        const size_t nv = (size_t)B * d.mf.nnzK;
+        for (int b = 0; b < B; ++b) {
+            const size_t on = (size_t)b * d.n, om = (size_t)b * d.m;
+            h2d(C, d.jcoo + (size_t)b * d.nnzj_coo, Jval + (size_t)b * d.nnzj_coo, d.nnzj_coo);
+            if (Hval) h2d(C, d.hcoo + (size_t)b * d.nnzh_coo, Hval + (size_t)b * d.nnzh_coo, d.nnzh_coo);
+            else SQPHIP_HIP_OK(hipMemsetAsync(d.hcoo + (size_t)b * d.nnzh_coo, 0, sizeof(double) * (size_t)d.nnzh_coo, C.stream));
+            h2d(C, d.Dd + om, Dd + om, d.m); h2d(C, d.sigp + on, sigp + on, d.n); h2d(C, d.hd + on, hd + on, d.n);
+            SQPHIP_HIP_OK(hipMemcpyAsync(d.rtype + om, rtype + om, sizeof(int) * (size_t)d.m, hipMemcpyHostToDevice, C.stream));
+            hipLaunchKernelGGL(k_mf_inst_set, dim3(1), dim3(64), 0, C.stream, d, b, active[b] ? 1 : 0, (int)PH_IDLE, 0.0, 0.0, 0.0, 0);
+        }
+        launch_qp_gather(C);
+        for (int b = 0; b < B; ++b)
+            hipLaunchKernelGGL(k_mf_inst_set, dim3(1), dim3(64), 0, C.stream, d, b, 0, active[b] ? (int)PH_FACTOR : (int)PH_IDLE,
+                               hsc[b], dw[b], dw_last[b], (int)fac_attempt[b]);
+        std::vector<double> fill(nv, sentinel), out1(nv, sentinel);
+        h2d(C, d.mf.vals, fill.data(), nv);
+        if (d.mf.vals1) h2d(C, d.mf.vals1, fill.data(), nv);
+        mf_values(C, PH_FACTOR);
+        if (vals0) d2h(C, vals0, d.mf.vals, nv);
+        if (d.mf.vals1) d2h(C, out1.data(), d.mf.vals1, nv);
+        for (int b = 0; b < B; ++b)
+            hipLaunchKernelGGL(k_mf_inst_set, dim3(1), dim3(64), 0, C.stream, d, b, 0, (int)PH_IDLE, 0.0, 0.0, 0.0, 0);
+        SQPHIP_HIP_OK(hipStreamSynchronize(C.stream));
+        SQPHIP_HIP_OK(hipGetLastError());
+        if (vals1) std::copy(out1.begin(), out1.end(), vals1);
+        return SQPHIP_OK;
+    });
+}
+
 extern "C" int sqphip_mf_census(const sqphip_ctx *h, int64_t *counts, char *names, int32_t cap, int32_t *n_kernels)
 {
     if (!h || cap < 0 || (cap > 0 && !counts)) return SQPHIP_EINVAL;
diff --git a/sqpsolver.jl_amd/csrc/ctx.hpp b/sqpsolver.jl_amd/csrc/ctx.hpp
--- a/sqpsolver.jl_amd/csrc/ctx.hpp
+++ b/sqpsolver.jl_amd/csrc/ctx.hpp
@@ -67,6 +67,9 @@
     double *fronts1, *vals1;
     const int *asm_ptr, *dest_loc, *dest_rc, *item_ptr;
     const MfItem *items;
+    const MfItem *vitems;
+    const MfValBlock *vblk;
+    int nvblk;
     const int *ea_ptr, *ea_rc, *ea_src_ptr, *ea_src;
     const int *ev_ptr, *ev_idx, *ev_src_ptr, *ev_src;
     const MfFrontDesc *desc;
@@ -244,6 +247,7 @@
 void launch_qp_gather(Ctx &C);
 void comm_release(Ctx &C);
 void mf_device_setup(Ctx &C);
+void mf_values(Ctx &C, int want);
 void mf_factor(Ctx &C, int want, bool with_rhs, bool values_done = false);
 void mf_solve(Ctx &C, int want, bool skip_fwd, bool inertia = false, int also = -1);
 bool mf_solve_tests_inertia(const Ctx &C);
diff --git a/sqpsolver.jl_amd/csrc/mfplan.hip b/sqpsolver.jl_amd/csrc/mfplan.hip
--- a/sqpsolver.jl_amd/csrc/mfplan.hip
+++ b/sqpsolver.jl_amd/csrc/mfplan.hip
@@ -72,6 +72,21 @@
     P.item_ptr.push_back((int)P.items.size());
     for (int s = 0; s < S.ns; ++s) P.asm_ptr[s + 1] += P.asm_ptr[s];
     P.nnzK = (long)P.dest_loc.size();
+    {
+        int longest = 0;
+        for (long e = 0; e < P.nnzK; ++e) longest = std::max(longest, P.item_ptr[e + 1] - P.item_ptr[e]);
+        if (longest <= MF_VBLK_ITEMS && m > 0 && !jrslot.empty()) {
+            P.vitems = P.items;
+            for (MfItem &it : P.vitems) { if (it.row < 0) it.row = 0; if (it.a < 0) it.a = 0; if (it.b < 0) it.b = 0; }
+            MfValBlock blk{0, 0, 0, 0};
+            for (int e = 0; e < (int)P.nnzK; ++e) {
+                const int cnt = P.item_ptr[e + 1] - P.item_ptr[e];
+                if (blk.nitems + cnt > MF_VBLK_ITEMS) { P.vblk.push_back(blk); blk = MfValBlock{e, P.item_ptr[e], 0, 0}; }
+                blk.ndest++; blk.nitems += cnt;
+            }
+            if (blk.ndest > 0) P.vblk.push_back(blk);
+        }
+    }
     P.dest_rc.resize(P.dest_loc.size());
     for (int s = 0; s < S.ns; ++s) {
         const int ld = S.sn_nc[s] + S.sn_nr[s] + 1;
@@ -578,6 +593,59 @@
     return SQPHIP_OK;
 }
 
+extern "C" int sqphip_mf_values_blocks(int64_t n, int64_t m, int64_t nnzJ, const int64_t *jrow, const int64_t *jcol, int64_t nnzH,
+                                       const int64_t *hrow, const int64_t *hcol, const double *gL, const double *gU,
+                                       int32_t condense, const double *Jval, const double *Hval, const double *Dd,
+                                       const double *sigp, const double *hd, const int32_t *rtype, double hsc, double dw,
+                                       int32_t *blocks, int32_t cap_blocks, int32_t *n_blocks, int32_t *item_ptr,
+                                       int64_t cap_dest, int64_t *n_dest, int64_t *n_items, double *vals_list, double *vals_block)
+{
+    if (n <= 0 || m < 0 || cap_blocks < 0 || cap_dest < 0 || (cap_blocks > 0 && !blocks)) return SQPHIP_EINVAL;
+    using namespace sqphip;
+    std::vector<double> jv, hv;
+    const MfPlan P = host_plan(n, m, nnzJ, jrow, jcol, nnzH, hrow, hcol, gL, gU, condense, SymOptions(), Jval, Hval, jv, hv);
+    if (n_blocks) *n_blocks = (int32_t)P.vblk.size();
+    if (n_dest) *n_dest = P.nnzK;
+    if (n_items) *n_items = (int64_t)P.items.size();
+    for (int k = 0; k < (int)P.vblk.size() && k < cap_blocks; ++k) {
+        const MfValBlock &b = P.vblk[k];
+        blocks[4 * k] = b.dest0; blocks[4 * k + 1] = b.item0; blocks[4 * k + 2] = b.ndest; blocks[4 * k + 3] = b.nitems;
+    }
+    if (cap_dest < P.nnzK) return SQPHIP_OK;
+    if (item_ptr) std::copy(P.item_ptr.begin(), P.item_ptr.end(), item_ptr);
+    if (!vals_list && !vals_block) return SQPHIP_OK;
+    if (!Jval || !Dd || !sigp || !hd) return SQPHIP_EINVAL;
+    std::vector<int> rt(m > 0 ? m : 1, 1);
+    for (int64_t i = 0; i < m; ++i) rt[i] = rtype ? rtype[i] : 1;
+    const MfValues V{hv.data(), jv.data(), Dd, sigp, hd, rt.data(), hsc, dw};
+    if (vals_list)
+        for (long e = 0; e < P.nnzK; ++e) {
+            double a = 0.0;
+            for (int k = P.item_ptr[e]; k < P.item_ptr[e + 1]; ++k) a += item_value(P.items[k], V);
+            vals_list[e] = a;
+        }
+    if (vals_block)
+        for (const MfValBlock &b : P.vblk) {
+            double stage[MF_VBLK_ITEMS];
+            for (int t = 0; t < b.nitems; ++t) {
+                const MfItem it = P.vitems[b.item0 + t];
+                const double *p1 = it.type == MF_ITEM_H ? V.hv : (it.type == MF_ITEM_VDIAG ? V.hd : V.jv);
+                const double *p3 = it.type == MF_ITEM_VDIAG ? V.sigp + it.a : V.Dd + it.row;
+                const bool live = V.rtype[it.row] != 0;
+                const double x = p1[it.a], y = V.jv[it.b], z = *p3;
+                stage[t] = it.type == MF_ITEM_H ? hsc * x : it.type == MF_ITEM_JKEPT ? (live ? x : 0.0)
+                         : it.type == MF_ITEM_PAIR ? (live ? x * y / (z + 1e-8) : 0.0)
+                         : it.type == MF_ITEM_VDIAG ? x + z + dw + 1e-8 : (live ? -(z + 1e-8) : -1.0);
+            }
+            for (int t = 0; t < b.ndest; ++t) {
+                double a = 0.0;
+                for (int k = P.item_ptr[b.dest0 + t] - b.item0; k < P.item_ptr[b.dest0 + t + 1] - b.item0; ++k) a += stage[k];
+                vals_block[b.dest0 + t] = a;
+            }
+        }
+    return SQPHIP_OK;
+}
+
 extern "C" int sqphip_mf_plan_info(int64_t n, int64_t m, int64_t nnzJ, const int64_t *jrow, const int64_t *jcol, int64_t nnzH,
                                    const int64_t *hrow, const int64_t *hcol, const double *gL, const double *gU,
                                    int32_t condense, int32_t batch, int32_t *fronts, int32_t cap_fronts, int32_t *n_fronts,
diff --git a/sqpsolver.jl_amd/csrc/mfront.hip b/sqpsolver.jl_amd/csrc/mfront.hip
--- a/sqpsolver.jl_amd/csrc/mfront.hip
+++ b/sqpsolver.jl_amd/csrc/mfront.hip
@@ -116,7 +116,7 @@
 }
 #endif
 
-__global__ __launch_bounds__(256) void k_mf_values(DV d, int want)
+__global__ __launch_bounds__(256) void k_mf_values_serial(DV d, int want)
 {
     int inst, cand;
     if (!mf_candidate(d, want, inst, cand)) return;
@@ -133,6 +133,46 @@
     mf_vals(d, inst, cand)[e] = a;
 }
 
+__global__ __launch_bounds__(MF_VBLK_ITEMS) void k_mf_values(DV d, int want)
+{
+    int inst, cand;
+    if (!mf_candidate(d, want, inst, cand)) return;
+    const MfDev &M = d.mf;
+    __shared__ double val[MF_VBLK_ITEMS];
+    const MfValBlock Bk = M.vblk[blockIdx.x];
+    const int t = threadIdx.x;
+    int k0 = 0, k1 = 0;
+    if (t < Bk.ndest) { k0 = M.item_ptr[Bk.dest0 + t]; k1 = M.item_ptr[Bk.dest0 + t + 1]; }
+    if (t < Bk.nitems) {
+        const IpmState &st = d.ist[inst];
+        const double hsc = st.hsc, dw = cand ? next_shift(st.dw, st.dw_last) : st.dw;
+        const int4 rec = reinterpret_cast<const int4 *>(M.vitems)[Bk.item0 + t];
+        const int type = rec.x, row = rec.y, a = rec.z, b = rec.w;
+        const double *jv = d.jv + (long)inst * d.nnzjc;
+        const double *p1 = type == MF_ITEM_H ? d.hv + (long)inst * d.nnzhc : (type == MF_ITEM_VDIAG ? d.hd + (long)inst * d.n : jv);
+        const double *p3 = type == MF_ITEM_VDIAG ? d.sigp + (long)inst * d.n + a : d.Dd + (long)inst * d.m + row;
+        int rtv = d.rtype[(long)inst * d.m + row];
+        double x = p1[a], y = jv[b], z = *p3;
+        asm volatile("" : "+v"(rtv), "+v"(x), "+v"(y), "+v"(z));
+        const bool live = rtv != ROW_FREE;
+        double v;
+        switch (type) {
+        case MF_ITEM_H: v = hsc * x; break;
+        case MF_ITEM_JKEPT: v = live ? x : 0.0; break;
+        case MF_ITEM_PAIR: v = live ? x * y / (z + MF_REG_D) : 0.0; break;
+        case MF_ITEM_VDIAG: v = x + z + dw + MF_REG_P; break;
+        default: v = live ? -(z + MF_REG_D) : -1.0; break;
+        }
+        val[t] = v;
+    }
+    __syncthreads();
+    if (t < Bk.ndest) {
+        double acc = 0.0;
+        for (int k = k0 - Bk.item0; k < k1 - Bk.item0; ++k) acc += val[k];
+        mf_vals(d, inst, cand)[Bk.dest0 + t] = acc;
+    }
+}
+
 typedef double d4 __attribute__((ext_vector_type(4)));
 
 #ifndef SQPHIP_MF_RCP_NR
@@ -179,9 +219,21 @@
 #endif
 }
 
-template <int NW, int MAXT, bool LDSIMG>
+__device__ __forceinline__ int mf_pk(int row, int col)
+{
+    const int ti = row >> 4;
+    return 256 * ((ti * (ti + 1) >> 1) + (col >> 4)) + 16 * (col & 15) + (row & 15);
+}
+static constexpr size_t mf_factor2_lds_doubles(int T, bool img, bool packed)
+{
+    const size_t R = 16 * (size_t)T, pan = 9 * R + 16, tri = 128 * (size_t)T * (T + 1);
+    return !img ? pan : packed ? (tri > pan ? tri : pan) : R * R + pan;
+}
+
+template <int NW, int MAXT, bool LDSIMG, bool PACKED = false>
 __global__ __launch_bounds__(64 * NW) void k_mf_factor2(DV d, int sbegin, int want, int with_rhs, int Tl)
 {
+    static_assert(LDSIMG || !PACKED, "the packed layout is that of the LDS image");
     constexpr int NT = 64 * NW;
     int inst, cand;
     if (!mf_candidate(d, want, inst, cand)) return;
@@ -193,14 +245,15 @@
     double *G = mf_arena(d, inst, cand) + Fd.off;
     extern __shared__ double mf_lds[];
     const int R = 16 * Tl;
-    double *Xp = mf_lds + (LDSIMG ? R * R : 0), *Lp = Xp + 4 * R, *blk = Lp + 4 * R, *dl = blk + 16;
+    double *Xp = mf_lds + (LDSIMG && !PACKED ? R * R : 0), *Lp = Xp + 4 * R, *blk = Lp + 4 * R, *dl = blk + 16;
     double *F = LDSIMG ? mf_lds : G;
     const int LD = LDSIMG ? R : ld;
     const int tid = threadIdx.x, lane = tid & 63, l15 = lane & 15, l4 = lane >> 4;
     const int wave = __builtin_amdgcn_readfirstlane(tid >> 6);
     const int T = (ld + 15) >> 4;
     MF_TR(0)
-    if (LDSIMG) {
+    if (PACKED) for (int e = tid; e < 128 * T * (T + 1); e += NT) F[e] = 0.0;
+    else if (LDSIMG) {
         if (T == Tl) for (int e = tid; e < R * R; e += NT) F[e] = 0.0;
         else for (int e = tid; e < 256 * T * T; e += NT) F[(e / (16 * T)) * LD + e % (16 * T)] = 0.0;
     } else for (int e = tid; e < ld * fs; e += NT) F[e] = 0.0;
@@ -210,11 +263,11 @@
         const double *vals = mf_vals(d, inst, cand);
         for (int e = Fd.asm_begin + tid; e < Fd.asm_end; e += NT) {
             const int rc = M.dest_rc[e];
-            F[(rc >> 16) * LD + (rc & 0xffff)] = vals[e];
+            F[PACKED ? mf_pk(rc & 0xffff, rc >> 16) : (rc >> 16) * LD + (rc & 0xffff)] = vals[e];
         }
         if (with_rhs) {
             const double *b = d.xv + (long)inst * d.Fpad + f0;
-            for (int j = tid; j < nc; j += NT) F[j * LD + fs] = b[j];
+            for (int j = tid; j < nc; j += NT) F[PACKED ? mf_pk(fs, j) : j * LD + fs] = b[j];
         }
     }
     __syncthreads();
@@ -224,7 +277,7 @@
         double a = arena[g.src0];
         for (int q = g.src_begin + 1; q < g.src_end; ++q) a += arena[M.ea_src[q]];
         const int rc = g.where;
-        F[(rc >> 16) * LD + (rc & 0xffff)] += a;
+        F[PACKED ? mf_pk(rc & 0xffff, rc >> 16) : (rc >> 16) * LD + (rc & 0xffff)] += a;
     }
     __syncthreads();
     MF_TR(3)
@@ -241,7 +294,7 @@
         for (int rr = 0; rr < 4; ++rr) {
             const int col = 16 * tj + l4 + 4 * rr, row = 16 * ti + l15;
             const bool in = valid && (LDSIMG || (row <= fs && col < fs));
-            acc[q][rr] = in ? F[col * LD + row] : 0.0;
+            acc[q][rr] = in ? F[PACKED ? 256 * ((ti * (ti + 1) >> 1) + tj) + 64 * rr + lane : col * LD + row] : 0.0;
         }
     }
     __syncthreads();
@@ -1734,6 +1787,18 @@
     C.mf_big_lds = ok;
 }
 
+void mf_values(Ctx &C, int want)
+{
+    const DV &d = C.d;
+    hipStream_t s = C.stream;
+    const int nb = d.mf.fronts1 && d.spec_mode != 0 ? 2 * d.B : d.B;
+    const bool serial = d.mf.nvblk == 0 || (getenv("SQPHIP_MF_VALUES_SERIAL") && atoi(getenv("SQPHIP_MF_VALUES_SERIAL")) != 0);
+    C.tm.open(s); C.mf_census[MFK_VALUES]++;
+    if (serial) hipLaunchKernelGGL(k_mf_values_serial, dim3((d.mf.nnzK + 255) / 256, nb), dim3(256), 0, s, d, want);
+    else hipLaunchKernelGGL(k_mf_values, dim3(d.mf.nvblk, nb), dim3(MF_VBLK_ITEMS), 0, s, d, want);
+    C.tm.close(KC_VALUES, s);
+}
+
 void mf_factor(Ctx &C, int want, bool with_rhs, bool values_done)
 {
     const DV &d = C.d;
@@ -1741,8 +1806,9 @@
     static const bool v1 = getenv("SQPHIP_MF_V1") != nullptr;
     const int wr = (int)with_rhs;
     const int nb = d.mf.fronts1 && d.spec_mode != 0 ? 2 * d.B : d.B;
-    if (!v1 && !values_done) { C.tm.open(s); C.mf_census[MFK_VALUES]++; hipLaunchKernelGGL(k_mf_values, dim3((d.mf.nnzK + 255) / 256, nb), dim3(256), 0, s, d, want); C.tm.close(KC_VALUES, s); }
+    if (!v1 && !values_done) mf_values(C, want);
     const bool stat = !(getenv("SQPHIP_MF_STATIC") && atoi(getenv("SQPHIP_MF_STATIC")) == 0);
+    const bool packed = !(getenv("SQPHIP_MF_F2_PACKED") && atoi(getenv("SQPHIP_MF_F2_PACKED")) == 0);
     const bool spine = !v1 && d.mf.sp_n > 0 && C.mf_big_lds;
     int li = 0, cls_open = -1;
     for (const MfLaunch &L : C.mfp().fac) {
@@ -1750,9 +1816,11 @@
         const int cls = L.level >= C.mfp().narrow_level ? KC_FRONTS_TOP : KC_FRONTS_LOW;
         if (cls != cls_open) { if (cls_open >= 0) C.tm.close(cls_open, s); C.tm.open(s); cls_open = cls; }
         const dim3 grid(L.count, nb);
-        const int T = L.tiles, R = 16 * T;
+        const int T = L.tiles;
         if (v1 || T > 13) { C.mf_census[MFK_FACTOR_R1]++; hipLaunchKernelGGL((k_mf_factor<256, true>), grid, dim3(256), 0, s, d, L.begin, want, wr); continue; }
-#define MF_GENERIC(NW, MAXT, IMG) do { constexpr int kid_ = mf_factor2_kid(NW, MAXT, IMG); static_assert(kid_ >= 0, "census: no counter"); C.mf_census[kid_]++; hipLaunchKernelGGL((k_mf_factor2<NW, MAXT, IMG>), grid, dim3(64 * NW), 8 * (size_t)((IMG ? R * R : 0) + 9 * R + 16), s, d, L.begin, want, wr, T); } while (0)
+#define MF_GENERIC(NW, MAXT, IMG) do { constexpr int kid_ = mf_factor2_kid(NW, MAXT, IMG); static_assert(kid_ >= 0, "census: no counter"); C.mf_census[kid_]++; \
+        if (IMG && packed) hipLaunchKernelGGL((k_mf_factor2<NW, MAXT, IMG, IMG>), grid, dim3(64 * NW), 8 * mf_factor2_lds_doubles(T, IMG, true), s, d, L.begin, want, wr, T); \
+        else hipLaunchKernelGGL((k_mf_factor2<NW, MAXT, IMG, false>), grid, dim3(64 * NW), 8 * mf_factor2_lds_doubles(T, IMG, false), s, d, L.begin, want, wr, T); } while (0)
 #define MF_STATIC(TT, NW, IMG) do { constexpr int kid_ = mf_front_kid(TT, NW, IMG); static_assert(kid_ >= 0, "census: no counter"); C.mf_census[kid_]++; hipLaunchKernelGGL((k_mf_front<TT, NW, IMG>), grid, dim3(64 * NW), 8 * (size_t)mf_front_lds_doubles(TT, NW, IMG), s, d, L.begin, want, wr); } while (0)
         const int stat_min = getenv("SQPHIP_MF_STATIC_MIN") ? atoi(getenv("SQPHIP_MF_STATIC_MIN")) : (L.count <= 8 && L.level >= C.mfp().narrow_level ? 1 : 4);
         const bool nw8 = !(getenv("SQPHIP_MF_NW8") && atoi(getenv("SQPHIP_MF_NW8")) == 0);
diff --git a/sqpsolver.jl_amd/csrc/sparse.hpp b/sqpsolver.jl_amd/csrc/sparse.hpp
--- a/sqpsolver.jl_amd/csrc/sparse.hpp
+++ b/sqpsolver.jl_amd/csrc/sparse.hpp
@@ -59,6 +59,9 @@
        MF_ITEM_RDIAG = 4 };
 struct MfItem { int type, row, a, b; };
 
+constexpr int MF_VBLK_ITEMS = 256;
+struct MfValBlock { int dest0, item0, ndest, nitems; };
+
 struct MfFrontDesc { int nc, nr, first, rowptr, off, asm_begin, asm_end, ea_begin, ea_end, ev_begin, ev_end, pad; };
 struct MfGather { int where, src_begin, src_end, src0; };
 
@@ -74,6 +77,8 @@
     long stride = 0;
     std::vector<int> asm_ptr, dest_loc, item_ptr;
     std::vector<MfItem> items;
+    std::vector<MfItem> vitems;
+    std::vector<MfValBlock> vblk;
     std::vector<int> dest_rc;
     std::vector<int> ea_ptr, ea_rc, ea_src_ptr, ea_src;
     std::vector<int> ev_ptr, ev_idx, ev_src_ptr, ev_src;
diff --git a/sqpsolver.jl_amd/host.py b/sqpsolver.jl_amd/host.py
--- a/sqpsolver.jl_amd/host.py
+++ b/sqpsolver.jl_amd/host.py
@@ -103,6 +103,31 @@
     if L.sqphip_mf_plan_info(*args, _i(fr), nf.value, C.byref(nf), _i(la), nl.value, C.byref(nl), C.byref(top), C.byref(sp)) != 0:
         raise SqpHipError("sqphip_mf_plan_info failed")
     return fr, la, top.value, sp.value
+
+
+def mf_values_blocks(n, m, jrow, jcol, hrow, hcol, gL, gU, condense=1, values=None):
+    L = _lib.lib()
+    jr, jc, hr, hc = (np.ascontiguousarray(a, dtype=np.int64) for a in (jrow, jcol, hrow, hcol))
+    nb, nd, ni = C.c_int32(), C.c_int64(), C.c_int64()
+    head = (n, m, len(jr), _l(jr), _l(jc), len(hr), _l(hr), _l(hc), _d(_f(gL)), _d(_f(gU)), int(condense))
+    none = (None, None, None, None, None, None, 0.0, 0.0)
+    if L.sqphip_mf_values_blocks(*head, *none, None, 0, C.byref(nb), None, 0, C.byref(nd), C.byref(ni), None, None) != 0:
+        raise SqpHipError("sqphip_mf_values_blocks failed")
+    blocks = np.zeros((nb.value, 4), dtype=np.int32); ptr = np.zeros(nd.value + 1, dtype=np.int32)
+    out = {"blocks": blocks, "item_ptr": ptr, "n_items": ni.value, "vals_list": None, "vals_block": None}
+    vals = none; vl = vb = None
+    if values is not None:
+        jval, hval, Dd, sigp, hd, rtype, hsc, dw = values
+        rt = np.ascontiguousarray(rtype, dtype=np.int32)
+        vals = (_d(_f(jval)), _d(_f(hval)), _d(_f(Dd)), _d(_f(sigp)), _d(_f(hd)), _i(rt), float(hsc), float(dw))
+        vl = np.zeros(nd.value); vb = np.zeros(nd.value)
+    if L.sqphip_mf_values_blocks(*head, *vals, _i(blocks) if nb.value else None, nb.value, C.byref(nb), _i(ptr), nd.value,
+                                 C.byref(nd), C.byref(ni), _d(vl) if vl is not None else None,
+                                 _d(vb) if vb is not None else None) != 0:
+        raise SqpHipError("sqphip_mf_values_blocks failed")
+    if values is not None:
+        out["vals_list"] = vl; out["vals_block"] = vb if nb.value else None
+    return out
 
 
 class Context:
@@ -298,6 +323,17 @@
         out["decision"] = dec; out["dw"] = dwo
         return out
 
+    def mf_values_test(self, active, jval, hval, Dd, sigp, hd, rtype, hsc, dw, dw_last, fac_attempt, sentinel=-7.5):
+        nk = C.c_int64()
+        self._ck(self.L.sqphip_mf_values_test(self.h, *([None] * 11), 0.0, None, None, C.byref(nk)))
+        i32 = lambda a: np.ascontiguousarray(a, dtype=np.int32)
+        act, rt, fa = i32(active), i32(rtype), i32(fac_attempt)
+        v0 = np.zeros((len(act), nk.value)); v1 = np.zeros_like(v0)
+        self._ck(self.L.sqphip_mf_values_test(self.h, _i(act), _d(_f(jval)), _d(_f(hval)), _d(_f(Dd)), _d(_f(sigp)), _d(_f(hd)),
+                                              _i(rt), _d(_f(hsc)), _d(_f(dw)), _d(_f(dw_last)), _i(fa), float(sentinel),
+                                              _d(v0), _d(v1), C.byref(nk)))
+        return v0, v1
+
     def mf_census(self):
         nk = C.c_int32()
         self._ck(self.L.sqphip_mf_census(self.h, None, None, 0, C.byref(nk)))
```

Result: faster. 10160, median of 6 (+8.0%).
